# uiuc-robovision/video-dqn

Hardware: AMD Instinct MI355X
Metric: (s,a,r,s') TD-updates/sec, 224x224 frames, batch 256, 1/2/4/8 MI355X (higher is better)
Workload: dtype bf16; 1 GPU; HabitatDQNMultiAction ResNet-18 extra_capacity, 5 categories x 3 actions, full TD update (online fwd on [s;s'], target fwd on s', Double-DQN target + L2 TD loss, backward, Adam); batch_per_gpu=256, global_batch=256, frame=224x224x3 uint8 (normalise fused), parallelism=dp1, target_update_interval=1000, loss_clip=rect, loss_kind=l2, minibatch_pool=4, frame_pack=at the start of every update

## Files before the change

include/vdqn.h:

```cpp
#ifndef VDQN_H_
#define VDQN_H_

#include <stddef.h>
#include <stdint.h>

#ifdef __cplusplus
extern "C" {
#endif

#define VDQN_F32 0
#define VDQN_BF16 1
#define VDQN_F32X3 2

#define VDQN_OK 0
#define VDQN_ERR_INVALID (-1)
#define VDQN_ERR_LAUNCH (-2)

const char* vdqn_last_error(void);
int vdqn_abi_version(void);
int32_t vdqn_abi_struct_size(int32_t which);

typedef struct vdqn_prof_entry {
  char name[48];
  int64_t launches;
  double ms;
  double flops;
  double bytes;
} vdqn_prof_entry;
int vdqn_profile_enable(int on);
int vdqn_profile_collect(vdqn_prof_entry* out, int max_entries);


typedef struct vdqn_conv_args {
  const void* in;
  const void* wt;
  const float* bias;
  const void* resid;
  const void* mask;
  void* out;
  float* out_f32;
  float* colsum_part;
  int32_t n_img, hi, wi, ci, pix_stride;
  int32_t ho, wo, co, ldo;
  int32_t r, s, stride, pad;
  int32_t mode, relu, dtype;
  const void* in2;
  const void* wt2;
  const float* bias2;
  void* out2;
  int32_t co2, ldo2, relu2, ci2;
} vdqn_conv_args;
int vdqn_conv2d(const vdqn_conv_args* a, void* stream);
int32_t vdqn_conv2d_colsum_rows(const vdqn_conv_args* a);

typedef struct vdqn_wgrad_args {
  const void* gy;
  const void* x;
  float* dw;
  float* dbias;
  int32_t n_img, hi, wi, ci, pix_stride;
  int32_t ho, wo, co, ldg;
  int32_t r, s, stride, pad;
  int32_t splitk, dtype;
  void* workspace;
  int64_t workspace_bytes;
} vdqn_wgrad_args;
int vdqn_conv2d_wgrad(const vdqn_wgrad_args* a, void* stream);
int64_t vdqn_conv2d_wgrad_workspace_bytes(const vdqn_wgrad_args* a);

int vdqn_host_gather(void* dst, const void* const* src, int64_t n, int64_t bytes_each, int32_t threads);

int vdqn_pack_input(const void* src, int32_t src_kind, void* dst, int32_t n_img, int32_t dtype, void* stream);

int vdqn_maxpool_fwd(const void* in, void* out, uint8_t* idx, int32_t n_img, int32_t hi, int32_t wi, int32_t c,
                     int32_t dtype, void* stream);
int vdqn_maxpool_bwd(const void* gy, const uint8_t* idx, const void* x, void* gx, int32_t n_img, int32_t hi,
                     int32_t wi, int32_t c, int32_t dtype, void* stream);

typedef struct vdqn_td_args {
  const float* q_before;
  const float* q_after_online;
  const float* q_after_target;
  const int64_t* act;
  const float* rew;
  const float* term;
  const float* valid;
  float* loss;
  void* dq;
  float* dq_f32;
  int32_t batch, n_cat, n_act, ldq;
  float gamma, inv_count;
  int32_t clip_rect, linear, use_valid, dtype;
  int32_t loss_kind;
  int32_t deterministic;
  float* q_copy;
} vdqn_td_args;
int vdqn_td_loss(const vdqn_td_args* a, void* stream);
int vdqn_td_loss_weighted(const vdqn_td_args* a, const float* weight, float* err_out, void* stream);

int vdqn_gt_loss(const float* q_before, const int64_t* act, const float* gt, float* loss, void* dq, float* dq_f32,
                 int32_t batch, int32_t n_cat, int32_t n_act, int32_t ldq, float inv_count, int32_t value_learning,
                 int32_t dtype, void* stream);

int vdqn_stem_conv_pool(const void* t_in, const void* wt, const float* bias, void* pool, void* idx, int32_t n_img,
                        int32_t dtype, void* stream);
int vdqn_stem_conv_pool_n(const void* t_in, const void* wt, const float* bias, void* pool, void* idx, int32_t n_img,
                          int32_t n_idx_img, int32_t dtype, void* stream);

int vdqn_stem_wgrad_pool(const void* g_pool, const uint8_t* idx, const void* t_in, float* dw, int32_t n_img, void* workspace,
                         int64_t workspace_bytes, void* stream);
int64_t vdqn_stem_wgrad_pool_workspace_bytes(int32_t n_img);

int vdqn_softmax_rows(const float* x, float* y, int32_t rows, int32_t ld, int32_t n_valid, void* stream);

int vdqn_softmax_ce(const float* logits, const int64_t* labels, float* loss, void* dlogits, int32_t rows, int32_t ld,
                    int32_t n_cls, float inv_count, int32_t dtype, void* stream);
int vdqn_mask_scale(const void* x, const void* mask, void* out, int64_t n, float scale, int32_t dtype, void* stream);
int vdqn_axpy(float* y, const float* x, float alpha, int64_t n, void* stream);

int vdqn_adam(float* p, const float* g, float* m, float* v, int64_t n, int32_t step, double lr, double beta1,
              double beta2, double eps, void* stream);

int vdqn_bn_train_fwd(const void* y, const void* resid, void* z, const float* gamma, const float* beta,
                      float* running_mean, float* running_var, float* work, int32_t n_img, int32_t hw, int32_t c,
                      int32_t num_frames, int32_t imgs_per_half, int32_t relu, float momentum, float eps, int32_t dtype,
                      void* workspace, int64_t workspace_bytes, void* stream);
int vdqn_bn_train_bwd(const void* g, const void* y, void* dy, float* work, float* dgamma, float* dbeta, int32_t n_img,
                      int32_t hw, int32_t c, int32_t num_frames, int32_t imgs_per_half, int32_t dtype, void* workspace,
                      int64_t workspace_bytes, void* stream);
int64_t vdqn_bn_train_workspace_bytes(int32_t n_img, int32_t hw, int32_t c, int32_t num_frames, int32_t imgs_per_half);
int vdqn_avgpool_fwd(const void* x, void* out, int32_t n_img, int32_t hw, int32_t c, int32_t dtype, void* stream);
int vdqn_avgpool_bwd(const void* g, const void* x, void* gx, int32_t n_img, int32_t hw, int32_t c, int32_t dtype,
                     void* stream);

typedef struct vdqn_net_config {
  int32_t action_dim;
  int32_t num_classes;
  int32_t num_frames;
  int32_t extra_capacity;
  int32_t dtype;
// ... 60 lines not shown
  const float* term;
  const float* valid;
  const float* gt;
  float gamma;
  float inv_count;
  int32_t clip_rect, linear, use_valid, train_on_ground_truth, value_learning;
  void* acts_online;
  void* acts_target;
  void* bwd;
  float* grads;
  float* loss;
  float* q_before;
  int32_t loss_kind;
  const void* packed_frames;
  int32_t acts_samples;
} vdqn_step_args;
int vdqn_net_td_forward(vdqn_net* net, const vdqn_step_args* a, void* stream);
int vdqn_net_backward_stage(vdqn_net* net, const vdqn_step_args* a, int32_t stage, void* stream);
int vdqn_net_backward_begin(vdqn_net* net, const vdqn_step_args* a, const float* dq_f32, void* stream);
void* vdqn_net_grad_stream(vdqn_net* net);
int vdqn_net_set_sample_weights(vdqn_net* net, const float* weight, float* err_out);

int64_t vdqn_per_workspace_bytes(int64_t n);
int vdqn_per_sample(const float* prio, int64_t n, int32_t global_batch, uint64_t seed, uint64_t step, double beta, void* workspace,
                    int64_t* idx_out, float* weight_out, void* stream);
int vdqn_per_update(float* prio, int64_t n, const int64_t* idx, const float* err, int32_t global_batch, double alpha, void* stream);

int vdqn_aug_draw(uint64_t seed, uint64_t step, int32_t global_batch, int32_t first, int32_t n, int32_t pad, int32_t flip,
                  int32_t* params, void* stream);
int vdqn_aug_swap_actions(const int64_t* act, const int32_t* params, int32_t n, int32_t a0, int32_t a1, int64_t* act_out,
                          void* stream);
int vdqn_pack_input_aug(const void* src, void* dst, int32_t n_img, int32_t frames_per_sample, const int32_t* params,
                        int32_t n_params, int32_t dtype, void* stream);
int vdqn_net_set_augment(vdqn_net* net, const int32_t* params);

#define VDQN_COMM_UID_BYTES 128
typedef struct vdqn_comm vdqn_comm;
int vdqn_comm_unique_id(void* uid_host);
int vdqn_comm_init(int32_t rank, int32_t nranks, const void* uid_host, vdqn_comm** out);
int vdqn_allreduce_bucket(vdqn_comm* comm, void* ptr, int64_t count, int32_t dtype, void* stream);
int vdqn_comm_rank(const vdqn_comm* comm);
int vdqn_comm_size(const vdqn_comm* comm);
int vdqn_comm_destroy(vdqn_comm* comm);

#ifdef __cplusplus
}
#endif
#endif
```

video_dqn_amd/_lib.py:

```python
from __future__ import annotations

import ctypes as C
import os

import torch

_HERE = os.path.dirname(os.path.abspath(__file__))
LIB_PATH = os.path.join(_HERE, "lib", f"libvdqn{'_' + os.environ['VDQN_LIB'] if os.environ.get('VDQN_LIB') else ''}.so")

VDQN_F32, VDQN_BF16, VDQN_F32X3 = 0, 1, 2
ABI_VERSION = 15

c_i32, c_i64, c_f32, c_vp = C.c_int32, C.c_int64, C.c_float, C.c_void_p


class ConvArgs(C.Structure):
    _fields_ = [("in_", c_vp), ("wt", c_vp), ("bias", c_vp), ("resid", c_vp), ("mask", c_vp), ("out", c_vp),
                ("out_f32", c_vp), ("colsum_part", c_vp),
                ("n_img", c_i32), ("hi", c_i32), ("wi", c_i32), ("ci", c_i32), ("pix_stride", c_i32),
                ("ho", c_i32), ("wo", c_i32), ("co", c_i32), ("ldo", c_i32),
                ("r", c_i32), ("s", c_i32), ("stride", c_i32), ("pad", c_i32),
                ("mode", c_i32), ("relu", c_i32), ("dtype", c_i32),
                ("in2", c_vp), ("wt2", c_vp), ("bias2", c_vp), ("out2", c_vp),
                ("co2", c_i32), ("ldo2", c_i32), ("relu2", c_i32), ("ci2", c_i32),
]


class WgradArgs(C.Structure):
    _fields_ = [("gy", c_vp), ("x", c_vp), ("dw", c_vp), ("dbias", c_vp),
                ("n_img", c_i32), ("hi", c_i32), ("wi", c_i32), ("ci", c_i32), ("pix_stride", c_i32),
                ("ho", c_i32), ("wo", c_i32), ("co", c_i32), ("ldg", c_i32),
                ("r", c_i32), ("s", c_i32), ("stride", c_i32), ("pad", c_i32),
                ("splitk", c_i32), ("dtype", c_i32), ("workspace", c_vp), ("workspace_bytes", c_i64)]


class TdArgs(C.Structure):
    _fields_ = [("q_before", c_vp), ("q_after_online", c_vp), ("q_after_target", c_vp), ("act", c_vp),
                ("rew", c_vp), ("term", c_vp), ("valid", c_vp), ("loss", c_vp), ("dq", c_vp), ("dq_f32", c_vp),
                ("batch", c_i32), ("n_cat", c_i32), ("n_act", c_i32), ("ldq", c_i32),
                ("gamma", c_f32), ("inv_count", c_f32),
                ("clip_rect", c_i32), ("linear", c_i32), ("use_valid", c_i32), ("dtype", c_i32), ("loss_kind", c_i32), ("deterministic", c_i32), ("q_copy", c_vp)]


class NetConfig(C.Structure):
    _fields_ = [("action_dim", c_i32), ("num_classes", c_i32), ("num_frames", c_i32), ("extra_capacity", c_i32),
                ("dtype", c_i32), ("max_batch", c_i32), ("deterministic", c_i32)]


class ParamInfo(C.Structure):
    _fields_ = [("name", C.c_char * 96), ("offset", c_i64), ("numel", c_i64), ("ndim", c_i32),
                ("shape", c_i32 * 4), ("kind", c_i32), ("param_id", c_i32), ("stage", c_i32)]


class ProfEntry(C.Structure):
    _fields_ = [("name", C.c_char * 48), ("launches", c_i64), ("ms", C.c_double), ("flops", C.c_double),
                ("bytes", C.c_double)]


class StepArgs(C.Structure):
    _fields_ = [("params", c_vp), ("bnstats", c_vp), ("packed_online", c_vp), ("packed_target", c_vp),
                ("before", c_vp), ("after", c_vp), ("src_kind", c_i32), ("batch", c_i32),
                ("act", c_vp), ("rew", c_vp), ("term", c_vp), ("valid", c_vp), ("gt", c_vp),
                ("gamma", c_f32), ("inv_count", c_f32),
                ("clip_rect", c_i32), ("linear", c_i32), ("use_valid", c_i32), ("train_on_ground_truth", c_i32),
                ("value_learning", c_i32),
                ("acts_online", c_vp), ("acts_target", c_vp), ("bwd", c_vp), ("grads", c_vp), ("loss", c_vp),
                ("q_before", c_vp), ("loss_kind", c_i32), ("packed_frames", c_vp), ("acts_samples", c_i32)]


ALLREDUCE_FN = C.CFUNCTYPE(None, c_vp, c_vp, c_i64, c_vp)

_SIGS = {
    "vdqn_last_error": (C.c_char_p, []),
    "vdqn_abi_version": (C.c_int, []),
    "vdqn_profile_enable": (C.c_int, [C.c_int]),
    "vdqn_profile_collect": (C.c_int, [C.POINTER(ProfEntry), C.c_int]),
    "vdqn_conv2d": (C.c_int, [C.POINTER(ConvArgs), c_vp]),
    "vdqn_abi_struct_size": (c_i32, [c_i32]),
    "vdqn_conv2d_colsum_rows": (c_i32, [C.POINTER(ConvArgs)]),
    "vdqn_conv2d_wgrad": (C.c_int, [C.POINTER(WgradArgs), c_vp]),
    "vdqn_conv2d_wgrad_workspace_bytes": (c_i64, [C.POINTER(WgradArgs)]),
    "vdqn_pack_input": (C.c_int, [c_vp, c_i32, c_vp, c_i32, c_i32, c_vp]),
    "vdqn_maxpool_fwd": (C.c_int, [c_vp, c_vp, c_vp, c_i32, c_i32, c_i32, c_i32, c_i32, c_vp]),
    "vdqn_maxpool_bwd": (C.c_int, [c_vp, c_vp, c_vp, c_vp, c_i32, c_i32, c_i32, c_i32, c_i32, c_vp]),
    "vdqn_stem_conv_pool": (C.c_int, [c_vp, c_vp, c_vp, c_vp, c_vp, c_i32, c_i32, c_vp]),
    "vdqn_stem_conv_pool_n": (C.c_int, [c_vp, c_vp, c_vp, c_vp, c_vp, c_i32, c_i32, c_i32, c_vp]),
    "vdqn_td_loss": (C.c_int, [C.POINTER(TdArgs), c_vp]),
    "vdqn_gt_loss": (C.c_int, [c_vp, c_vp, c_vp, c_vp, c_vp, c_vp, c_i32, c_i32, c_i32, c_i32, c_f32, c_i32, c_i32, c_vp]),
    "vdqn_adam": (C.c_int, [c_vp, c_vp, c_vp, c_vp, c_i64, c_i32, C.c_double, C.c_double, C.c_double, C.c_double, c_vp]),
    "vdqn_bn_train_fwd": (C.c_int, [c_vp, c_vp, c_vp, c_vp, c_vp, c_vp, c_vp, c_vp, c_i32, c_i32, c_i32, c_i32, c_i32, c_i32,
                                    c_f32, c_f32, c_i32, c_vp, c_i64, c_vp]),
    "vdqn_bn_train_bwd": (C.c_int, [c_vp, c_vp, c_vp, c_vp, c_vp, c_vp, c_i32, c_i32, c_i32, c_i32, c_i32, c_i32, c_vp, c_i64, c_vp]),
    "vdqn_bn_train_workspace_bytes": (c_i64, [c_i32, c_i32, c_i32, c_i32, c_i32]),
    "vdqn_avgpool_fwd": (C.c_int, [c_vp, c_vp, c_i32, c_i32, c_i32, c_i32, c_vp]),
    "vdqn_avgpool_bwd": (C.c_int, [c_vp, c_vp, c_vp, c_i32, c_i32, c_i32, c_i32, c_vp]),
    "vdqn_net_create": (C.c_int, [C.POINTER(NetConfig), C.POINTER(c_vp)]),
    "vdqn_net_destroy": (None, [c_vp]),
    "vdqn_stem_wgrad_pool": (C.c_int, [c_vp, c_vp, c_vp, c_vp, c_i32, c_vp, c_i64, c_vp]),
    "vdqn_stem_wgrad_pool_workspace_bytes": (c_i64, [c_i32]),
    "vdqn_net_set_overlap": (C.c_int, [c_vp, C.c_int]),
    "vdqn_net_grad_stream": (c_vp, [c_vp]),
    "vdqn_net_set_bn_sync": (C.c_int, [c_vp, c_vp, c_vp, c_i32]),
    "vdqn_net_num_params": (C.c_int, [c_vp]),
    "vdqn_net_param_info": (C.c_int, [c_vp, C.c_int, C.POINTER(ParamInfo)]),
    "vdqn_net_params_numel": (c_i64, [c_vp]),
    "vdqn_net_trainable_numel": (c_i64, [c_vp]),
    "vdqn_net_bnstats_numel": (c_i64, [c_vp]),
    "vdqn_net_stage_range": (C.c_int, [c_vp, C.c_int, C.POINTER(c_i64), C.POINTER(c_i64)]),
    "vdqn_net_packed_bytes": (c_i64, [c_vp]),
    "vdqn_net_acts_bytes": (c_i64, [c_vp, c_i32]),
    "vdqn_net_bwd_bytes": (c_i64, [c_vp, c_i32]),
    "vdqn_net_act_offset": (c_i64, [c_vp, c_i32, C.c_char_p]),
    "vdqn_net_bwd_offset": (c_i64, [c_vp, c_i32, C.c_char_p]),
    "vdqn_net_pack_weights": (C.c_int, [c_vp, c_vp, c_vp, c_vp, c_i32, c_vp]),
    "vdqn_net_forward": (C.c_int, [c_vp, c_vp, c_vp, c_i32, c_i32, c_vp, c_vp, c_vp]),
    "vdqn_net_trunk_forward": (C.c_int, [c_vp, c_vp, c_vp, c_i32, c_i32, c_vp, c_vp]),
    "vdqn_softmax_rows": (C.c_int, [c_vp, c_vp, c_i32, c_i32, c_i32, c_vp]),
    "vdqn_softmax_ce": (C.c_int, [c_vp, c_vp, c_vp, c_vp, c_i32, c_i32, c_i32, c_f32, c_i32, c_vp]),
    "vdqn_mask_scale": (C.c_int, [c_vp, c_vp, c_vp, c_i64, c_f32, c_i32, c_vp]),
    "vdqn_axpy": (C.c_int, [c_vp, c_vp, c_f32, c_i64, c_vp]),
    "vdqn_net_forward_train": (C.c_int, [c_vp, c_vp, c_vp, c_vp, c_vp, c_i32, c_i32, c_vp, c_vp, c_vp]),
    "vdqn_net_td_forward": (C.c_int, [c_vp, C.POINTER(StepArgs), c_vp]),
    "vdqn_net_backward_stage": (C.c_int, [c_vp, C.POINTER(StepArgs), c_i32, c_vp]),
    "vdqn_net_backward_begin": (C.c_int, [c_vp, C.POINTER(StepArgs), c_vp, c_vp]),
    "vdqn_comm_unique_id": (C.c_int, [c_vp]),
    "vdqn_comm_init": (C.c_int, [c_i32, c_i32, c_vp, C.POINTER(c_vp)]),
    "vdqn_allreduce_bucket": (C.c_int, [c_vp, c_vp, c_i64, c_i32, c_vp]),
    "vdqn_comm_rank": (C.c_int, [c_vp]),
    "vdqn_comm_size": (C.c_int, [c_vp]),
    "vdqn_comm_destroy": (C.c_int, [c_vp]),
    "vdqn_host_gather": (C.c_int, [c_vp, c_vp, c_i64, c_i64, c_i32]),
    "vdqn_td_loss_weighted": (C.c_int, [C.POINTER(TdArgs), c_vp, c_vp, c_vp]),
    "vdqn_net_set_sample_weights": (C.c_int, [c_vp, c_vp, c_vp]),
    "vdqn_per_workspace_bytes": (c_i64, [c_i64]),
    "vdqn_per_sample": (C.c_int, [c_vp, c_i64, c_i32, C.c_uint64, C.c_uint64, C.c_double, c_vp, c_vp, c_vp, c_vp]),
    "vdqn_per_update": (C.c_int, [c_vp, c_i64, c_vp, c_vp, c_i32, C.c_double, c_vp]),
    "vdqn_aug_draw": (C.c_int, [C.c_uint64, C.c_uint64, c_i32, c_i32, c_i32, c_i32, c_i32, c_vp, c_vp]),
    "vdqn_aug_swap_actions": (C.c_int, [c_vp, c_vp, c_i32, c_i32, c_i32, c_vp, c_vp]),
    "vdqn_pack_input_aug": (C.c_int, [c_vp, c_vp, c_i32, c_i32, c_vp, c_i32, c_i32, c_vp]),
    "vdqn_net_set_augment": (C.c_int, [c_vp, c_vp]),
}
COMM_UID_BYTES = 128
EXPORTS = tuple(_SIGS)

_lib = None


class VdqnError(RuntimeError):
    pass


def load():
    global _lib
    if _lib is not None:
        return _lib
    if not os.path.exists(LIB_PATH):
        raise VdqnError(f"{LIB_PATH} is missing: build it with `python -m video_dqn_amd.build` "
                        "(the HIP extension is required; there is no CPU fallback)")
    lib = C.CDLL(LIB_PATH)
    for name, (res, args) in _SIGS.items():
        fn = getattr(lib, name)
        fn.restype = res
        fn.argtypes = args
    if lib.vdqn_abi_version() != ABI_VERSION:
        raise VdqnError(f"libvdqn ABI {lib.vdqn_abi_version()} != binding ABI {ABI_VERSION}: rebuild")
    for which, st in enumerate((ConvArgs, WgradArgs, TdArgs, NetConfig, ParamInfo, ProfEntry, StepArgs)):
        if lib.vdqn_abi_struct_size(which) != C.sizeof(st):
            raise VdqnError(f"libvdqn: sizeof({st.__name__}) is {lib.vdqn_abi_struct_size(which)} in the library, "
                            f"{C.sizeof(st)} in this binding: include/vdqn.h and video_dqn_amd/_lib.py have drifted apart")
    _lib = lib
    return lib

# ... 17 lines not shown
```

video_dqn_amd/augment.py:

```python
from __future__ import annotations

import torch

from . import _lib

MAX_PAD = 32


def check_config(pad, flip, flip_actions) -> None:
    if isinstance(pad, bool) or not isinstance(pad, int) or not 0 <= pad <= MAX_PAD:
        raise ValueError(f"AUG_SHIFT_PAD must be an integer in [0, {MAX_PAD}] (got {pad!r})")
    if not isinstance(flip, bool):
        raise ValueError(f"AUG_FLIP must be True or False (got {flip!r})")
    fa = list(flip_actions) if isinstance(flip_actions, (list, tuple)) else None
    if (fa is None or len(fa) != 2 or any(isinstance(a, bool) or not isinstance(a, int) for a in fa)
            or fa[0] == fa[1] or not all(0 <= a <= 2 for a in fa)):
        raise ValueError(f"AUG_FLIP_ACTIONS must be two different actions out of 0, 1, 2 (got {flip_actions!r})")


def _u64(v: int) -> int:
    return int(v) & (2**64 - 1)


def aug_draw(seed: int, step: int, global_batch: int, first: int, n: int, pad: int, flip: bool, device="cuda",
             out: torch.Tensor = None) -> torch.Tensor:
    dev = torch.device(device) if out is None else out.device
    with torch.cuda.device(dev):
        if out is None:
            out = torch.empty((n, 4), dtype=torch.int32, device=dev)
        _lib.check(_lib.load().vdqn_aug_draw(_u64(seed), _u64(step), global_batch, first, n, pad, int(bool(flip)), out.data_ptr(),
                                             torch.cuda.current_stream().cuda_stream), "vdqn_aug_draw")
    return out


def pack_input_aug(src: torch.Tensor, params: torch.Tensor, frames_per_sample: int, dtype: torch.dtype) -> torch.Tensor:
    if src.dtype != torch.uint8 or not src.is_contiguous() or params.dtype != torch.int32 or not params.is_contiguous():
        raise _lib.VdqnError("pack_input_aug: src must be contiguous uint8 NHWC frames and params contiguous int32 [*][4]")
    n_img = src.numel() // (224 * 224 * 3)
    with torch.cuda.device(src.device):
        dst = torch.empty((n_img, 115, 115, 16), dtype=dtype, device=src.device)
        code = _lib.VDQN_BF16 if dtype == torch.bfloat16 else _lib.VDQN_F32
        _lib.check(_lib.load().vdqn_pack_input_aug(src.data_ptr(), dst.data_ptr(), n_img, frames_per_sample, params.data_ptr(),
                                                   params.numel() // 4, code, torch.cuda.current_stream().cuda_stream), "vdqn_pack_input_aug")
    return dst


class Augmenter:

    def __init__(self, batch: int, device, pad: int = 0, flip: bool = False, flip_actions=(1, 2), seed: int = 0, rank: int = 0,
                 world_size: int = 1):
        check_config(pad, flip, flip_actions)
        self.lib = _lib.load()
        self.B, self.rank, self.world = int(batch), int(rank), int(world_size)
        self.G = self.B * self.world
        self.pad, self.flip, self.flip_actions, self.seed = int(pad), bool(flip), tuple(int(a) for a in flip_actions), int(seed)
        self.device = torch.device(device)
        with torch.cuda.device(self.device):
            self.params = torch.zeros((self.B, 4), dtype=torch.int32, device=self.device)
            self._act = torch.zeros(self.B, dtype=torch.int64, device=self.device)
        self.last_step = None

    def draw(self, step: int) -> torch.Tensor:
        aug_draw(self.seed, step, self.G, self.rank * self.B, self.B, self.pad, self.flip, out=self.params)
        self.last_step = int(step)
        return self.params

    def actions(self, act: torch.Tensor) -> torch.Tensor:
        if not self.flip:
            return act
        if act.dtype != torch.int64 or act.numel() != self.B or not act.is_contiguous() or act.device != self.params.device:
            raise _lib.VdqnError(f"Augmenter.actions: act must be a contiguous int64 [{self.B}] tensor on {self.params.device}")
        with torch.cuda.device(self.device):
            _lib.check(self.lib.vdqn_aug_swap_actions(act.data_ptr(), self.params.data_ptr(), self.B, self.flip_actions[0], self.flip_actions[1],
                                                      self._act.data_ptr(), torch.cuda.current_stream().cuda_stream), "vdqn_aug_swap_actions")
        return self._act
```

video_dqn_amd/csrc/augment.hip:

```cpp
#include "common.h"

namespace {

constexpr uint64_t kAugStream = 0x4155474D454E5431ull;
constexpr int kMaxPad = 32;

__host__ __device__ inline uint64_t splitmix64(uint64_t x) {
  uint64_t z = x + 0x9E3779B97F4A7C15ull;
  z = (z ^ (z >> 30)) * 0xBF58476D1CE4E5B9ull;
  z = (z ^ (z >> 27)) * 0x94D049BB133111EBull;
  return z ^ (z >> 31);
}

__global__ __launch_bounds__(256) void aug_draw_kernel(uint64_t seed, uint64_t step, int G, int first, int n, int pad, int flip_on,
                                                       int4* __restrict__ params) {
  const int i = blockIdx.x * blockDim.x + threadIdx.x;
  if (i >= n) return;
  const uint64_t key = splitmix64(seed ^ kAugStream);
  const uint64_t h = splitmix64(key ^ (step * (uint64_t)G + (uint64_t)(first + i)));
  const uint32_t span = 2u * (uint32_t)pad + 1u;
  const int sx = (int)((((uint32_t)h & 0xFFFFu) * span) >> 16) - pad;
  const int sy = (int)((((uint32_t)(h >> 16) & 0xFFFFu) * span) >> 16) - pad;
  params[i] = make_int4(sx, sy, flip_on ? (int)((h >> 32) & 1) : 0, 0);
}

__global__ __launch_bounds__(256) void aug_swap_actions_kernel(const int64_t* __restrict__ act, const int4* __restrict__ params, int n,
                                                               int64_t a0, int64_t a1, int64_t* __restrict__ act_out) {
  const int b = blockIdx.x * blockDim.x + threadIdx.x;
  if (b >= n) return;
  int64_t a = act[b];
  if (params[b].z != 0) a = a == a0 ? a1 : a == a1 ? a0 : a;
  act_out[b] = a;
}

constexpr int kPackPairs = 4;
__device__ __forceinline__ int clamp223(int v) { return min(max(v, 0), 223); }

template <typename T>
__global__ __launch_bounds__(256) void pack_input_aug_kernel(const uint8_t* __restrict__ src, T* __restrict__ dst, int frames_per_sample,
                                                             const int4* __restrict__ params, int n_params) {
  __shared__ uint4 rows[4][42];
  __shared__ T lut[3][256];
  const int n = blockIdx.y;
  const int tid = threadIdx.x;
  {
    const float mean[3] = {0.485f, 0.456f, 0.406f};
    const float stdv[3] = {0.229f, 0.224f, 0.225f};
#pragma unroll
    for (int c = 0; c < 3; ++c) lut[c][tid] = from_f32<T>((((float)tid / 255.0f) - mean[c]) / stdv[c]);
  }
  const int4 p = params[(n / frames_per_sample) % n_params];
  const int sx = min(max(p.x, -224), 224), sy = min(max(p.y, -224), 224);
  const bool flip = p.z != 0;
  const int yy = tid / 115, x = tid - yy * 115;
  int o0 = 0, o1 = 0;
  {
    const int xs = x - 2;
    int X0 = clamp223(2 * xs + sx), X1 = clamp223(2 * xs + 1 + sx);
    if (flip) {
      X0 = 223 - X0;
      X1 = 223 - X1;
    }
    o0 = 3 * X0;
    o1 = 3 * X1;
  }
  for (int pr = 0; pr < kPackPairs; ++pr) {
    const int y0 = 2 * ((int)blockIdx.x * kPackPairs + pr);
    if (y0 >= 115) break;
    const int Y0 = 2 * (y0 - 2);
    const bool inside = (unsigned)Y0 < 224u;
    const int Ys0 = clamp223(Y0 + sy), Ys3 = clamp223(Y0 + 3 + sy);
    __syncthreads();
    if (tid < 168 && inside) {
      const int s = tid / 42, c = tid - s * 42;
      if (Ys0 + s <= Ys3) rows[s][c] = reinterpret_cast<const uint4*>(src + ((size_t)n * 224 + (Ys0 + s)) * 672)[c];
    }
    __syncthreads();
    const int y = y0 + yy;
    if (tid >= 230 || y >= 115) continue;
    const int ys = y - 2, xs = x - 2;
    __attribute__((aligned(16))) T v[16];
#pragma unroll
    for (int e = 0; e < 16; ++e) v[e] = from_f32<T>(0.f);
    if (inside && (unsigned)ys < 112u && (unsigned)xs < 112u) {
      const int r0 = clamp223(Y0 + 2 * yy + sy) - Ys0, r1 = clamp223(Y0 + 2 * yy + 1 + sy) - Ys0;
      const uint8_t* b0 = reinterpret_cast<const uint8_t*>(rows[r0]);
      const uint8_t* b1 = reinterpret_cast<const uint8_t*>(rows[r1]);
#pragma unroll
      for (int c = 0; c < 3; ++c) {
        v[c] = lut[c][b0[o0 + c]];
        v[3 + c] = lut[c][b0[o1 + c]];
        v[6 + c] = lut[c][b1[o0 + c]];
        v[9 + c] = lut[c][b1[o1 + c]];
      }
    }
    T* d = dst + ((size_t)n * 115 * 115 + (size_t)y * 115 + x) * 16;
    constexpr int V16 = (int)(16 * sizeof(T) / 16);
#pragma unroll
    for (int q = 0; q < V16; ++q) reinterpret_cast<uint4*>(d)[q] = reinterpret_cast<const uint4*>(v)[q];
  }
// ... 2 lines not shown
}

extern "C" int vdqn_aug_draw(uint64_t seed, uint64_t step, int32_t global_batch, int32_t first, int32_t n, int32_t pad, int32_t flip,
                             int32_t* params, void* stream) {
  VDQN_CHECK(params, "vdqn_aug_draw: null params");
  VDQN_CHECK(n > 0, "vdqn_aug_draw: n = %d", n);
  VDQN_CHECK(global_batch >= 1 && first >= 0 && (int64_t)first + n <= (int64_t)global_batch,
             "vdqn_aug_draw: samples %d .. %lld outside the global batch of %d", first, (long long)first + n, global_batch);
  VDQN_CHECK(pad >= 0 && pad <= kMaxPad, "vdqn_aug_draw: pad %d outside [0, %d]", pad, kMaxPad);
  VDQN_CHECK(((uintptr_t)params & 15) == 0, "vdqn_aug_draw: params must be 16-byte aligned");
  ProfScope ps_("aug_draw", 0.0, (double)n * 16.0, (hipStream_t)stream);
  hipLaunchKernelGGL(aug_draw_kernel, dim3((n + 255) / 256), dim3(256), 0, (hipStream_t)stream, seed, step, (int)global_batch, (int)first, (int)n,
                     (int)pad, (int)(flip != 0), (int4*)params);
  VDQN_LAUNCH_CHECK();
  return VDQN_OK;
}

extern "C" int vdqn_aug_swap_actions(const int64_t* act, const int32_t* params, int32_t n, int32_t a0, int32_t a1, int64_t* act_out,
                                     void* stream) {
  VDQN_CHECK(act && params && act_out, "vdqn_aug_swap_actions: null arg");
  VDQN_CHECK(n > 0, "vdqn_aug_swap_actions: n = %d", n);
  VDQN_CHECK(a0 != a1 && a0 >= 0 && a0 <= 2 && a1 >= 0 && a1 <= 2, "vdqn_aug_swap_actions: actions (%d, %d) must be two different values of 0 .. 2",
             a0, a1);
  VDQN_CHECK(((uintptr_t)params & 15) == 0, "vdqn_aug_swap_actions: params must be 16-byte aligned");
  ProfScope ps_("aug_swap_actions", 0.0, (double)n * 32.0, (hipStream_t)stream);
  hipLaunchKernelGGL(aug_swap_actions_kernel, dim3((n + 255) / 256), dim3(256), 0, (hipStream_t)stream, act, (const int4*)params, (int)n,
                     (int64_t)a0, (int64_t)a1, act_out);
  VDQN_LAUNCH_CHECK();
  return VDQN_OK;
}

extern "C" int vdqn_pack_input_aug(const void* src, void* dst, int32_t n_img, int32_t frames_per_sample, const int32_t* params,
                                   int32_t n_params, int32_t dtype, void* stream) {
  VDQN_CHECK(src && dst && params, "vdqn_pack_input_aug: null arg");
  VDQN_CHECK(n_img > 0 && frames_per_sample > 0 && n_params > 0, "vdqn_pack_input_aug: n_img %d, frames_per_sample %d, n_params %d must be > 0",
             n_img, frames_per_sample, n_params);
  VDQN_CHECK(dtype == VDQN_F32 || dtype == VDQN_BF16, "vdqn_pack_input_aug: bad dtype");
  VDQN_CHECK((((uintptr_t)src | (uintptr_t)dst | (uintptr_t)params) & 15) == 0, "vdqn_pack_input_aug: src, dst and params must be 16-byte aligned");
  ProfScope ps_("pack_input_aug", 0.0, (double)n_img * (224.0 * 224 * 3 + 115.0 * 115 * 16 * (dtype == VDQN_BF16 ? 2 : 4)), (hipStream_t)stream);
  const dim3 grid((58 + kPackPairs - 1) / kPackPairs, n_img);
  if (dtype == VDQN_BF16)
    hipLaunchKernelGGL((pack_input_aug_kernel<bf16raw>), grid, dim3(256), 0, (hipStream_t)stream, (const uint8_t*)src, (bf16raw*)dst,
                       (int)frames_per_sample, (const int4*)params, (int)n_params);
  else
    hipLaunchKernelGGL((pack_input_aug_kernel<float>), grid, dim3(256), 0, (hipStream_t)stream, (const uint8_t*)src, (float*)dst,
                       (int)frames_per_sample, (const int4*)params, (int)n_params);
  VDQN_LAUNCH_CHECK();
  return VDQN_OK;
}
```

video_dqn_amd/csrc/common.h:

```cpp
#pragma once
#include <hip/hip_runtime.h>
#include <stdint.h>
#include <stdio.h>
#include <string.h>

#include "../../include/vdqn.h"

typedef uint16_t bf16raw;

typedef __attribute__((ext_vector_type(4))) float f32x4;
typedef __attribute__((ext_vector_type(8))) __bf16 bf16x8;
typedef __attribute__((ext_vector_type(4))) short s16x4;
typedef __attribute__((ext_vector_type(8))) short s16x8;

template <typename T> struct TInfo;
template <> struct TInfo<float> {
  static constexpr int kDtype = VDQN_F32;
  static constexpr int kPer16B = 4;
};
template <> struct TInfo<bf16raw> {
  static constexpr int kDtype = VDQN_BF16;
  static constexpr int kPer16B = 8;
};

// ... 5 lines not shown
__device__ __forceinline__ void split_bf16x8(const f32x4 x0, const f32x4 x1, bf16x8& hi, bf16x8& lo) {
#pragma unroll
  for (int j = 0; j < 8; ++j) {
    const float v = j < 4 ? x0[j] : x1[j - 4];
    const __bf16 h = (__bf16)v;
    hi[j] = h;
    lo[j] = (__bf16)(v - (float)h);
  }
}
template <typename T> __device__ __forceinline__ float to_f32(T v);
template <> __device__ __forceinline__ float to_f32<float>(float v) { return v; }
template <> __device__ __forceinline__ float to_f32<bf16raw>(bf16raw v) { return bf16_to_f32(v); }
template <typename T> __device__ __forceinline__ T from_f32(float v);
template <> __device__ __forceinline__ float from_f32<float>(float v) { return v; }
template <> __device__ __forceinline__ bf16raw from_f32<bf16raw>(float v) { return f32_to_bf16(v); }

struct FastDiv {
  uint64_t mul;
  uint32_t div;
};
static inline FastDiv make_fastdiv(uint32_t d) {
  FastDiv f;
  f.div = d;
  f.mul = ((1ull << 40) + d - 1) / d;
  return f;
}
__device__ __forceinline__ uint32_t fastdiv(uint32_t p, const FastDiv& f) { return (uint32_t)(((uint64_t)p * f.mul) >> 40); }

__device__ __forceinline__ uint32_t xcd_remap(uint32_t bid, uint32_t nblk) {
  const uint32_t q = nblk >> 3, r = nblk & 7, x = bid & 7, i = bid >> 3;
  return (x < r ? x * (q + 1) : r * (q + 1) + (x - r) * q) + i;
}

void vdqn_set_error(const char* fmt, ...);

void vdqn_ensure_dyn_smem(const void* kernel, size_t bytes);
int vdqn_num_cus();

void vdqn_prof_begin(const char* tag, double flops, double bytes, hipStream_t st);
void vdqn_prof_end(hipStream_t st);
extern thread_local double g_prof_alg_flops;
extern thread_local const char* g_prof_suffix;
struct ProfScope {
  hipStream_t st;
  ProfScope(const char* tag, double flops, double bytes, hipStream_t s) : st(s) { vdqn_prof_begin(tag, flops, bytes, s); }
  ~ProfScope() { vdqn_prof_end(st); }
};
struct BnSync {
  vdqn_allreduce_fn fn;
  void* user;
  float* scratch;
  int world;
  float* det_ws = nullptr;
  int64_t det_ws_bytes = 0;
};
int vdqn_bn_train_fwd_impl(const void* y, const void* resid, void* z, const float* gamma, const float* beta, float* running_mean,
                           float* running_var, float* work, int32_t n_img, int32_t hw, int32_t c, int32_t num_frames, int32_t imgs_per_half,
                           int32_t relu, float momentum, float eps, int32_t dtype, void* stream, const BnSync* sync);
int vdqn_bn_train_bwd_impl(const void* g, const void* y, void* dy, float* work, float* dgamma, float* dbeta, int32_t n_img, int32_t hw, int32_t c,
                           int32_t num_frames, int32_t imgs_per_half, int32_t dtype, void* stream, const BnSync* sync);

int vdqn_skinny_kind(const vdqn_conv_args* a);
int vdqn_skinny_part_rows(int conv);
int vdqn_launch_skinny(const void* igemm_params, int kind, hipStream_t stream);

#define VDQN_CHECK(cond, ...)        \
// ... 15 lines not shown
```

video_dqn_amd/csrc/engine.hip:

```cpp
#include <math.h>
#include <stdarg.h>
#include <stdlib.h>

#include <algorithm>
#include <string>
#include <vector>

#include "common.h"

static thread_local char g_err[512] = "";
void vdqn_set_error(const char* fmt, ...) {
  va_list ap;
  va_start(ap, fmt);
  vsnprintf(g_err, sizeof(g_err), fmt, ap);
  va_end(ap);
}
extern "C" const char* vdqn_last_error(void) { return g_err; }
extern "C" int vdqn_abi_version(void) { return 15; }
extern "C" int32_t vdqn_abi_struct_size(int32_t which) {
  switch (which) {
    case 0: return (int32_t)sizeof(vdqn_conv_args);
    case 1: return (int32_t)sizeof(vdqn_wgrad_args);
    case 2: return (int32_t)sizeof(vdqn_td_args);
    case 3: return (int32_t)sizeof(vdqn_net_config);
    case 4: return (int32_t)sizeof(vdqn_param_info);
    case 5: return (int32_t)sizeof(vdqn_prof_entry);
    case 6: return (int32_t)sizeof(vdqn_step_args);
    default: return -1;
  }
}

namespace {

constexpr int kMaxLayers = 24;
constexpr float kBnEps = 1e-5f;
constexpr float kBnMomentum = 0.1f;

enum LayerKind { K_CONV = 0, K_CONV1_S2D = 1, K_LINEAR = 2, K_LINEAR_PERM = 3 };

struct Layer {
  std::string name, bn_name;
  int kind;
  int co, ci, r, s, stride, pad;
  int has_bn, has_bias;
  int k_ci, k_r, k_s, pix_stride;
  int co_pad;
  int hi, wi, ho, wo;
  int per_sample;
  int stage, has_dgrad;
  int64_t w_off, g_off, b_off, mean_off, var_off;
  int64_t wf_off, wd_off, bias_off, scale_off;
// ... 25 lines not shown
  int64_t avg, r_c1, r_h[8], r_o[8], r_ds[8], bnw[kMaxLayers], bnw_begin, bnw_bytes, bn_sync;
  int64_t bn_det = -1, bn_det_bytes = 0;
  int64_t total;
};
struct BwdLayout {
  int64_t zero_begin, zero_bytes;
  int64_t dq, g_l1, g_l0, g_f8, g_o[8], g_h[8], dsg[8], g_pool, g_c1;
  int64_t p_l1, p_l0, p_f8, p_o[8], p_h[8], p_pool;
  int64_t g_avg, g_or[8], g_dsr[8];
  int64_t det_ws, det_ws_bytes;
  int64_t total;
};

inline int64_t align_up(int64_t v, int64_t a = 256) { return (v + a - 1) / a * a; }

}

struct vdqn_net {
  vdqn_net_config cfg;
  int gemm_dtype;
  int esz;
  std::vector<Layer> layers;
  std::vector<vdqn_param_info> params;
  int64_t trainable_numel, params_numel, bnstats_numel, packed_bytes;
  int64_t stage_begin[3], stage_end[3];
  int layer_stage_first[3], layer_stage_count[3];
  int64_t dw_bytes;
  FoldTable fold;
  int l_conv1, l_f8, l_top0, l_top2, l_top4;
  bool basic() const { return cfg.extra_capacity == 0; }
  int l_b_conv1[8], l_b_conv2[8], l_b_ds[8];
  BnSync bn_sync = {nullptr, nullptr, nullptr, 1};
  int wgrad_rr = 0;
  int overlap = 1;
  int bwd_samples = 0;
  const float* sample_w = nullptr;
  float* sample_err = nullptr;
  const int32_t* aug = nullptr;
  hipStream_t side = nullptr;
  hipStream_t side2 = nullptr;
  std::vector<hipEvent_t> events;
  size_t ev_next = 0;
};

namespace {

bool side_ready(vdqn_net* net) {
  if (!net->overlap) return false;
  if (!net->side) {
    int prio = 0;
    {
      const char* e = getenv("VDQN_SIDE_PRIORITY");
      int lo = 0, hi = 0;
      if (hipDeviceGetStreamPriorityRange(&lo, &hi) == hipSuccess) prio = (!e || e[0] == 'l') ? lo : (e[0] == 'h' ? hi : 0);
    }
    if (hipStreamCreateWithPriority(&net->side, hipStreamNonBlocking, prio) != hipSuccess ||
        hipStreamCreateWithPriority(&net->side2, hipStreamNonBlocking, prio) != hipSuccess) {
      net->overlap = 0;
      net->side = nullptr;
      net->side2 = nullptr;
      return false;
    }
    net->events.resize(64);
    for (auto& e : net->events)
      if (hipEventCreateWithFlags(&e, hipEventDisableTiming) != hipSuccess) {
        net->overlap = 0;
// ... 15 lines not shown
  return net->side;
}
void join_side(vdqn_net* net, hipStream_t main) {
  if (!net->overlap || !net->side) return;
  hipEvent_t e = next_event(net);
  (void)hipEventRecord(e, net->side);
  (void)hipStreamWaitEvent(main, e, 0);
}
hipStream_t fork_side2(vdqn_net* net, hipStream_t main) {
  if (!side_ready(net)) return main;
  hipEvent_t e = next_event(net);
  (void)hipEventRecord(e, main);
  (void)hipStreamWaitEvent(net->side2, e, 0);
  return net->side2;
}
void join_side2(vdqn_net* net, hipStream_t main) {
  if (!net->overlap || !net->side2) return;
  hipEvent_t e = next_event(net);
  (void)hipEventRecord(e, net->side2);
  (void)hipStreamWaitEvent(main, e, 0);
}

int g_wgrad_streams_override = -1;
bool wgrad_two_streams(const vdqn_net* net) {
  static const bool env_on = [] { const char* e = getenv("VDQN_WGRAD_STREAMS"); return !e || atoi(e) == 2; }();
  const bool on = g_wgrad_streams_override > 0 ? g_wgrad_streams_override == 2 : env_on;
  static const bool two_stage = [] { const char* e = getenv("VDQN_WGRAD_TWO_STAGE"); return e && e[0] == '1'; }();
  return on && !two_stage && !net->cfg.deterministic;
}
}
extern "C" void vdqn_debug_set_wgrad_streams(int v) { g_wgrad_streams_override = v; }
static int g_stem_wgrad_main_override = -1;
extern "C" void vdqn_debug_set_stem_wgrad_main(int v) { g_stem_wgrad_main_override = v; }
namespace {
hipStream_t wgrad_stream(vdqn_net* net, hipStream_t main) {
  if (!wgrad_two_streams(net)) return fork_side(net, main);
  net->wgrad_rr ^= 1;
  return net->wgrad_rr ? fork_side2(net, main) : fork_side(net, main);
}
void join_wgrad_streams(vdqn_net* net) {
  if (!wgrad_two_streams(net) || !net->overlap || !net->side2) return;
  hipEvent_t e = next_event(net);
  (void)hipEventRecord(e, net->side2);
  (void)hipStreamWaitEvent(net->side, e, 0);
}

__device__ __forceinline__ long fold_src_index(const FoldDesc& d, int co, int k) {
  if (d.kind == K_CONV1_S2D) {
    const int a = k >> 6, j = (k >> 4) & 3, ch = k & 15;
    if (ch >= 12) return -1;
    const int bh = ch / 6, bw = (ch / 3) & 1, c = ch % 3;
    const int r7 = 2 * a + bh - 1, s7 = 2 * j + bw - 1;
    if (r7 < 0 || s7 < 0) return -1;
    return ((long)(co * 3 + c) * 7 + r7) * 7 + s7;
  } else if (d.kind == K_LINEAR_PERM) {
    const int f = k / 1600, rem = k - f * 1600;
    const int hw = rem >> 6, c = rem & 63;
    return (long)co * d.ci + f * 1600 + c * 25 + hw;
  } else {
    const int tap = k / d.k_ci, c = k - tap * d.k_ci;
    const int kr = tap / d.k_s, ks = tap - kr * d.k_s;
    return (((long)co * d.ci + c) * d.r + kr) * d.s + ks;
  }
}

__device__ __forceinline__ float fold_scale(const FoldDesc& d, const float* params, const float* bnstats, int co, int raw) {
  if (!d.has_bn || raw) return 1.0f;
// ... 589 lines not shown
vdqn_wgrad_args wgrad_shape_args(const vdqn_net* net, const Layer& L, int n_units) {
  vdqn_wgrad_args a;
  memset(&a, 0, sizeof(a));
  a.n_img = n_units; a.hi = L.hi; a.wi = L.wi; a.ci = L.k_ci; a.pix_stride = L.pix_stride;
  a.ho = L.ho; a.wo = L.wo; a.co = L.co_pad; a.ldg = L.co_pad;
  a.r = L.k_r; a.s = L.k_s;
  a.stride = L.kind == K_CONV1_S2D ? 1 : L.stride;
  a.pad = L.kind == K_CONV1_S2D ? 0 : L.pad;
  a.splitk = 0; a.dtype = net->gemm_dtype;
  return a;
}
int64_t wgrad_max_imgs(const vdqn_net* net, const Layer& L) {
  const int64_t esz = net->esz;
  const int64_t pix = (int64_t)L.ho * L.wo, gy_img = pix * L.co_pad * esz, x_img = (int64_t)L.hi * L.wi * L.pix_stride * esz;
  int64_t m = ((1ll << 24) - 1) / pix;
  m = std::min(m, (int64_t)0x7ffffffell / gy_img);
  m = std::min(m, (int64_t)0x7ffffffell / x_img);
  return m;
}

bool wgrad_two_stage() {
  static const bool on = [] { const char* e = getenv("VDQN_WGRAD_TWO_STAGE"); return e && e[0] == '1'; }();
  return on;
}

int fuse_ds_mask() {
  static const int m = [] { const char* e = getenv("VDQN_FUSE_DS"); return e ? atoi(e) : 3; }();
  return m;
}
bool fuse_ds() { return (fuse_ds_mask() & 1) != 0; }
bool fuse_ds_fwd(int dtype) { return (fuse_ds_mask() & 2) != 0 && (dtype == VDQN_BF16 || (fuse_ds_mask() & 4) != 0); }

int run_conv(const vdqn_net* net, const Layer& L, const unsigned char* packed, const void* in, void* out, int n_units, const void* resid,
             int relu, float* out_f32, hipStream_t st, const Layer* sib = nullptr, void* sib_out = nullptr) {
  vdqn_conv_args a;
  memset(&a, 0, sizeof(a));
  a.in = in;
  a.wt = packed + L.wf_off;
  a.bias = reinterpret_cast<const float*>(packed + L.bias_off);
  a.resid = resid;
  a.mask = nullptr;
  a.out = out;
  a.out_f32 = out_f32;
  a.n_img = n_units; a.hi = L.hi; a.wi = L.wi; a.ci = L.k_ci; a.pix_stride = L.pix_stride;
  a.ho = L.ho; a.wo = L.wo; a.co = L.co_pad; a.ldo = L.co_pad;
  a.r = L.k_r; a.s = L.k_s;
  a.stride = L.kind == K_CONV1_S2D ? 1 : L.stride;
  a.pad = L.kind == K_CONV1_S2D ? 0 : L.pad;
  a.mode = 0; a.relu = relu; a.dtype = net->gemm_dtype;
  g_prof_alg_flops = 2.0 * n_units * L.ho * L.wo * (double)L.co * L.ci * L.r * L.s;
  if (sib) {
    a.wt2 = packed + sib->wf_off;
    a.bias2 = reinterpret_cast<const float*>(packed + sib->bias_off);
    a.out2 = sib_out;
    a.co2 = sib->co_pad; a.ldo2 = sib->co_pad; a.relu2 = 0;
    g_prof_alg_flops += 2.0 * n_units * sib->ho * sib->wo * (double)sib->co * sib->ci;
  }
  prof_layer(L, n_units);
  return vdqn_conv2d(&a, st);
}

int run_dgrad(const vdqn_net* net, const Layer& L, const unsigned char* packed, const void* gy, void* gx, int n_units, const void* resid,
              const void* mask, hipStream_t st, void* colsum_part = nullptr, const Layer* sib = nullptr, const void* sib_gy = nullptr,
              int* part_rows = nullptr) {
  vdqn_conv_args a;
  memset(&a, 0, sizeof(a));
  a.in = gy;
  a.wt = packed + L.wd_off;
  a.bias = nullptr;
  a.resid = resid;
  a.mask = mask;
  a.out = gx;
  a.colsum_part = reinterpret_cast<float*>(colsum_part);
  a.n_img = n_units; a.hi = L.ho; a.wi = L.wo; a.ci = L.co_pad; a.pix_stride = L.co_pad;
  a.ho = L.hi; a.wo = L.wi; a.co = L.k_ci; a.ldo = L.k_ci;
  a.r = L.k_r; a.s = L.k_s; a.stride = L.stride; a.pad = L.pad;
  a.mode = 1; a.relu = 0; a.dtype = net->gemm_dtype;
  g_prof_alg_flops = 2.0 * n_units * L.ho * L.wo * (double)L.co * L.ci * L.r * L.s;
  if (sib) {
    a.in2 = sib_gy;
    a.wt2 = packed + sib->wd_off;
    a.ci2 = sib->co_pad;
    g_prof_alg_flops += 2.0 * n_units * sib->ho * sib->wo * (double)sib->co * sib->ci;
  }
  if (part_rows) {
    const int kind = vdqn_skinny_kind(&a);
    *part_rows = kind ? vdqn_skinny_part_rows(kind == 2) : 128;
  }
  prof_layer(L, n_units);
  return vdqn_conv2d(&a, st);
}

int run_wgrad(const vdqn_net* net, const Layer& L, unsigned char* bwd, const void* gy, const void* x, int n_units, hipStream_t st,
              bool colsum_kernel = false) {
  vdqn_wgrad_args a = wgrad_shape_args(net, L, n_units);
  a.gy = gy;
  a.x = x;
  a.dw = reinterpret_cast<float*>(bwd + L.dw_off);
  a.dbias = colsum_kernel ? reinterpret_cast<float*>(bwd + L.db_off) : nullptr;
  if (net->cfg.deterministic || wgrad_two_stage()) {
    const BwdLayout W = bwd_layout(net, net->bwd_samples);
    a.workspace = bwd + W.det_ws;
    a.workspace_bytes = W.det_ws_bytes;
  }
  const int64_t esz = net->esz;
  const int64_t pix = (int64_t)L.ho * L.wo, gy_img = pix * L.co_pad * esz, x_img = (int64_t)L.hi * L.wi * L.pix_stride * esz;
  const int64_t max_imgs = wgrad_max_imgs(net, L);
  if (max_imgs < 1) {
    vdqn_set_error("run_wgrad: one image of layer %s exceeds the weight-gradient kernel's addressing range", L.name.c_str());
    return VDQN_ERR_INVALID;
  }
  for (int64_t i0 = 0; i0 < n_units; i0 += max_imgs) {
    const int n_chunk = (int)std::min<int64_t>(max_imgs, n_units - i0);
    a.gy = (const unsigned char*)gy + i0 * gy_img;
    a.x = (const unsigned char*)x + i0 * x_img;
    a.n_img = n_chunk;
    g_prof_alg_flops = 2.0 * n_chunk * L.ho * L.wo * (double)L.co * L.ci * L.r * L.s;
    prof_layer(L, n_chunk);
    const int rc = vdqn_conv2d_wgrad(&a, st);
    if (rc != VDQN_OK) return rc;
  }
  return VDQN_OK;
}

#define RC(x)                     \
  do {                            \
    int rc_ = (x);                \
    if (rc_ != VDQN_OK) return rc_; \
  } while (0)

int forward_impl(const vdqn_net* net, const unsigned char* packed, const void* t_in, int n_samples, unsigned char* acts, const ActLayout& A,
                 hipStream_t st, bool trunk_only = false, int grad_samples = -1) {
  const int n = n_samples * net->cfg.num_frames;
  const int dt = net->cfg.dtype;
  static const bool stem_noidx = [] { const char* e = getenv("VDQN_STEM_NOIDX"); return !(e && e[0] == '0'); }();
  const int n_idx = (grad_samples >= 0 && stem_noidx) ? (grad_samples * net->cfg.num_frames < n ? grad_samples * net->cfg.num_frames : n) : n;
  if (A.c1 >= 0) {
    RC(run_conv(net, net->layers[net->l_conv1], packed, t_in, acts + A.c1, n, nullptr, 1, nullptr, st));
    RC(vdqn_maxpool_fwd(acts + A.c1, acts + A.pool, acts + A.idx, n, 112, 112, 64, dt, st));
  } else {
    const Layer& L1 = net->layers[net->l_conv1];
    prof_layer(L1, n);
    RC(vdqn_stem_conv_pool_n(t_in, packed + L1.wf_off, reinterpret_cast<const float*>(packed + L1.bias_off), acts + A.pool, acts + A.idx, n, n_idx, net->gemm_dtype, st));
  }
  const unsigned char* x = acts + A.pool;
  for (int b = 0; b < 8; ++b) {
    const Layer& c1 = net->layers[net->l_b_conv1[b]];
    const Layer& c2 = net->layers[net->l_b_conv2[b]];
    const void* identity = x;
    if (net->l_b_ds[b] >= 0 && fuse_ds_fwd(dt)) {
      RC(run_conv(net, c1, packed, x, acts + A.h[b], n, nullptr, 1, nullptr, st, &net->layers[net->l_b_ds[b]], acts + A.ds[b]));
      identity = acts + A.ds[b];
    } else {
      RC(run_conv(net, c1, packed, x, acts + A.h[b], n, nullptr, 1, nullptr, st));
      if (net->l_b_ds[b] >= 0) {
        RC(run_conv(net, net->layers[net->l_b_ds[b]], packed, x, acts + A.ds[b], n, nullptr, 0, nullptr, st));
        identity = acts + A.ds[b];
      }
    }
    RC(run_conv(net, c2, packed, acts + A.h[b], acts + A.o[b], n, identity, 1, nullptr, st));
    x = acts + A.o[b];
  }
  if (trunk_only) return VDQN_OK;
  if (net->basic()) {
    RC(vdqn_avgpool_fwd(x, acts + A.avg, n, 49, 512, dt, st));
    RC(run_conv(net, net->layers[net->l_top4], packed, acts + A.avg, acts + A.q, n_samples, nullptr, 0, reinterpret_cast<float*>(acts + A.qf), st));
    return VDQN_OK;
  }
  RC(run_conv(net, net->layers[net->l_f8], packed, x, acts + A.f8, n, nullptr, 1, nullptr, st));
  RC(run_conv(net, net->layers[net->l_top0], packed, acts + A.f8, acts + A.l0, n_samples, nullptr, 1, nullptr, st));
  RC(run_conv(net, net->layers[net->l_top2], packed, acts + A.l0, acts + A.l1, n_samples, nullptr, 1, nullptr, st));
  RC(run_conv(net, net->layers[net->l_top4], packed, acts + A.l1, acts + A.q, n_samples, nullptr, 0, reinterpret_cast<float*>(acts + A.qf), st));
  return VDQN_OK;
}

int run_bn(const vdqn_net* net, int li, const float* params, float* bnstats, unsigned char* acts, const ActLayout& A, const void* y,
           const void* resid, void* z, int n_img, int iph, int relu, hipStream_t st) {
  const Layer& L = net->layers[li];
  BnSync sy = net->bn_sync;
  sy.scratch = reinterpret_cast<float*>(acts + A.bn_sync);
  if (A.bn_det >= 0) {
    sy.det_ws = reinterpret_cast<float*>(acts + A.bn_det);
    sy.det_ws_bytes = A.bn_det_bytes;
  }
  return vdqn_bn_train_fwd_impl(y, resid, z, params + L.g_off, params + L.b_off, bnstats + L.mean_off, bnstats + L.var_off,
                                reinterpret_cast<float*>(acts + A.bnw[li]), n_img, L.ho * L.wo, L.co, net->cfg.num_frames, iph, relu, kBnMomentum,
                                kBnEps, net->cfg.dtype, st, &sy);
}

int forward_train_impl(const vdqn_net* net, const unsigned char* packed, const float* params, float* bnstats, const void* t_in, int n_samples,
                       int halves, unsigned char* acts, const ActLayout& A, hipStream_t st) {
  const int F = net->cfg.num_frames, n = n_samples * F, iph = n / halves;
  const int dt = net->cfg.dtype;
  RC(run_conv(net, net->layers[net->l_conv1], packed, t_in, acts + A.r_c1, n, nullptr, 0, nullptr, st));
  RC(run_bn(net, net->l_conv1, params, bnstats, acts, A, acts + A.r_c1, nullptr, acts + A.c1, n, iph, 1, st));
  RC(vdqn_maxpool_fwd(acts + A.c1, acts + A.pool, acts + A.idx, n, 112, 112, 64, dt, st));
  const unsigned char* x = acts + A.pool;
  for (int b = 0; b < 8; ++b) {
    const int i1 = net->l_b_conv1[b], i2 = net->l_b_conv2[b], ids = net->l_b_ds[b];
    RC(run_conv(net, net->layers[i1], packed, x, acts + A.r_h[b], n, nullptr, 0, nullptr, st));
    RC(run_bn(net, i1, params, bnstats, acts, A, acts + A.r_h[b], nullptr, acts + A.h[b], n, iph, 1, st));
    RC(run_conv(net, net->layers[i2], packed, acts + A.h[b], acts + A.r_o[b], n, nullptr, 0, nullptr, st));
    const void* identity = x;
    if (ids >= 0) {
      RC(run_conv(net, net->layers[ids], packed, x, acts + A.r_ds[b], n, nullptr, 0, nullptr, st));
// ... 295 lines not shown
    t.clip_rect = a->clip_rect; t.linear = a->linear; t.use_valid = a->use_valid; t.dtype = dt;
    t.loss_kind = a->loss_kind;
    t.deterministic = net->cfg.deterministic;
    t.q_copy = a->q_before;
    if (net->sample_w) RC(vdqn_td_loss_weighted(&t, net->sample_w, net->sample_err, st));
    else RC(vdqn_td_loss(&t, st));
  } else {
    VDQN_CHECK(!net->sample_w, "vdqn_net_td_forward: sample weights are set, but the ground-truth branch has no weighted loss");
    RC(vdqn_gt_loss(qf_online, a->act, a->gt, a->loss, bw + W.dq, nullptr, B, net->cfg.num_classes, net->cfg.action_dim, 64, a->inv_count,
                    a->value_learning, dt, st));
  }
  if (a->q_before && gtb) {
    const int nq = net->cfg.action_dim * net->cfg.num_classes;
    e = hipMemcpy2DAsync(a->q_before, (size_t)nq * 4, qf_online, 64 * 4, (size_t)nq * 4, (size_t)B, hipMemcpyDeviceToDevice, st);
    VDQN_CHECK(e == hipSuccess, "vdqn_net_td_forward: q copy failed: %s", hipGetErrorString(e));
  }
  return VDQN_OK;
}

namespace {

int block_backward(vdqn_net* net, const vdqn_step_args* a, int b, const ActLayout& A, const BwdLayout& W, int n, hipStream_t st) {
  const unsigned char* pk = (const unsigned char*)a->packed_online;
  unsigned char* ao = (unsigned char*)a->acts_online;
  unsigned char* bw = (unsigned char*)a->bwd;
  const Layer& c1 = net->layers[net->l_b_conv1[b]];
  const Layer& c2 = net->layers[net->l_b_conv2[b]];
  const unsigned char* x = b == 0 ? ao + A.pool : ao + A.o[b - 1];
  unsigned char* gx = b == 0 ? bw + W.g_pool : bw + W.g_o[b - 1];
  const void* g_out = bw + W.g_o[b];
  hipStream_t ws = wgrad_stream(net, st);
  RC(run_wgrad(net, c2, bw, g_out, ao + A.h[b], n, ws));
  if (net->l_b_ds[b] >= 0) RC(run_wgrad(net, net->layers[net->l_b_ds[b]], bw, g_out, x, n, ws));
  RC(run_dgrad(net, c2, pk, g_out, bw + W.g_h[b], n, nullptr, ao + A.h[b], st, bw + W.p_h[b]));
  ws = wgrad_stream(net, st);
  RC(run_wgrad(net, c1, bw, bw + W.g_h[b], x, n, ws));
  const void* resid = g_out;
  if (net->l_b_ds[b] >= 0) {
    const Layer& ds = net->layers[net->l_b_ds[b]];
    if (fuse_ds()) {
      RC(run_dgrad(net, c1, pk, bw + W.g_h[b], gx, n, nullptr, x, st, b > 0 ? bw + W.p_o[b - 1] : bw + W.p_pool, &ds, g_out));
      return VDQN_OK;
    }
    RC(run_dgrad(net, ds, pk, g_out, bw + W.dsg[b], n, nullptr, nullptr, st));
    resid = bw + W.dsg[b];
  }
  RC(run_dgrad(net, c1, pk, bw + W.g_h[b], gx, n, resid, x, st, b > 0 ? bw + W.p_o[b - 1] : bw + W.p_pool));
  return VDQN_OK;
}

int run_bn_bwd(const vdqn_net* net, const vdqn_step_args* a, int li, const ActLayout& A, const void* g, const void* y, void* dy, int n,
               hipStream_t st) {
  const Layer& L = net->layers[li];
  BnSync sy = net->bn_sync;
  sy.scratch = reinterpret_cast<float*>((unsigned char*)a->acts_online + A.bn_sync);
  if (A.bn_det >= 0) {
    sy.det_ws = reinterpret_cast<float*>((unsigned char*)a->acts_online + A.bn_det);
    sy.det_ws_bytes = A.bn_det_bytes;
  }
  return vdqn_bn_train_bwd_impl(g, y, dy, reinterpret_cast<float*>((unsigned char*)a->acts_online + A.bnw[li]), a->grads + L.g_off, a->grads + L.b_off,
                                n, L.ho * L.wo, L.co, net->cfg.num_frames, n, net->cfg.dtype, st, &sy);
}

int block_backward_train(vdqn_net* net, const vdqn_step_args* a, int b, const ActLayout& A, const BwdLayout& W, int n, hipStream_t st) {
  const unsigned char* pk = (const unsigned char*)a->packed_online;
  unsigned char* ao = (unsigned char*)a->acts_online;
  unsigned char* bw = (unsigned char*)a->bwd;
  const int i1 = net->l_b_conv1[b], i2 = net->l_b_conv2[b], ids = net->l_b_ds[b];
  const Layer& c1 = net->layers[i1];
  const Layer& c2 = net->layers[i2];
  const unsigned char* x = b == 0 ? ao + A.pool : ao + A.o[b - 1];
  unsigned char* gx = b == 0 ? bw + W.g_pool : bw + W.g_o[b - 1];
  const void* g_out = bw + W.g_o[b];
  RC(run_bn_bwd(net, a, i2, A, g_out, ao + A.r_o[b], bw + W.g_or[b], n, st));
  hipStream_t ws = fork_side(net, st);
  RC(run_wgrad(net, c2, bw, bw + W.g_or[b], ao + A.h[b], n, ws));
  if (ids >= 0) {
    RC(run_bn_bwd(net, a, ids, A, g_out, ao + A.r_ds[b], bw + W.g_dsr[b], n, st));
    ws = fork_side(net, st);
    RC(run_wgrad(net, net->layers[ids], bw, bw + W.g_dsr[b], x, n, ws));
// ... 63 lines not shown
  bool split_conv1 = false;
  int pr_l1 = 128, pr_l0 = 128, pr_f8 = 128;

  if (net->basic()) {
    if (stage == 0) {
      const Layer& top = net->layers[net->l_top4];
      RC(run_wgrad(net, top, bw, bw + W.dq, ao + A.avg, B, wgrad_stream(net, st), true));
      RC(run_dgrad(net, top, pk, bw + W.dq, bw + W.g_avg, B, nullptr, nullptr, st));
      RC(vdqn_avgpool_bwd(bw + W.g_avg, ao + A.o[7], bw + W.g_o[7], n, 49, 512, dt, st));
      RC(block_backward_train(net, a, 7, A, W, n, st));
      RC(block_backward_train(net, a, 6, A, W, n, st));
    } else if (stage == 1) {
      RC(block_backward_train(net, a, 5, A, W, n, st));
      RC(block_backward_train(net, a, 4, A, W, n, st));
    } else {
      for (int b = 3; b >= 0; --b) RC(block_backward_train(net, a, b, A, W, n, st));
      RC(vdqn_maxpool_bwd(bw + W.g_pool, ao + A.idx, nullptr, bw + W.g_c1, n, 112, 112, 64, dt, st));
      RC(run_bn_bwd(net, a, net->l_conv1, A, bw + W.g_c1, ao + A.r_c1, bw + W.g_c1, n, st));
      RC(run_wgrad(net, net->layers[net->l_conv1], bw, bw + W.g_c1, a->packed_frames ? a->packed_frames : ao + A.t_in, n, wgrad_stream(net, st)));
    }
  } else if (stage == 0) {
    const Layer& t4 = net->layers[net->l_top4];
    const Layer& t2 = net->layers[net->l_top2];
    const Layer& t0 = net->layers[net->l_top0];
    const Layer& f8 = net->layers[net->l_f8];
    RC(run_wgrad(net, t4, bw, bw + W.dq, ao + A.l1, B, wgrad_stream(net, st), true));
    RC(run_dgrad(net, t4, pk, bw + W.dq, bw + W.g_l1, B, nullptr, ao + A.l1, st, bw + W.p_l1, nullptr, nullptr, &pr_l1));
    RC(run_wgrad(net, t2, bw, bw + W.g_l1, ao + A.l0, B, wgrad_stream(net, st)));
    RC(run_dgrad(net, t2, pk, bw + W.g_l1, bw + W.g_l0, B, nullptr, ao + A.l0, st, bw + W.p_l0, nullptr, nullptr, &pr_l0));
    RC(run_wgrad(net, t0, bw, bw + W.g_l0, ao + A.f8, B, wgrad_stream(net, st)));
    RC(run_dgrad(net, t0, pk, bw + W.g_l0, bw + W.g_f8, B, nullptr, ao + A.f8, st, bw + W.p_f8, nullptr, nullptr, &pr_f8));
    RC(run_wgrad(net, f8, bw, bw + W.g_f8, ao + A.o[7], n, wgrad_stream(net, st)));
    RC(run_dgrad(net, f8, pk, bw + W.g_f8, bw + W.g_o[7], n, nullptr, ao + A.o[7], st, bw + W.p_o[7]));
    RC(block_backward(net, a, 7, A, W, n, st));
    RC(block_backward(net, a, 6, A, W, n, st));
  } else if (stage == 1) {
    RC(block_backward(net, a, 5, A, W, n, st));
    RC(block_backward(net, a, 4, A, W, n, st));
  } else {
    for (int b = 3; b >= 0; --b) RC(block_backward(net, a, b, A, W, n, st));
    split_conv1 = net->overlap && net->side && net->l_conv1 == net->layer_stage_first[2] && net->layer_stage_count[2] > 1;
  }
  int max_co = 0;
  for (int i = net->layer_stage_first[stage]; i < net->layer_stage_first[stage] + net->layer_stage_count[stage]; ++i)
    max_co = net->layers[i].co > max_co ? net->layers[i].co : max_co;
  PartTable pt;
  memset(&pt, 0, sizeof(pt));
  if (!net->basic()) {
    auto tiles = [](int64_t rows) { return (int)((rows + 127) / 128); };
    auto set = [&](int li, int64_t off, int64_t rows, int ld, int groups, int gstride) {
      if (li < 0) return;
      pt.off[li] = off; pt.tiles[li] = tiles(rows); pt.ld[li] = ld; pt.groups[li] = groups; pt.gstride[li] = gstride;
    };
    set(net->l_top2, W.p_l1, B, 256, 1, 0);
    set(net->l_top0, W.p_l0, B, 512, 1, 0);
    set(net->l_f8, W.p_f8, B, 1600 * F, 25 * F, 64);
    if (stage == 0) {
      pt.tiles[net->l_top2] = (B + pr_l1 - 1) / pr_l1;
      pt.tiles[net->l_top0] = (B + pr_l0 - 1) / pr_l0;
      pt.tiles[net->l_f8] = (B + pr_f8 - 1) / pr_f8;
    }
    set(net->l_conv1, W.p_pool, (int64_t)n * 56 * 56, 64, 1, 0);
    for (int b = 0; b < 8; ++b) {
      const int planes = 64 << (b / 2), sp = 56 >> (b / 2);
      set(net->l_b_conv2[b], W.p_o[b], (int64_t)n * sp * sp, planes, 1, 0);
      set(net->l_b_ds[b], W.p_o[b], (int64_t)n * sp * sp, planes, 1, 0);
// ... 51 lines not shown
```

video_dqn_amd/csrc/igemm.hip:

```cpp
#include <stdlib.h>

#include "common.h"

int vdqn_stem_bf16(const void* t_in, const void* wt, const float* bias, void* pool, void* idx, int n_img, int n_idx_img, hipStream_t st);
int vdqn_launch_win9s(const void* igemm_params, hipStream_t stream);
int vdqn_win9s_supports(int cpk, int has_sib);
int vdqn_launch_win9d(const void* igemm_params, hipStream_t stream);
int vdqn_win9d_supports(int ci, int co, int has_sib, int ci2);
int vdqn_launch_win9u(const void* igemm_params, int mode, hipStream_t stream);

#include "igemm_common.h"

namespace {

template <typename T, int BM, int BN, int MODE, int WN, int NS = 2, bool X3 = false>
__global__ __launch_bounds__(BM * WN, 2) void igemm_kernel(const IgemmParams p) {
  static_assert(!X3 || sizeof(T) == 4, "bf16x3 splits f32 operands");
  constexpr int NT = BM * WN;
  constexpr int RPS = NT / 8;
  constexpr int ESZ = (int)sizeof(T);
  constexpr int KC = 128 / ESZ;
  constexpr int NF = BN / (16 * WN);
  constexpr int CPL = 4 * NF;
  constexpr int BROWS = BN / RPS;
  constexpr int AROWS = BM / RPS;
  static_assert(AROWS == 4 || AROWS == 8, "A staging is issued in groups of four pieces");
  static_assert(NF == 2 || NF == 4, "wave tile is 64 x 32 or 64 x 64");
  constexpr int PSTR = RPS * 128;
  extern __shared__ __attribute__((aligned(16))) unsigned char smem[];
  static_assert(NS == 2 || (NS == 4 && (MODE == 0 || MODE == 1)), "deep ring: forward / stride-1 data gradient only");
  unsigned char* sA = smem;
  unsigned char* sB = smem + NS * BM * 128;

  const int tid = threadIdx.x;
  const int lane = tid & 63, wave = tid >> 6;
  const uint32_t lb = xcd_remap(blockIdx.x, gridDim.x);
  const int tile_n = (int)(lb % (uint32_t)p.tiles_n), tile_m = (int)(lb / (uint32_t)p.tiles_n);
  const bool sib = MODE == 0 && tile_n >= p.tiles_n1;
  const int n0 = (sib ? tile_n - p.tiles_n1 : tile_n) * BN;
  int m0 = tile_m * BM, nk = p.nk, kr0 = 0, ks0 = 0, cls_ph = 0, cls_pw = 0;
  if constexpr (MODE == 2) {
    const int cls = p.cls_interleave ? (tile_m & 3) : (tile_m >= p.cls_tile0[1]) + (tile_m >= p.cls_tile0[2]) + (tile_m >= p.cls_tile0[3]);
    m0 = (p.cls_interleave ? (tile_m >> 2) : (tile_m - p.cls_tile0[cls])) * BM;
    cls_ph = cls >> 1;
    cls_pw = cls & 1;
    kr0 = (cls_ph + p.pad) & 1;
    ks0 = (cls_pw + p.pad) & 1;
    const int nkr = p.r > kr0 ? (p.r - kr0 + 1) / 2 : 0, nks = p.s > ks0 ? (p.s - ks0 + 1) / 2 : 0;
    nk = nkr * nks * (p.ci / KC);
  }
  if (sib) {
    kr0 = p.r >> 1;
    ks0 = p.s >> 1;
    nk = p.ci / KC;
  }
  const int nk2 = (MODE == 2 && p.in2 != nullptr && cls_ph == 0 && cls_pw == 0) ? p.ci2 / KC : 0;
  const int nk_all = nk + nk2;
  constexpr bool FWD = (MODE == 0 || MODE == 3);
  const int st_img = MODE == 3 ? tile_m >> 6 : 0, st_ty = (tile_m >> 3) & 7, st_tx = tile_m & 7;
  const int row_w = MODE == 2 ? p.cls_w[cls_pw] : p.wo;
  const int pix_per_img = MODE == 2 ? p.cls_h[cls_ph] * row_w : p.howo;
  const int rows_total = MODE == 2 ? p.n_img * pix_per_img : p.M;
  const int lrow = tid >> 3;
  const int lchunk_a = (tid & 7) ^ (lrow & 7);
  const int lchunk_b = (tid & 7) ^ ((((lrow / CPL) & 1) << 2) | (lrow & 3));

  const int img0 = MODE == 3 ? st_img : m0 / pix_per_img;
  const long long img_bytes = (long long)p.hi * p.wi * p.pix_stride * ESZ;
  const long long a_base_off = (long long)img0 * img_bytes;
// ... 414 lines not shown
        const int img = mm / pix_per_img;
        const int rem = mm - img * pix_per_img;
        const int ohc = rem / row_w;
        const int mo = (img * p.ho + 2 * ohc + cls_ph) * p.wo + 2 * (rem - ohc * row_w) + cls_pw;
        off[f] = ok ? (uint32_t)(mo * p.ldo + ncol) * 2u : kOob;
      }
      lean_epilogue_dgrad<NF>(led, acc, reinterpret_cast<float*>(smem), off, n0, tile_m, tid);
      return;
    }
  }
  igemm_epilogue<T, BM, BN, MODE, WN>(p, acc, smem, m0, n0, tile_m, rows_total, pix_per_img, row_w, cls_ph, cls_pw, p.bias);
}

template <typename T, int BN, int MODE, bool X3 = false>
__global__ __launch_bounds__(256, BN == 64 ? 3 : 2) void igemm_win_kernel(const IgemmParams p) {
  static_assert(MODE == 0 || MODE == 1, "window kernel: forward or stride-1 data gradient");
  static_assert(!X3 || sizeof(T) == 4, "bf16x3 splits f32 operands");
  constexpr int BM = 128, WN = 2, RPS = 32, AROWS = 4;
  constexpr int ESZ = (int)sizeof(T);
  constexpr int KC = 128 / ESZ;
  constexpr int NF = BN / (16 * WN);
  constexpr int CPL = 4 * NF;
  constexpr int BROWS = BN / RPS;
  constexpr int PSTR = RPS * 128;
  constexpr int WROWS = BM + 8;
  constexpr int WBYTES = WROWS * 128;
  extern __shared__ __attribute__((aligned(16))) unsigned char smem[];
  unsigned char* sA = smem;
  unsigned char* sB = smem + 2 * WBYTES;
  unsigned char* sZ = smem + 2 * WBYTES + 2 * BN * 128;

  const int tid = threadIdx.x;
  const int lane = tid & 63, wave = tid >> 6;
  const uint32_t lb = xcd_remap(blockIdx.x, gridDim.x);
  const int tile_n = (int)(lb % (uint32_t)p.tiles_n), tile_m = (int)(lb / (uint32_t)p.tiles_n);
  const int n0 = tile_n * BN, m0 = tile_m * BM;
  const int nk = p.nk;
  const int row_w = p.wo, pix_per_img = p.howo, rows_total = p.M;
  const int lrow = tid >> 3;
  const int lchunk_a = (tid & 7) ^ (lrow & 7);
  const int lchunk_b = (tid & 7) ^ ((((lrow / CPL) & 1) << 2) | (lrow & 3));
  if (tid < 8) reinterpret_cast<uint4*>(sZ)[tid] = make_uint4(0, 0, 0, 0);

  const int q0 = m0 > 0 ? m0 - 1 : 0;
  const int img0 = q0 / pix_per_img;
  const long long img_bytes = (long long)p.hi * p.wi * p.pix_stride * ESZ;
  const long long a_base_off = (long long)img0 * img_bytes;
  long long a_rem = p.in_bytes - a_base_off;
  if (a_rem > 0x7fffffffLL) a_rem = 0x7fffffffLL;
  const unsigned long long a_ptr = (unsigned long long)((const unsigned char*)p.in + a_base_off);
  const unsigned long long b_ptr = (unsigned long long)p.wt;
  const i32x4 rs_a = {__builtin_amdgcn_readfirstlane((int)(unsigned)a_ptr), __builtin_amdgcn_readfirstlane((int)((a_ptr >> 32) & 0xffff)),
                      __builtin_amdgcn_readfirstlane((int)a_rem), 0x00020000};
  const i32x4 rs_b = {__builtin_amdgcn_readfirstlane((int)(unsigned)b_ptr), __builtin_amdgcn_readfirstlane((int)((b_ptr >> 32) & 0xffff)),
                      __builtin_amdgcn_readfirstlane(p.wt_bytes), 0x00020000};

  const int pixB = p.pix_stride * ESZ;
  uint32_t a_off[AROWS + 1];
  int a_hb[AROWS + 1];
#pragma unroll
  for (int i = 0; i <= AROWS; ++i) {
    const int j = i < AROWS ? lrow + RPS * i : BM + (lrow & 7);
    const int q = m0 - 1 + j;
    const bool ok = q >= 0 && q < rows_total;
    const int qq = ok ? q : q0;
    const int img = qq / pix_per_img;
    const int rem = qq - img * pix_per_img;
// ... 180 lines not shown
                  esz * ((double)p.n_img * p.hi * p.wi * p.ci + (double)p.co * p.ktot + (double)p.M * p.co * (1 + (p.resid != nullptr) + (p.mask != nullptr))),
                  stream);
  hipLaunchKernelGGL((igemm_win_kernel<T, BN, MODE, X3>), dim3(grid), dim3(256), smem, stream, p);
  vdqn_prof_end(stream);
  VDQN_LAUNCH_CHECK();
  return VDQN_OK;
}

template <typename T, int MODE>
__global__ __launch_bounds__(256, 2) void igemm_win9_kernel(const IgemmParams p, const int wrows, const FastDiv d_wo, const FastDiv d_howo) {
  static_assert(MODE == 0 || MODE == 1, "window kernel: forward or stride-1 data gradient");
  constexpr int BM = 128, BN = 128, WN = 2, RPS = 32;
  constexpr int ESZ = (int)sizeof(T);
  constexpr int KC = 128 / ESZ;
  constexpr int NF = BN / (16 * WN);
  constexpr int CPL = 4 * NF;
  constexpr int BROWS = BN / RPS;
  constexpr int PSTR = RPS * 128;
  constexpr int NPASS = 6;
  const int WBYTES = wrows * 128;
  extern __shared__ __attribute__((aligned(16))) unsigned char smem[];
  unsigned char* sA = smem;
  unsigned char* sB = smem + 2 * WBYTES;

  const int tid = threadIdx.x;
  const int lane = tid & 63, wave = tid >> 6;
#ifdef VDQN_PRIO
  {
    unsigned hwid_p;
    asm volatile("s_getreg_b32 %0, hwreg(HW_REG_HW_ID)" : "=s"(hwid_p));
    if (hwid_p & 1) __builtin_amdgcn_s_setprio(VDQN_PRIO);
  }
#endif
  const uint32_t lb = xcd_remap(blockIdx.x, gridDim.x);
  const int tile_n = (int)(lb % (uint32_t)p.tiles_n), tile_m = (int)(lb / (uint32_t)p.tiles_n);
  const int n0 = tile_n * BN, m0 = tile_m * BM;
  const int nk = p.nk;
  const int W = p.wo, H = p.ho, rows_total = p.M;
  const int lrow = tid >> 3;
  const int lchunk_a = (tid & 7) ^ (lrow & 7);
  const int lchunk_b = (tid & 7) ^ ((((lrow / CPL) & 1) << 2) | (lrow & 3));

  const unsigned long long a_ptr = (unsigned long long)p.in;
  const unsigned long long b_ptr = (unsigned long long)p.wt;
  const i32x4 rs_a = {__builtin_amdgcn_readfirstlane((int)(unsigned)a_ptr), __builtin_amdgcn_readfirstlane((int)((a_ptr >> 32) & 0xffff)),
                      __builtin_amdgcn_readfirstlane((int)p.in_bytes), 0x00020000};
  const i32x4 rs_b = {__builtin_amdgcn_readfirstlane((int)(unsigned)b_ptr), __builtin_amdgcn_readfirstlane((int)((b_ptr >> 32) & 0xffff)),
                      __builtin_amdgcn_readfirstlane(p.wt_bytes), 0x00020000};

  const int pixB = p.pix_stride * ESZ;
  const int need = BM + 2 * W + 2;
  uint32_t a_off[NPASS];
#pragma unroll
  for (int i = 0; i < NPASS; ++i) {
    const int j = lrow + RPS * i;
    const int q = m0 - W - 1 + j;
    a_off[i] = (j < need && (unsigned)q < (unsigned)rows_total) ? (uint32_t)q * (uint32_t)pixB + (uint32_t)(lchunk_a * 16) : kOob;
  }
  uint32_t b_off[BROWS];
#pragma unroll
  for (int i = 0; i < BROWS; ++i) b_off[i] = (uint32_t)(n0 + lrow + RPS * i) * (uint32_t)(p.ktot * ESZ) + (uint32_t)(lchunk_b * 16);

  const uint32_t lds_base = (uint32_t)(uintptr_t)(__attribute__((address_space(3))) unsigned char*)smem;
  const int wave_u = __builtin_amdgcn_readfirstlane(wave);
  const uint32_t lds_wave = lds_base + (uint32_t)wave_u * (8 * 128);
  const int npass_w = (wrows - 8 * wave_u + 31) / 32;

// ... 286 lines not shown
      if (wave_u < 3) {
        const uint32_t l2_ = l_ + (uint32_t)PSTR;
        asm volatile("s_nop 4\n\ts_mov_b32 m0, %1\n\ts_nop 0\n\tbuffer_load_dwordx4 %0, %2, 0 offen lds" ::"v"(vo[7]), "s"(l2_), "s"(rs_a) : "memory");
      }
    }
  };

  auto issue_window_part = [&](int tl, int buf, int part) {
    const int q0 = tl * 128 - W - 1;
    const uint32_t v0 = (uint32_t)(q0 + lrow + 32 * (2 * part)) * 128u + (uint32_t)(lchunk * 16);
    const uint32_t v1 = v0 + 32u * 128u;
    const uint32_t l_ = lds_wave + (uint32_t)(buf * kC64WinBytes) + (uint32_t)(2 * part * PSTR);
    if (part < 3) {
      asm volatile(
          "s_mov_b32 m0, %2\n\ts_nop 0\n\tbuffer_load_dwordx4 %0, %3, 0 offen lds\n\t"
          "s_add_u32 m0, %2, %4\n\ts_nop 0\n\tbuffer_load_dwordx4 %1, %3, 0 offen lds"
          ::"v"(v0), "v"(v1), "s"(l_), "s"(rs_a), "n"(PSTR)
          : "memory", "scc");
    } else {
      asm volatile("s_mov_b32 m0, %1\n\ts_nop 0\n\tbuffer_load_dwordx4 %0, %2, 0 offen lds" ::"v"(v0), "s"(l_), "s"(rs_a) : "memory");
      if (wave_u < 3) {
        const uint32_t l2_ = l_ + (uint32_t)PSTR;
        asm volatile("s_mov_b32 m0, %1\n\ts_nop 0\n\tbuffer_load_dwordx4 %0, %2, 0 offen lds" ::"v"(v1), "s"(l2_), "s"(rs_a) : "memory");
      }
    }
  };
  (void)issue_window_part;
#ifndef VDQN_C64_SPREAD
#define VDQN_C64_SPREAD 1
#endif
  constexpr bool kSpread = VDQN_C64_SPREAD == 2 || (VDQN_C64_SPREAD == 1 && MODE == 0);
  const uint32_t c64_adv_oh = (uint32_t)((16 / W) % H), c64_adv_ow = (uint32_t)(16 - (16 / W) * W);
  int t = g_bid, buf = 0;
  if (t < g_tiles) issue_window(g_first + (int)xcd_remap((uint32_t)t, (uint32_t)g_tiles), 0);
  for (; t < g_tiles; t += g_blocks, buf ^= 1) {
    const int tl = g_first + (int)xcd_remap((uint32_t)t, (uint32_t)g_tiles);
    const int m0 = tl * 128;
#ifdef VDQN_STAMP
    const unsigned long long st_w0 = __builtin_amdgcn_s_memtime();
#endif
    asm volatile("s_waitcnt vmcnt(0)" ::: "memory");
    __builtin_amdgcn_s_barrier();
#ifdef VDQN_STAMP
    const int st_k = (t - g_bid) / g_blocks;
    unsigned long long* st_row = (p.pool_out && st_k < 16) ? reinterpret_cast<unsigned long long*>(p.pool_out) + ((size_t)blockIdx.x * 16 + st_k) * 8 : nullptr;
    if (st_row && tid == 0) { st_row[0] = st_w0; st_row[1] = __builtin_amdgcn_s_memtime(); }
#endif
    const bool c64_has_nx = t + g_blocks < g_tiles;
    const int c64_tl_nx = c64_has_nx ? g_first + (int)xcd_remap((uint32_t)(t + g_blocks), (uint32_t)g_tiles) : 0;
    if constexpr (!kSpread) {
      if (c64_has_nx) issue_window(c64_tl_nx, buf ^ 1);
    }
#ifdef VDQN_STAMP
    if (st_row && tid == 0) st_row[2] = __builtin_amdgcn_s_memtime();
#endif
#pragma unroll
    for (int f = 0; f < 4; ++f) __builtin_amdgcn_raw_buffer_store_b128(held[f], r_out, (int)held_off[f], 0, 0);
    __builtin_amdgcn_raw_buffer_store_b32(__float_as_uint(held_cs), r_cs, (int)held_cs_off, 0, 0);

    uint32_t edge = 0u;
    {
      const uint32_t m = (uint32_t)(m0 + wr * 64 + i16);
      const uint32_t rem = m - fastdiv(m, d_howo) * d_howo.div;
      uint32_t oh = fastdiv(rem, d_wo), ow = rem - oh * d_wo.div;
      const uint32_t adv_oh = c64_adv_oh, adv_ow = c64_adv_ow;
#pragma unroll
      for (int f = 0; f < 4; ++f) {
        edge |= ((oh == 0 ? 1u : 0u) | (oh == (uint32_t)H - 1 ? 2u : 0u) | (ow == 0 ? 4u : 0u) | (ow == (uint32_t)W - 1 ? 8u : 0u)) << (4 * f);
        ow += adv_ow;
        oh += adv_oh;
        const bool c1 = ow >= (uint32_t)W;
        ow -= c1 ? (uint32_t)W : 0u;
        oh += c1 ? 1u : 0u;
        oh -= oh >= (uint32_t)H ? (uint32_t)H : 0u;
      }
    }
    f32x4 acc[4][2];
#pragma unroll
    for (int f = 0; f < 4; ++f)
#pragma unroll
      for (int j = 0; j < 2; ++j) acc[f][j] = (f32x4){0.f, 0.f, 0.f, 0.f};
    const unsigned char* a_rd = smem + buf * kC64WinBytes + (wr * 64 + i16) * 128;
// ... 219 lines not shown
  if (mode == 0) return launch_igemm<T, BM, BN, 0, 2, X3>(p, st);
  if (mode == 1) return launch_igemm<T, BM, BN, 1, 2, X3>(p, st);
  if constexpr (BM == 128) return launch_igemm<T, BM, BN, 2, 2, X3>(p, st);
  return VDQN_ERR_INVALID;
}

}

#ifdef VDQN_STAMP
extern "C" void vdqn_debug_stamp_buffer(void* p) { g_stamp_buffer = p; }
#endif

extern "C" int vdqn_conv2d(const vdqn_conv_args* a, void* stream) {
  VDQN_CHECK(a != nullptr, "vdqn_conv2d: null args");
  VDQN_CHECK(a != nullptr, "vdqn_conv2d: null args");
  VDQN_CHECK(a->dtype == VDQN_F32 || a->dtype == VDQN_BF16 || a->dtype == VDQN_F32X3, "vdqn_conv2d: bad dtype %d", a->dtype);
  const int esz = a->dtype == VDQN_BF16 ? 2 : 4;
  const bool x3 = a->dtype == VDQN_F32X3;
  const int kc = 128 / esz;
  VDQN_CHECK(a->in && a->wt && (a->out || a->out_f32), "vdqn_conv2d: null tensor");
  VDQN_CHECK(a->ci > 0 && a->ci % kc == 0, "vdqn_conv2d: ci=%d must be a multiple of %d", a->ci, kc);
  VDQN_CHECK(a->stride == 1 || a->stride == 2, "vdqn_conv2d: stride %d unsupported", a->stride);
  VDQN_CHECK(a->mode == 0 || a->mode == 1, "vdqn_conv2d: bad mode %d", a->mode);
  VDQN_CHECK(a->n_img > 0 && a->ho > 0 && a->wo > 0 && a->co > 0 && a->ldo >= a->co, "vdqn_conv2d: bad dims");
  VDQN_CHECK((int64_t)a->n_img * a->ho * a->wo < (1ll << 31), "vdqn_conv2d: too many output pixels");
  VDQN_CHECK((a->pix_stride * esz) % 16 == 0 && (((uintptr_t)a->in | (uintptr_t)a->wt) & 15) == 0, "vdqn_conv2d: in/wt must be 16-byte aligned");
  IgemmParams p;
  p.in = a->in; p.wt = a->wt; p.bias = a->bias; p.resid = a->resid; p.mask = a->mask; p.out = a->out; p.out_f32 = a->out_f32; p.colsum_part = a->colsum_part;
  p.pool_out = nullptr; p.pool_idx = nullptr;
  p.in2 = nullptr; p.wt2 = nullptr; p.bias2 = nullptr; p.out2 = nullptr;
  p.co2 = p.ldo2 = p.relu2 = p.ci2 = p.wt2_bytes = 0;
  static const int no_lean = [] { const char* e = getenv("VDQN_LEAN_EPILOGUE"); return (e && e[0] == '0') ? 1 : 0; }();
  p.no_lean = no_lean;
  p.n_img = a->n_img; p.hi = a->hi; p.wi = a->wi; p.ci = a->ci; p.pix_stride = a->pix_stride;
  p.ho = a->ho; p.wo = a->wo; p.co = a->co; p.ldo = a->ldo; p.r = a->r; p.s = a->s; p.stride = a->stride; p.pad = a->pad;
  p.relu = a->relu;
  p.M = a->n_img * a->ho * a->wo;
  p.howo = a->ho * a->wo;
  p.ktot = a->r * a->s * a->ci;
  p.nk = p.ktot / kc;
  const int bn = (a->co % 128 == 0) ? 128 : 64;
  p.tiles_m = (p.M + 127) / 128;
  memset(p.cls_tile0, 0, sizeof(p.cls_tile0));
  p.cls_h[0] = p.cls_h[1] = p.cls_w[0] = p.cls_w[1] = 0;
  p.cls_interleave = 0;
  if (a->mode == 1 && a->stride == 2) {
    p.cls_h[0] = (a->ho + 1) / 2; p.cls_h[1] = a->ho / 2;
    p.cls_w[0] = (a->wo + 1) / 2; p.cls_w[1] = a->wo / 2;
    for (int c = 0; c < 4; ++c) p.cls_tile0[c + 1] = p.cls_tile0[c] + (a->n_img * p.cls_h[c >> 1] * p.cls_w[c & 1] + 127) / 128;
    p.tiles_m = p.cls_tile0[4];
    static const int inter = [] { const char* e = getenv("VDQN_DGRAD_S2_INTERLEAVE"); return e ? atoi(e) : 1; }();
    p.cls_interleave = inter && p.cls_h[0] == p.cls_h[1] && p.cls_w[0] == p.cls_w[1];
  }
  p.tiles_n = (a->co + bn - 1) / bn;
  p.tiles_n1 = p.tiles_n;
  const bool has_sib = a->wt2 != nullptr;
  if (has_sib) {
    VDQN_CHECK(a->r == 3 && a->s == 3 && a->stride == 2 && a->pad == 1, "vdqn_conv2d: a sibling 1x1 needs a 3x3 / stride-2 / pad-1 call");
    VDQN_CHECK((((uintptr_t)a->wt2) & 15) == 0, "vdqn_conv2d: wt2 must be 16-byte aligned");
    if (a->mode == 0) {
      VDQN_CHECK(a->out2 && a->co2 > 0 && a->ldo2 >= a->co2 && a->co2 % bn == 0 && bn == 128 && !a->out_f32 && !a->colsum_part,
                 "vdqn_conv2d: fused sibling (forward) needs out2, co2 a multiple of the 128-column tile, no f32 copy / column sums");
      VDQN_CHECK(((a->ldo2 * esz) % 16 == 0) && ((((uintptr_t)a->out2) & 15) == 0) && (a->ldo2 % 8 == 0), "vdqn_conv2d: out2 must be 16-byte aligned rows");
      p.wt2 = a->wt2; p.bias2 = a->bias2; p.out2 = a->out2; p.co2 = a->co2; p.ldo2 = a->ldo2; p.relu2 = a->relu2;
      p.wt2_bytes = (int)((long long)a->co2 * a->ci * esz);
      p.tiles_n = p.tiles_n1 + a->co2 / bn;
// ... 42 lines not shown
      if (bn == 128) return mode == 0 ? launch_igemm_win<float, 128, 0, true>(p, st) : launch_igemm_win<float, 128, 1, true>(p, st);
      return mode == 0 ? launch_igemm_win<float, 64, 0, true>(p, st) : launch_igemm_win<float, 64, 1, true>(p, st);
    }
    if (bn == 128) return mode == 0 ? launch_igemm_win<float, 128, 0>(p, st) : launch_igemm_win<float, 128, 1>(p, st);
    return mode == 0 ? launch_igemm_win<float, 64, 0>(p, st) : launch_igemm_win<float, 64, 1>(p, st);
  }
  static const int use_s2win = [] { const char* e = getenv("VDQN_S2WIN"); return e ? atoi(e) : 1; }();
  if (use_s2win && mode == 0 && a->dtype == VDQN_BF16 && a->r == 3 && a->s == 3 && a->stride == 2 && a->pad == 1 &&
      bn == 128 && a->co % 128 == 0 && a->hi == 2 * a->ho && a->wi == 2 * a->wo && a->wo >= 2 && a->wo <= 28 && a->pix_stride == a->ci && a->ci % 64 == 0 &&
      p.in_bytes < 0x7fffffffLL && !a->colsum_part && !a->mask && vdqn_win9s_supports(a->ci / 64, has_sib) &&
      (!has_sib || (a->co2 == a->co && p.vec_ok && !a->out_f32 && !a->resid))) {
    return vdqn_launch_win9s(&p, st);
  }
  static const int use_s2dwin = [] { const char* e = getenv("VDQN_S2DGRAD_WIN"); return e ? atoi(e) : 1; }();
  if (use_s2dwin && mode == 2 && a->dtype == VDQN_BF16 && a->r == 3 && a->s == 3 && a->pad == 1 && a->ho == 2 * a->hi && a->wo == 2 * a->wi &&
      a->wi >= 2 && a->wi <= 28 && a->pix_stride == a->ci && p.vec_ok && a->out && !a->out_f32 && !a->bias && !p.no_lean &&
      p.in_bytes < 0x7fffffffLL && (long long)p.M * a->ldo * 2 < 0x7fffffffLL && (long long)a->co * p.ktot * 2 < 0x7fffffffLL &&
      vdqn_win9d_supports(a->ci, a->co, has_sib, a->ci2)) {
    return vdqn_launch_win9d(&p, st);
  }
  static const long long min256 = [] { const char* e = getenv("VDQN_BM256_MIN_ROWS"); return e ? atoll(e) : 256ll * 1024; }();
  if (bn == 64 && mode != 2 && p.M >= min256 && !has_sib) {
    p.tiles_m = (p.M + 255) / 256;
    if (x3) return launch_mode<float, 256, 64, true>(p, mode, st);
    return a->dtype == VDQN_BF16 ? launch_mode<bf16raw, 256, 64>(p, mode, st) : launch_mode<float, 256, 64>(p, mode, st);
  }
  if (a->dtype == VDQN_BF16) return bn == 128 ? launch_mode<bf16raw, 128, 128>(p, mode, st) : launch_mode<bf16raw, 128, 64>(p, mode, st);
  if (x3) return bn == 128 ? launch_mode<float, 128, 128, true>(p, mode, st) : launch_mode<float, 128, 64, true>(p, mode, st);
  return bn == 128 ? launch_mode<float, 128, 128>(p, mode, st) : launch_mode<float, 128, 64>(p, mode, st);
}

extern "C" int vdqn_stem_conv_pool_n(const void* t_in, const void* wt, const float* bias, void* pool, void* idx, int32_t n_img, int32_t n_idx_img,
                                     int32_t dtype, void* stream) {
  VDQN_CHECK(t_in && wt && bias && pool && n_img > 0 && n_idx_img >= 0 && n_idx_img <= n_img && (idx || n_idx_img == 0), "vdqn_stem_conv_pool: bad args");
  VDQN_CHECK(dtype == VDQN_F32 || dtype == VDQN_BF16 || dtype == VDQN_F32X3, "vdqn_stem_conv_pool: bad dtype %d", dtype);
  VDQN_CHECK((((uintptr_t)t_in | (uintptr_t)wt | (uintptr_t)pool | (uintptr_t)idx) & 15) == 0, "vdqn_stem_conv_pool: tensors must be 16-byte aligned");
  const int esz = dtype == VDQN_BF16 ? 2 : 4;
  VDQN_CHECK((long long)n_img * 64 < (1ll << 31) / 256, "vdqn_stem_conv_pool: too many images");
  IgemmParams p;
  memset(&p, 0, sizeof(p));
  p.in = t_in; p.wt = wt; p.bias = bias; p.pool_out = pool; p.pool_idx = (uint8_t*)idx; p.n_idx_img = n_idx_img;
  p.n_img = n_img; p.hi = 115; p.wi = 115; p.ci = 64; p.pix_stride = 16;
  p.ho = 112; p.wo = 112; p.co = 64; p.ldo = 64; p.r = 4; p.s = 1; p.stride = 1; p.pad = 0; p.relu = 1;
  p.howo = 112 * 112;
  p.ktot = 256;
  p.nk = p.ktot / (128 / esz);
  p.tiles_m = n_img * 64;
  p.tiles_n = 1;
  p.M = p.tiles_m * 256;
  p.in_bytes = (long long)n_img * 115 * 115 * 16 * esz;
  p.wt_bytes = 64 * p.ktot * esz;
  p.vec_ok = 1;
  hipStream_t st = (hipStream_t)stream;
  static const bool persistent = [] { const char* e = getenv("VDQN_STEM_PERSISTENT"); return !(e && e[0] == '0'); }();
  if (dtype == VDQN_BF16 && persistent) return vdqn_stem_bf16(t_in, wt, bias, pool, idx, n_img, n_idx_img, st);
  if (dtype == VDQN_F32X3) return launch_igemm<float, 256, 64, 3, 2, true>(p, st);
  return dtype == VDQN_BF16 ? launch_igemm<bf16raw, 256, 64, 3>(p, st) : launch_igemm<float, 256, 64, 3>(p, st);
}

extern "C" int vdqn_stem_conv_pool(const void* t_in, const void* wt, const float* bias, void* pool, void* idx, int32_t n_img, int32_t dtype,
                                   void* stream) {
  return vdqn_stem_conv_pool_n(t_in, wt, bias, pool, idx, n_img, idx ? n_img : 0, dtype, stream);
}
```

video_dqn_amd/csrc/igemm_common.h:

```cpp
#pragma once
#include "common.h"

namespace {


typedef int i32x4 __attribute__((ext_vector_type(4)));
typedef unsigned u32x4 __attribute__((ext_vector_type(4)));

struct IgemmParams {
  const void* in;
  const void* wt;
  const float* bias;
  const void* resid;
  const void* mask;
  void* out;
  float* out_f32;
  float* colsum_part;
  void* pool_out;
  uint8_t* pool_idx;
  int n_idx_img;
  int n_img, hi, wi, ci, pix_stride, ho, wo, co, ldo, r, s, stride, pad, relu;
  int M, howo, ktot, nk, tiles_m, tiles_n;
  int cls_tile0[5], cls_h[2], cls_w[2];
  int cls_interleave;
  long long in_bytes;
  int wt_bytes;
  int vec_ok;
  const void* in2;
  const void* wt2;
  const float* bias2;
  void* out2;
  int co2, ldo2, relu2, ci2, wt2_bytes, tiles_n1;
  int no_lean;
};

constexpr unsigned kOob = 0x80000000u;

template <typename T, int BM, int BN, int MODE, int WN>
__device__ __forceinline__ void igemm_epilogue(const IgemmParams& p, f32x4 (&acc)[4][BN / (16 * WN)], unsigned char* smem, int m0, int n0, int tile_m,
                                               int rows_total, int pix_per_img, int row_w, int cls_ph, int cls_pw, const float* __restrict__ bias,
                                               int tid_override = -1) {
  constexpr int ESZ = (int)sizeof(T);
  constexpr int NF = BN / (16 * WN);
  constexpr int CPL = 4 * NF;
  const int tid = tid_override >= 0 ? tid_override : (int)threadIdx.x;
  const int lane = tid & 63, wave = tid >> 6;
  const int wr = wave / WN, wc = wave % WN;
  const int i16 = lane & 15, g = lane >> 4;
  T* __restrict__ out = (T*)p.out;
  const T* __restrict__ resid = (const T*)p.resid;
  const T* __restrict__ mask = (const T*)p.mask;
  constexpr int V16 = CPL * ESZ / 16;
  const int ncol = n0 + wc * (BN / WN) + g * CPL;
  float cs[CPL];
#pragma unroll
  for (int e = 0; e < CPL; ++e) cs[e] = 0.f;
  if (ncol < p.co) {
    const bool vec = p.vec_ok && (ncol + CPL <= p.co);
    float bv[CPL];
#pragma unroll
    for (int e = 0; e < CPL; ++e) bv[e] = (bias && ncol + e < p.co) ? bias[ncol + e] : 0.f;
    size_t o[4];
    bool okr[4];
#pragma unroll
    for (int f = 0; f < 4; ++f) {
// ... 322 lines not shown
```

video_dqn_amd/csrc/pointwise.hip:

```cpp
#include <math.h>

#include "common.h"

namespace {

template <typename T>
__global__ __launch_bounds__(256) void pack_input_kernel(const void* __restrict__ src, int src_kind, T* __restrict__ dst, int n_img) {
  const int total = n_img * 115 * 115;
  const float mean[3] = {0.485f, 0.456f, 0.406f};
  const float stdv[3] = {0.229f, 0.224f, 0.225f};
  for (int i = blockIdx.x * blockDim.x + threadIdx.x; i < total; i += gridDim.x * blockDim.x) {
    const int n = i / (115 * 115);
    const int rem = i - n * (115 * 115);
    const int y = rem / 115, x = rem - y * 115;
    const int ys = y - 2, xs = x - 2;
    float v[16];
#pragma unroll
    for (int e = 0; e < 16; ++e) v[e] = 0.f;
    if ((unsigned)ys < 112u && (unsigned)xs < 112u) {
#pragma unroll
      for (int bh = 0; bh < 2; ++bh)
#pragma unroll
        for (int bw = 0; bw < 2; ++bw) {
          const int Y = 2 * ys + bh, X = 2 * xs + bw;
#pragma unroll
          for (int c = 0; c < 3; ++c) {
            float val;
            if (src_kind == 0) {
              const uint8_t u = ((const uint8_t*)src)[(((size_t)n * 224 + Y) * 224 + X) * 3 + c];
              val = (((float)u / 255.0f) - mean[c]) / stdv[c];
            } else {
              val = ((const float*)src)[(((size_t)n * 3 + c) * 224 + Y) * 224 + X];
            }
            v[(bh * 2 + bw) * 3 + c] = val;
          }
        }
    }
    T* d = dst + (size_t)i * 16;
    if constexpr (sizeof(T) == 2) {
      uint32_t w[8];
#pragma unroll
      for (int e = 0; e < 8; ++e) w[e] = (uint32_t)f32_to_bf16(v[2 * e]) | ((uint32_t)f32_to_bf16(v[2 * e + 1]) << 16);
      reinterpret_cast<uint4*>(d)[0] = make_uint4(w[0], w[1], w[2], w[3]);
      reinterpret_cast<uint4*>(d)[1] = make_uint4(w[4], w[5], w[6], w[7]);
    } else {
#pragma unroll
      for (int e = 0; e < 4; ++e) reinterpret_cast<float4*>(d)[e] = make_float4(v[4 * e], v[4 * e + 1], v[4 * e + 2], v[4 * e + 3]);
    }
  }
}

constexpr int kPackPairs = 4;
template <typename T>
__global__ __launch_bounds__(256) void pack_input_rows_kernel(const uint8_t* __restrict__ src, T* __restrict__ dst) {
  __shared__ uint4 rows[4][42];
  __shared__ T lut[3][256];
  const int n = blockIdx.y;
  const int tid = threadIdx.x;
  {
    const float mean[3] = {0.485f, 0.456f, 0.406f};
    const float stdv[3] = {0.229f, 0.224f, 0.225f};
#pragma unroll
    for (int c = 0; c < 3; ++c) lut[c][tid] = from_f32<T>((((float)tid / 255.0f) - mean[c]) / stdv[c]);
  }
  const int yy = tid / 115, x = tid - yy * 115;
  for (int pr = 0; pr < kPackPairs; ++pr) {
    const int y0 = 2 * ((int)blockIdx.x * kPackPairs + pr);
    if (y0 >= 115) break;
    const int Y0 = 2 * (y0 - 2);
    __syncthreads();
    if (tid < 168) {
      const int r = tid / 42, c = tid - r * 42, Y = Y0 + r;
      rows[r][c] = ((unsigned)Y < 224u) ? reinterpret_cast<const uint4*>(src + ((size_t)n * 224 + Y) * 672)[c] : make_uint4(0, 0, 0, 0);
    }
    __syncthreads();
    const int y = y0 + yy;
    if (tid >= 230 || y >= 115) continue;
    const int ys = y - 2, xs = x - 2;
    __attribute__((aligned(16))) T v[16];
#pragma unroll
    for (int e = 0; e < 16; ++e) v[e] = from_f32<T>(0.f);
    if ((unsigned)ys < 112u && (unsigned)xs < 112u) {
      const uint8_t* b0 = reinterpret_cast<const uint8_t*>(rows[2 * yy]) + 6 * xs;
      const uint8_t* b1 = reinterpret_cast<const uint8_t*>(rows[2 * yy + 1]) + 6 * xs;
#pragma unroll
      for (int e = 0; e < 6; ++e) {
        v[e] = lut[e % 3][b0[e]];
        v[6 + e] = lut[e % 3][b1[e]];
      }
    }
    T* d = dst + ((size_t)n * 115 * 115 + (size_t)y * 115 + x) * 16;
    constexpr int V16 = (int)(16 * sizeof(T) / 16);
#pragma unroll
    for (int q = 0; q < V16; ++q) reinterpret_cast<uint4*>(d)[q] = reinterpret_cast<const uint4*>(v)[q];
  }
}

template <typename T>
__global__ __launch_bounds__(256) void maxpool_fwd_kernel(const T* __restrict__ in, T* __restrict__ out, uint8_t* __restrict__ idx,
                                                          int n_img, int hi, int wi, int c) {
// ... 325 lines not shown
    const float4 gg = reinterpret_cast<const float4*>(g)[i];
    float4 mm = reinterpret_cast<float4*>(m)[i];
    float4 vv = reinterpret_cast<float4*>(v)[i];
#define VDQN_ADAM1(c)                                              \
  mm.c = beta1 * mm.c + omb1 * gg.c;                     \
  vv.c = beta2 * vv.c + omb2 * gg.c * gg.c;              \
  pp.c = pp.c - step_size * (mm.c / (sqrtf(vv.c) * inv_sqrt_bc2 + eps));
    VDQN_ADAM1(x) VDQN_ADAM1(y) VDQN_ADAM1(z) VDQN_ADAM1(w)
#undef VDQN_ADAM1
    reinterpret_cast<float4*>(p)[i] = pp;
    reinterpret_cast<float4*>(m)[i] = mm;
    reinterpret_cast<float4*>(v)[i] = vv;
  }
  for (long i = (n4 << 2) + (long)blockIdx.x * blockDim.x + threadIdx.x; i < n; i += stride) {
    const float gg = g[i];
    const float mm = beta1 * m[i] + omb1 * gg;
    const float vv = beta2 * v[i] + omb2 * gg * gg;
    m[i] = mm;
    v[i] = vv;
    p[i] = p[i] - step_size * (mm / (sqrtf(vv) * inv_sqrt_bc2 + eps));
  }
}

inline int grid_for(long total, int cap = 8192) {
  long b = (total + 255) / 256;
  if (b > cap) b = cap;
  if (b < 1) b = 1;
  return (int)b;
}

}

extern "C" int vdqn_pack_input(const void* src, int32_t src_kind, void* dst, int32_t n_img, int32_t dtype, void* stream) {
  VDQN_CHECK(src && dst && n_img > 0, "vdqn_pack_input: bad args");
  VDQN_CHECK(src_kind == 0 || src_kind == 1, "vdqn_pack_input: src_kind %d", src_kind);
  VDQN_CHECK(dtype == VDQN_F32 || dtype == VDQN_BF16, "vdqn_pack_input: bad dtype");
  const int g = grid_for((long)n_img * 115 * 115);
  ProfScope ps_("pack_input", 0.0, (double)n_img * (224.0 * 224 * 3 * (src_kind == 0 ? 1 : 4) + 115.0 * 115 * 16 * (dtype == VDQN_BF16 ? 2 : 4)), (hipStream_t)stream);
  if (src_kind == 0 && n_img <= 65535 && (((uintptr_t)src) & 15) == 0) {
    if (dtype == VDQN_BF16) hipLaunchKernelGGL((pack_input_rows_kernel<bf16raw>), dim3((58 + kPackPairs - 1) / kPackPairs, n_img), dim3(256), 0, (hipStream_t)stream, (const uint8_t*)src, (bf16raw*)dst);
    else hipLaunchKernelGGL((pack_input_rows_kernel<float>), dim3((58 + kPackPairs - 1) / kPackPairs, n_img), dim3(256), 0, (hipStream_t)stream, (const uint8_t*)src, (float*)dst);
    VDQN_LAUNCH_CHECK();
    return VDQN_OK;
  }
  if (dtype == VDQN_BF16) hipLaunchKernelGGL((pack_input_kernel<bf16raw>), dim3(g), dim3(256), 0, (hipStream_t)stream, src, src_kind, (bf16raw*)dst, n_img);
  else hipLaunchKernelGGL((pack_input_kernel<float>), dim3(g), dim3(256), 0, (hipStream_t)stream, src, src_kind, (float*)dst, n_img);
  VDQN_LAUNCH_CHECK();
  return VDQN_OK;
}

extern "C" int vdqn_maxpool_fwd(const void* in, void* out, uint8_t* idx, int32_t n_img, int32_t hi, int32_t wi, int32_t c, int32_t dtype,
                                void* stream) {
  VDQN_CHECK(in && out && idx && n_img > 0, "vdqn_maxpool_fwd: bad args");
  VDQN_CHECK(dtype == VDQN_F32 || dtype == VDQN_BF16, "vdqn_maxpool_fwd: bad dtype");
  VDQN_CHECK(c % 8 == 0, "vdqn_maxpool_fwd: channels must be a multiple of 8");
  const int ho = (hi - 1) / 2 + 1, wo = (wi - 1) / 2 + 1;
  const int e16 = dtype == VDQN_BF16 ? 8 : 4;
  const int g = grid_for((long)n_img * ho * wo * (c / e16), 65536);
  ProfScope ps_("maxpool_fwd", 0.0, (double)n_img * c * ((double)hi * wi * (16 / e16) + (double)ho * wo * (16 / e16 + 1)), (hipStream_t)stream);
  if (dtype == VDQN_BF16) hipLaunchKernelGGL((maxpool_fwd_kernel<bf16raw>), dim3(g), dim3(256), 0, (hipStream_t)stream, (const bf16raw*)in, (bf16raw*)out, idx, n_img, hi, wi, c);
  else hipLaunchKernelGGL((maxpool_fwd_kernel<float>), dim3(g), dim3(256), 0, (hipStream_t)stream, (const float*)in, (float*)out, idx, n_img, hi, wi, c);
  VDQN_LAUNCH_CHECK();
  return VDQN_OK;
}

extern "C" int vdqn_maxpool_bwd(const void* gy, const uint8_t* idx, const void* x, void* gx, int32_t n_img, int32_t hi, int32_t wi,
                                int32_t c, int32_t dtype, void* stream) {
  VDQN_CHECK(gy && idx && gx && n_img > 0, "vdqn_maxpool_bwd: bad args");
  VDQN_CHECK(dtype == VDQN_F32 || dtype == VDQN_BF16, "vdqn_maxpool_bwd: bad dtype");
  VDQN_CHECK(c % 8 == 0, "vdqn_maxpool_bwd: channels must be a multiple of 8");
  const int e16 = dtype == VDQN_BF16 ? 8 : 4;
  const int g = grid_for((long)n_img * hi * wi * (c / e16), 65536);
  ProfScope ps_("maxpool_bwd", 0.0, (double)n_img * c * ((x ? 2.0 : 1.0) * hi * wi * (16 / e16) + (double)(hi / 2) * (wi / 2) * (16 / e16 + 1)), (hipStream_t)stream);
  const size_t rows_smem = (size_t)2 * (wi / 2) * c * ((dtype == VDQN_BF16 ? 2 : 4) + 1);
// ... 153 lines not shown
```

video_dqn_amd/csrc/stem.hip:

```cpp
#include "common.h"

namespace {

typedef int i32x4 __attribute__((ext_vector_type(4)));
typedef unsigned u32x4 __attribute__((ext_vector_type(4)));
typedef short i16x2 __attribute__((ext_vector_type(2)));

struct StemParams {
  const bf16raw* t_in;
  const bf16raw* wt;
  const float* bias;
  bf16raw* pool;
  uint8_t* idx;
  int n_img, n_tiles;
  int n_idx_img;
  void* stamps;
};

struct KindArg { static constexpr bool value = true; };
struct KindPlain { static constexpr bool value = false; };

constexpr int kRowPitch = 38 * 16;
constexpr int kWBytes = 3 * 256 * 16;
constexpr int kPatchOff = 2 * kWBytes;
constexpr int kBiasOff = kPatchOff + 256 * 128;
constexpr int kXchOff = kBiasOff + 256;
constexpr int kSmem = kXchOff + 3 * 7 * 128;
constexpr unsigned kOobS = 0x80000000u;

__global__ __launch_bounds__(256, 2) void stem_kernel(const StemParams p) {
  extern __shared__ __attribute__((aligned(16))) unsigned char smem[];
  unsigned char* sW = smem;
  const int tid = threadIdx.x, lane = tid & 63, wave = tid >> 6;
  const int i16 = lane & 15, g = lane >> 4;
  const uint32_t lds_base = (uint32_t)(uintptr_t)(__attribute__((address_space(3))) unsigned char*)smem;
  const int wave_u = __builtin_amdgcn_readfirstlane(wave);
  const uint32_t lds_wave = lds_base + (uint32_t)wave_u * 1024u;
  constexpr int PSTR = 256 * 16;
  constexpr long long kImgBytes = 115ll * 115 * 16 * 2;

  auto load_weights = [&](u32x4 (&fb)[4][2][4]) {
    const unsigned char* wrow = reinterpret_cast<const unsigned char*>(p.wt) + (size_t)((lane & 15) >> 2) * 16 * 512 + (size_t)(lane & 3) * 512;
    asm volatile("" : "+v"(wrow));
#pragma unroll
    for (int kr = 0; kr < 4; ++kr)
#pragma unroll
      for (int h = 0; h < 2; ++h)
#pragma unroll
        for (int j = 0; j < 4; ++j)
          fb[kr][h][j] = *reinterpret_cast<const u32x4*>(wrow + (size_t)j * 4 * 512 + kr * 128 + ((lane >> 4) + 4 * h) * 16);
  };
  auto issue_window = [&](int t, int buf) {
    int tid_w = tid;
    asm volatile("" : "+v"(tid_w));
    const int img = t >> 6, ty = (t >> 3) & 7, tx = t & 7;
    const int y0 = 14 * ty - 1, x0 = 14 * tx - 1;
    const unsigned long long a_ptr = (unsigned long long)((const unsigned char*)p.t_in + (long long)img * kImgBytes);
    const i32x4 rs_a = {__builtin_amdgcn_readfirstlane((int)(unsigned)a_ptr), __builtin_amdgcn_readfirstlane((int)((a_ptr >> 32) & 0xffff)), (int)kImgBytes, 0x00020000};
    uint32_t vw[3];
#pragma unroll
    for (int i = 0; i < 3; ++i) {
      const int sl = i * 256 + tid_w;
      const int row = (sl * 1725) >> 16;
      const int pc = sl - row * 38;
      const int lc = pc ^ ((pc >> 4) & 1);
      const int sy = y0 + row;
      const bool ok = row < 19 && (unsigned)sy < 115u;
      vw[i] = ok ? (uint32_t)((sy * 115 + x0) * 32 + lc * 16) : kOobS;
    }
    const uint32_t l0 = lds_wave + (uint32_t)(buf * kWBytes);
    asm volatile(
        "s_nop 4\n\t"
        "s_mov_b32 m0, %3\n\ts_nop 0\n\tbuffer_load_dwordx4 %0, %4, 0 offen lds\n\t"
        "s_add_u32 m0, %3, %5\n\ts_nop 0\n\tbuffer_load_dwordx4 %1, %4, 0 offen lds\n\t"
        "s_add_u32 m0, %3, %6\n\ts_nop 0\n\tbuffer_load_dwordx4 %2, %4, 0 offen lds"
        ::"v"(vw[0]), "v"(vw[1]), "v"(vw[2]), "s"(l0), "s"(rs_a), "n"(PSTR), "n"(2 * PSTR)
        : "memory", "scc");
  };
  if (tid < 64) reinterpret_cast<float*>(smem + kBiasOff)[tid] = p.bias[tid];

  const int lc0 = 2 * i16 + g, lc1 = lc0 + 4;
  const int coff0 = (lc0 ^ ((lc0 >> 4) & 1)) << 4, coff1 = (lc1 ^ ((lc1 >> 4) & 1)) << 4;

#ifdef VDQN_STEM_LDS_POOL
  const int Ta = p.n_tiles;
#else
  const int Ta = p.n_idx_img * 64;
#endif
  const int Tn = p.n_tiles - Ta, G = (int)gridDim.x, b0 = (int)blockIdx.x;
  const int ka = b0 < Ta ? (Ta - b0 + G - 1) / G : 0;
  const int kn = b0 < Tn ? (Tn - b0 + G - 1) / G : 0;
  auto tile_at = [&](int k) {
    if (k < ka) return (int)xcd_remap((uint32_t)(b0 + k * G), (uint32_t)Ta);
    if (k < ka + kn) return Ta + (int)xcd_remap((uint32_t)(b0 + (k - ka) * G), (uint32_t)Tn);
    return -1;
  };
  auto tile = [&](auto kind, const int k, const u32x4 (&fb)[4][2][4]) {
    constexpr bool ARG = decltype(kind)::value;
    const int buf = k & 1;
    const int tl = tile_at(k);
    asm volatile("s_waitcnt vmcnt(0)" ::: "memory");
    __builtin_amdgcn_s_barrier();
#ifdef VDQN_STAMP
    const int st_k = k;
    unsigned long long* st_row = (p.stamps && st_k < 16) ? reinterpret_cast<unsigned long long*>(p.stamps) + ((size_t)blockIdx.x * 16 + st_k) * 8 : nullptr;
    if (st_row && tid == 0) { st_row[0] = __builtin_amdgcn_s_memtime(); st_row[5] = __builtin_amdgcn_s_getreg(4 | (31 << 11)); }
#endif
    {
      const int nx = tile_at(k + 1);
      if (nx >= 0) issue_window(nx, buf ^ 1);
    }
#ifdef VDQN_STAMP
    if (st_row && tid == 0) st_row[1] = __builtin_amdgcn_s_memtime();
#endif

    f32x4 acc[4][4];
#pragma unroll
    for (int f = 0; f < 4; ++f)
#pragma unroll
      for (int j = 0; j < 4; ++j) acc[f][j] = (f32x4){0.f, 0.f, 0.f, 0.f};
    const unsigned char* a_rd = sW + buf * kWBytes + (4 * wave) * kRowPitch;
#if !(defined(VDQN_STEM_PROBE) && (VDQN_STEM_PROBE & 1))
    u32x4 fa[2][2];
    fa[0][0] = *reinterpret_cast<const u32x4*>(a_rd + coff0);
    fa[0][1] = *reinterpret_cast<const u32x4*>(a_rd + coff1);
#pragma unroll
    for (int R = 0; R < 7; ++R) {
// ... 174 lines not shown
        }
      uint32_t key[8];
#pragma unroll
      for (int e = 0; e < 8; ++e) key[e] = 0u;
#pragma unroll
      for (int kh = 0; kh < 3; ++kh)
#pragma unroll
        for (int kw = 0; kw < 3; ++kw) {
          const uint32_t m = (kh == 0 ? row0 : 0x7fff0u) & (kw == 0 ? col0 : 0x7fff0u);
          const uint32_t tag = (kh == 0 || kw == 0) ? ((m >> 4) & (uint32_t)(8 - (kh * 3 + kw))) : (uint32_t)(8 - (kh * 3 + kw));
          const uint32_t w4[4] = {v[kh * 3 + kw].x, v[kh * 3 + kw].y, v[kh * 3 + kw].z, v[kh * 3 + kw].w};
#pragma unroll
          for (int q = 0; q < 4; ++q) {
            key[2 * q] = max(key[2 * q], ((w4[q] << 4) & m) | tag);
            key[2 * q + 1] = max(key[2 * q + 1], ((w4[q] >> 12) & m) | tag);
          }
        }
      uint4 ov;
      uint2 bi;
      ov.x = (key[0] >> 4) | ((key[1] << 12) & 0xffff0000u);
      ov.y = (key[2] >> 4) | ((key[3] << 12) & 0xffff0000u);
      ov.z = (key[4] >> 4) | ((key[5] << 12) & 0xffff0000u);
      ov.w = (key[6] >> 4) | ((key[7] << 12) & 0xffff0000u);
      bi.x = (8u - (key[0] & 15u)) | ((8u - (key[1] & 15u)) << 8) | ((8u - (key[2] & 15u)) << 16) | ((8u - (key[3] & 15u)) << 24);
      bi.y = (8u - (key[4] & 15u)) | ((8u - (key[5] & 15u)) << 8) | ((8u - (key[6] & 15u)) << 16) | ((8u - (key[7] & 15u)) << 24);
      *reinterpret_cast<uint4*>(p.pool + o) = ov;
      *reinterpret_cast<uint2*>(p.idx + o) = bi;
    }
#ifdef VDQN_STAMP
    if (st_row && tid == 0) st_row[4] = __builtin_amdgcn_s_memtime();
#endif
  };
  if (ka + kn > 0) issue_window(tile_at(0), 0);
  if (ka > 0) {
    u32x4 fb[4][2][4];
    load_weights(fb);
    for (int k = 0; k < ka; ++k) tile(KindArg{}, k, fb);
  }
  if (kn > 0) {
    u32x4 fb[4][2][4];
    load_weights(fb);
    for (int k = ka; k < ka + kn; ++k) tile(KindPlain{}, k, fb);
  }
}

}

int vdqn_stem_bf16(const void* t_in, const void* wt, const float* bias, void* pool, void* idx, int n_img, int n_idx_img, hipStream_t st) {
  vdqn_ensure_dyn_smem(reinterpret_cast<const void*>(&stem_kernel), (size_t)kSmem);
  const int n_cu = vdqn_num_cus();
  StemParams p;
  p.t_in = (const bf16raw*)t_in; p.wt = (const bf16raw*)wt; p.bias = bias; p.pool = (bf16raw*)pool; p.idx = (uint8_t*)idx;
  p.n_img = n_img;
  p.n_idx_img = idx ? n_idx_img : 0;
  p.n_tiles = n_img * 64;
  p.stamps = nullptr;
#ifdef VDQN_STAMP
  { extern void* g_stamp_buffer; p.stamps = g_stamp_buffer; }
#endif
  const int grid = p.n_tiles < 2 * n_cu ? p.n_tiles : 2 * n_cu;
  vdqn_prof_begin("stem_conv_pool<bf16>", 2.0 * n_img * 112 * 112 * 64 * 147,
                  2.0 * ((double)n_img * 115 * 115 * 16 + 64.0 * 256 + (double)n_img * 56 * 56 * 64) + (double)p.n_idx_img * 56 * 56 * 64, st);
  hipLaunchKernelGGL(stem_kernel, dim3(grid), dim3(256), kSmem, st, p);
  vdqn_prof_end(st);
  VDQN_LAUNCH_CHECK();
  return VDQN_OK;
}
```

video_dqn_amd/csrc/win9.hip:

```cpp
#include <stdlib.h>

#include "igemm_common.h"

namespace {

constexpr int kU_WtTile = 128 * 128;
constexpr int kU_WinBase = 2 * kU_WtTile;

template <int BM>
struct Win9Geom {
  static constexpr int NT = 2 * BM;
  static constexpr int RPP = NT / 8;
  static constexpr int PSTR = RPP * 128;
  static constexpr int WinRows = BM == 128 ? 192 : 320;
  static constexpr int WinStride = WinRows * 128;
  static constexpr int WPass = WinRows / RPP;
  static constexpr int BPass = 128 / RPP;
  static constexpr int Smem = kU_WinBase + 2 * WinStride;
};

template <int MODE, int BM>
__global__ __launch_bounds__(2 * BM, 2) void win9u_kernel(const IgemmParams p, const int wrows, const FastDiv d_wo, const FastDiv d_howo, const uint32_t total_tiles, void* stamps) {
  static_assert(MODE == 0 || MODE == 1, "window kernel: forward or stride-1 data gradient");
  static_assert(BM == 128 || BM == 256, "tile rows");
  using T = bf16raw;
  using G = Win9Geom<BM>;
  constexpr int BN = 128, WN = 2;
  constexpr int NF = BN / (16 * WN);
  constexpr int CPL = 4 * NF;
  constexpr int PSTR = G::PSTR;
  constexpr int kU_WinStride = G::WinStride;
  extern __shared__ __attribute__((aligned(16))) unsigned char smem[];

  const int tid = threadIdx.x;
  const int lane = tid & 63, wave = tid >> 6;
  const uint32_t xcd = blockIdx.x & 7u;
  const uint32_t tq = total_tiles >> 3, tr = total_tiles & 7u;
  const uint32_t x_first = xcd < tr ? xcd * (tq + 1) : tr * (tq + 1) + (xcd - tr) * tq;
  const uint32_t x_count = tq + (xcd < tr ? 1u : 0u);
  const uint32_t x_blocks = (gridDim.x >> 3) + (xcd < (gridDim.x & 7u) ? 1u : 0u);
  uint32_t lt = blockIdx.x >> 3;
  int tile_n, tile_m, n0, m0;
  const int m_end = p.M;
  if (lt >= x_count) return;
  tile_n = (int)((x_first + lt) % (uint32_t)p.tiles_n);
  tile_m = (int)((x_first + lt) / (uint32_t)p.tiles_n);
  n0 = tile_n * BN;
  m0 = tile_m * BM;
  const int W = p.wo, H = p.ho, rows_total = p.M;
  const int lrow = tid >> 3;
  const int lchunk_a = (tid & 7) ^ (lrow & 7);
  const int lchunk_b = (tid & 7) ^ ((((lrow / CPL) & 1) << 2) | (lrow & 3));

  const unsigned long long a_ptr = (unsigned long long)p.in;
  const unsigned long long b_ptr = (unsigned long long)p.wt;
  const i32x4 rs_a = {__builtin_amdgcn_readfirstlane((int)(unsigned)a_ptr), __builtin_amdgcn_readfirstlane((int)((a_ptr >> 32) & 0xffff)),
                      __builtin_amdgcn_readfirstlane((int)p.in_bytes), 0x00020000};
  const i32x4 rs_b = {__builtin_amdgcn_readfirstlane((int)(unsigned)b_ptr), __builtin_amdgcn_readfirstlane((int)((b_ptr >> 32) & 0xffff)),
                       __builtin_amdgcn_readfirstlane(p.wt_bytes), 0x00020000};

  const int pixB = p.pix_stride * 2;
  const int need = BM + 2 * W + 2;
  int q0 = m0 - W - 1 + lrow;
  const uint32_t a_lane = (uint32_t)(lchunk_a * 16);
  uint32_t b_off0 = (uint32_t)(n0 + lrow) * (uint32_t)(p.ktot * 2) + (uint32_t)(lchunk_b * 16);
  const int b_row32 = G::RPP * p.ktot * 2;

  const uint32_t lds_base = (uint32_t)(uintptr_t)(__attribute__((address_space(3))) unsigned char*)smem;
  const int wave_u = __builtin_amdgcn_readfirstlane(wave);
  const uint32_t lds_wave = lds_base + (uint32_t)wave_u * (8 * 128);

#define VDQN_DMA4(V0, V1, V2, V3, LDS, RSRC, SOFF)                                                                  \
  asm volatile(                                                                                                     \
      "s_mov_b32 m0, %4\n\ts_nop 0\n\tbuffer_load_dwordx4 %0, %5, %6 offen lds\n\t"                                \
      "s_add_u32 m0, %4, %7\n\ts_nop 0\n\tbuffer_load_dwordx4 %1, %5, %6 offen lds\n\t"                            \
      "s_add_u32 m0, %4, %8\n\ts_nop 0\n\tbuffer_load_dwordx4 %2, %5, %6 offen lds\n\t"                            \
      "s_add_u32 m0, %4, %9\n\ts_nop 0\n\tbuffer_load_dwordx4 %3, %5, %6 offen lds"                                 \
// ... 149 lines not shown
          \
                                                                                             \
    if constexpr (ci_ == 2) {                                                                                            \
      VDQN_ISSUE_B(cur_, ti_ * tap_k + so_nx, b_nx, rs_b)                                                               \
      if constexpr (ti_ == 0) VDQN_ISSUE_AW(0, so_nx, q_nx)                                                              \
    } else {                                                                                                             \
      VDQN_ISSUE_B(cur_, ti_ * tap_k + (cc2 + ci_) * 128, b_off0, rs_b)                                                  \
      if constexpr (ti_ == 0) VDQN_ISSUE_AW(ci_ & 1, (cc2 + ci_) * 128, q0)                                              \
    }                                                                                                                    \
    VDQN_ST(st_issue)                                                                                                    \
    __builtin_amdgcn_sched_barrier(0);                                                                                   \
    VDQN_LOAD_FRAGS(nxt_, tl_, cl_ & 1, nxt_)  \
    VDQN_MFMA_ALL(cur_)                                                                                                  \
    VDQN_INTERLEAVE(8 + 2 * NF)                                                                                          \
    __builtin_amdgcn_sched_barrier(0);                                                                                   \
  }


  VDQN_ISSUE_B(0, 0, b_off0, rs_b)
  VDQN_ISSUE_AW(0, 0, q0)
  VDQN_ISSUE_B(1, tap_k, b_off0, rs_b)
  asm volatile("s_waitcnt vmcnt(0)" ::: "memory");
  __builtin_amdgcn_s_barrier();
#ifdef VDQN_STAMP
  st_t = __builtin_amdgcn_s_memtime();
  unsigned long long st_loop_end = 0;
#endif
  for (;;) {
#pragma unroll
    for (int f = 0; f < 4; ++f)
#pragma unroll
      for (int j = 0; j < NF; ++j) acc[f][j] = (f32x4){0.f, 0.f, 0.f, 0.f};
    VDQN_LOAD_FRAGS(0, 0, 0, 0)
    const uint32_t lt_nx = lt + x_blocks;
    const bool has_nx = lt_nx < x_count;
    const int tn_nx = !has_nx ? tile_n : (int)((x_first + lt_nx) % (uint32_t)p.tiles_n);
    const int tm_nx = !has_nx ? tile_m : (int)((x_first + lt_nx) / (uint32_t)p.tiles_n);
    const int m0_nx = tm_nx * BM;
    const int q0_t = m0_nx - W - 1 + lrow;
    const uint32_t b_t = (uint32_t)(tn_nx * BN + lrow) * (uint32_t)(p.ktot * 2) + (uint32_t)(lchunk_b * 16);
#pragma clang loop unroll(disable)
    for (int it = 0; it < n_it; ++it) {
      const int cc2 = 2 * it;
      const bool last_it = has_nx && it == n_it - 1;
      const int so_nx = last_it ? 0 : (cc2 + 2) * 128;
      const int q_nx = last_it ? q0_t : q0;
      const uint32_t b_nx = last_it ? b_t : b_off0;
      VDQN_USTEP(0) VDQN_USTEP(1) VDQN_USTEP(2) VDQN_USTEP(3) VDQN_USTEP(4) VDQN_USTEP(5)
      VDQN_USTEP(6) VDQN_USTEP(7) VDQN_USTEP(8) VDQN_USTEP(9) VDQN_USTEP(10) VDQN_USTEP(11)
      VDQN_USTEP(12) VDQN_USTEP(13) VDQN_USTEP(14) VDQN_USTEP(15) VDQN_USTEP(16) VDQN_USTEP(17)
    }
    VDQN_ST(st_comp)
    asm volatile("s_waitcnt vmcnt(0)" ::: "memory");
    __builtin_amdgcn_s_barrier();
#ifdef VDQN_STAMP
    st_loop_end = __builtin_amdgcn_s_memtime();
#endif
    if (MODE == 0 && lean) lean_epilogue_128<WN>(le, acc, m0, n0, m_end, tid);
    else if (MODE == 1 && lean_d)
      lean_epilogue_dgrad_128<WN, BM / 64>(led, acc, reinterpret_cast<float*>(smem + kU_WinBase + kU_WinStride), m0, n0, tile_m, m_end, tid);
    else igemm_epilogue<T, BM, BN, MODE, WN>(p, acc, smem + kU_WinBase + kU_WinStride, m0, n0, tile_m, m_end, p.howo, W, 0, 0,
                                             p.bias);
    if (!has_nx) break;
    lt = lt_nx;
    tile_n = tn_nx; tile_m = tm_nx;
    n0 = tile_n * BN; m0 = m0_nx;
    q0 = q0_t;
// ... 72 lines not shown
```

video_dqn_amd/csrc/win9d.hip:

```cpp
#include <stdlib.h>

#include "igemm_common.h"

namespace {

constexpr int kD_WinRows = 160;
constexpr int kD_WinStride = kD_WinRows * 128;
constexpr int kD_WPass = kD_WinRows / 32;

struct DTap { int tap, dy, dx; };
__host__ __device__ constexpr int d_len(int kind) { return kind == 0 ? 4 : (kind <= 2 ? 2 : 1); }
__host__ __device__ constexpr DTap d_tap(int kind, int i) {
  constexpr DTap t0[4] = {{0, 1, 1}, {2, 1, 0}, {6, 0, 1}, {8, 0, 0}};
  constexpr DTap t1[2] = {{1, 1, 0}, {7, 0, 0}};
  constexpr DTap t2[2] = {{3, 0, 1}, {5, 0, 0}};
  return kind == 0 ? t0[i & 3] : kind == 1 ? t1[i & 1] : kind == 2 ? t2[i & 1] : kind == 3 ? DTap{4, 0, 0} : DTap{0, 0, 0};
}

template <int NF>
struct DGeom {
  static constexpr int BN = 32 * NF;
  static constexpr int WtTile = BN * 128;
  static constexpr int WinBase = 2 * WtTile;
  static constexpr int Scratch = WinBase + 2 * kD_WinStride;
  static constexpr int Smem = Scratch + 2 * BN * 4;
};

template <int NF, bool SIB, bool SPLIT>
__global__ __launch_bounds__(256, 2) void win9d_kernel(const IgemmParams p, const FastDiv d_wo, const FastDiv d_howo, const uint32_t total_tiles, const int tiles_n,
                                                       const uint32_t n_a) {
  using T = bf16raw;
  using G = DGeom<NF>;
  constexpr int BM = 128, BN = G::BN, WN = 2, CPL = 4 * NF;
  constexpr int PSTR = 32 * 128;
  constexpr int BPASS = BN / 32;
  extern __shared__ __attribute__((aligned(16))) unsigned char smem[];
  const int tid = threadIdx.x, lane = tid & 63, wave = tid >> 6;
  const uint32_t xcd = blockIdx.x & 7u;
  const uint32_t tq = total_tiles >> 3, tr = total_tiles & 7u;
  const uint32_t x_first = xcd < tr ? xcd * (tq + 1) : tr * (tq + 1) + (xcd - tr) * tq;
  const uint32_t x_count = tq + (xcd < tr ? 1u : 0u);
  const uint32_t x_blocks = (gridDim.x >> 3) + (xcd < (gridDim.x & 7u) ? 1u : 0u);
  uint32_t lt = blockIdx.x >> 3, lt_step = x_blocks;
  int grp = 0;
  if constexpr (SPLIT) {
    grp = lt < n_a ? 0 : (lt < 2u * n_a ? 1 : 2);
    grp = __builtin_amdgcn_readfirstlane(grp);
    lt_step = grp == 2 ? x_blocks - 2u * n_a : n_a;
    lt -= (uint32_t)grp * n_a;
  }
  if (lt >= x_count) return;
  int tile_n = (int)((x_first + lt) % (uint32_t)tiles_n), tile_m = (int)((x_first + lt) / (uint32_t)tiles_n);
  int n0 = tile_n * BN, m0 = tile_m * BM;
  const int Wo = p.wi, Ho = p.hi, Wi = p.wo;
  const int rows_total = p.n_img * Ho * Wo;
  const int lrow = tid >> 3;
  const int lchunk_a = (tid & 7) ^ (lrow & 7);
  const int lchunk_b = (tid & 7) ^ ((((lrow / CPL) & 1) << 2) | (lrow & 3));
  const int cpk = p.ci / 64;
  const int tap_k = p.ci * 2;
  const int b_row32 = 32 * 9 * tap_k;
  const int b2_row32 = 32 * tap_k;
  const int pixB = tap_k;
  const int need = BM + Wo + 2;

  const unsigned long long a_ptr = (unsigned long long)p.in, b_ptr = (unsigned long long)p.wt;
  const unsigned long long a2_ptr = (unsigned long long)(SIB ? p.in2 : p.in), b2_ptr = (unsigned long long)(SIB ? p.wt2 : p.wt);
  const i32x4 rs_a = {__builtin_amdgcn_readfirstlane((int)(unsigned)a_ptr), __builtin_amdgcn_readfirstlane((int)((a_ptr >> 32) & 0xffff)),
                      __builtin_amdgcn_readfirstlane((int)p.in_bytes), 0x00020000};
  const i32x4 rs_a2 = {__builtin_amdgcn_readfirstlane((int)(unsigned)a2_ptr), __builtin_amdgcn_readfirstlane((int)((a2_ptr >> 32) & 0xffff)),
                       __builtin_amdgcn_readfirstlane((int)p.in_bytes), 0x00020000};
  const i32x4 rs_b = {__builtin_amdgcn_readfirstlane((int)(unsigned)b_ptr), __builtin_amdgcn_readfirstlane((int)((b_ptr >> 32) & 0xffff)),
                      __builtin_amdgcn_readfirstlane(p.wt_bytes), 0x00020000};
  const i32x4 rs_b2 = {__builtin_amdgcn_readfirstlane((int)(unsigned)b2_ptr), __builtin_amdgcn_readfirstlane((int)((b2_ptr >> 32) & 0xffff)),
                       __builtin_amdgcn_readfirstlane(SIB ? p.wt2_bytes : p.wt_bytes), 0x00020000};

  const uint32_t lds_base = (uint32_t)(uintptr_t)(__attribute__((address_space(3))) unsigned char*)smem;
  const int wave_u = __builtin_amdgcn_readfirstlane(wave);
  const uint32_t lds_wave = lds_base + (uint32_t)wave_u * (8 * 128);
  const uint32_t a_lane = (uint32_t)(lchunk_a * 16);
  const uint32_t b_off0 = (uint32_t)lrow * (uint32_t)(9 * tap_k) + (uint32_t)(lchunk_b * 16);
  const uint32_t b2_off0 = (uint32_t)lrow * (uint32_t)tap_k + (uint32_t)(lchunk_b * 16);
  int b_n0 = n0 * 9 * tap_k, b2_n0 = n0 * tap_k;

// ... 329 lines not shown
```

video_dqn_amd/csrc/win9s.hip:

```cpp
#include <stdlib.h>

#include "igemm_common.h"

namespace {

constexpr int kS_WtTile = 128 * 128;
constexpr int kS_WinRows = 160;
constexpr int kS_WinStride = kS_WinRows * 128;
constexpr int kS_WinBase = 2 * kS_WtTile;
constexpr int kS_Smem = kS_WinBase + 2 * kS_WinStride;
constexpr int kS_WPass = kS_WinRows / 32;
constexpr int kSP_BiasCols = 512;
constexpr int kSP_Smem = kS_Smem + 2 * kSP_BiasCols * 4;

struct S2Step { int tap, a, b, dy, dx, wbuf; };
__host__ __device__ constexpr S2Step s2_step(int s) {
  constexpr S2Step tab[9] = {{0, 1, 1, -1, -1, 0}, {2, 1, 1, -1, 0, 0}, {6, 1, 1, 0, -1, 0}, {8, 1, 1, 0, 0, 0},
                             {1, 1, 0, -1, 0, 1},  {7, 1, 0, 0, 0, 1},
                             {3, 0, 1, 0, -1, 0},  {5, 0, 1, 0, 0, 0},
                             {4, 0, 0, 0, 0, 1}};
  return tab[s];
}
__host__ __device__ constexpr int s2_window_issued_at(int s) { return s == 2 ? 4 : s == 4 ? 6 : s == 6 ? 8 : s == 7 ? 9 : -1; }

__global__ __launch_bounds__(256, 2) void win9s_kernel(const IgemmParams p, const FastDiv d_wo, const FastDiv d_howo) {
  using T = bf16raw;
  constexpr int BM = 128, BN = 128, WN = 2, NF = 4, CPL = 16;
  constexpr int PSTR = 32 * 128;
  extern __shared__ __attribute__((aligned(16))) unsigned char smem[];
  const int tid = threadIdx.x, lane = tid & 63, wave = tid >> 6;
  const uint32_t lb = xcd_remap(blockIdx.x, gridDim.x);
  const int tile_n = (int)(lb % (uint32_t)p.tiles_n), tile_m = (int)(lb / (uint32_t)p.tiles_n);
  const int n0 = tile_n * BN, m0 = tile_m * BM;
  const int Wo = p.wo, rows_total = p.M;
  const int lrow = tid >> 3;
  const int lchunk_a = (tid & 7) ^ (lrow & 7);
  const int lchunk_b = (tid & 7) ^ ((((lrow / CPL) & 1) << 2) | (lrow & 3));

  const unsigned long long a_ptr = (unsigned long long)p.in, b_ptr = (unsigned long long)p.wt;
  const i32x4 rs_a = {__builtin_amdgcn_readfirstlane((int)(unsigned)a_ptr), __builtin_amdgcn_readfirstlane((int)((a_ptr >> 32) & 0xffff)),
                      __builtin_amdgcn_readfirstlane((int)p.in_bytes), 0x00020000};
  const i32x4 rs_b = {__builtin_amdgcn_readfirstlane((int)(unsigned)b_ptr), __builtin_amdgcn_readfirstlane((int)((b_ptr >> 32) & 0xffff)),
                      __builtin_amdgcn_readfirstlane(p.wt_bytes), 0x00020000};

  const int pixB = p.pix_stride * 2;
  const int need = BM + Wo + 1;
  uint32_t a_row[kS_WPass];
#pragma unroll
  for (int i = 0; i < kS_WPass; ++i) {
    const int j = lrow + 32 * i;
    const int q = m0 - Wo - 1 + j;
    const bool ok = j < need && (unsigned)q < (unsigned)rows_total;
    const uint32_t qq = ok ? (uint32_t)q : 0u;
    const uint32_t img = fastdiv(qq, d_howo), rem = qq - img * d_howo.div;
    const uint32_t y = fastdiv(rem, d_wo), x = rem - y * d_wo.div;
    a_row[i] = ok ? ((img * (uint32_t)p.hi + 2u * y) * (uint32_t)p.wi + 2u * x) * (uint32_t)pixB + (uint32_t)(lchunk_a * 16) : kOob;
  }
  const uint32_t b_off0 = (uint32_t)(n0 + lrow) * (uint32_t)(p.ktot * 2) + (uint32_t)(lchunk_b * 16);
  const int b_row32 = 32 * p.ktot * 2;

  const uint32_t lds_base = (uint32_t)(uintptr_t)(__attribute__((address_space(3))) unsigned char*)smem;
  const int wave_u = __builtin_amdgcn_readfirstlane(wave);
  const uint32_t lds_wave = lds_base + (uint32_t)wave_u * (8 * 128);

// ... 128 lines not shown
  asm volatile("s_waitcnt vmcnt(0) lgkmcnt(0)" ::: "memory");
  __builtin_amdgcn_s_barrier();
  igemm_epilogue<T, BM, BN, 0, WN>(p, acc, smem + kS_WinBase, m0, n0, tile_m, rows_total, p.howo, Wo, 0, 0, p.bias);
#undef VDQN_S_USTEP
#undef VDQN_S_LOAD_FRAGS
#undef VDQN_S_MFMA_ALL
#undef VDQN_S_ISSUE_AW
#undef VDQN_S_ISSUE_B
}


template <int CPK, bool SIB>
__global__ __launch_bounds__(256, 2) void win9sp_kernel(const IgemmParams p, const FastDiv d_wo, const FastDiv d_howo, const uint32_t total_tiles, const int tiles_n,
                                                       void* stamps) {
  static_assert(CPK == 1 || CPK == 2 || CPK == 4, "channel chunks of layer2.0 / layer3.0 / layer4.0");
  static_assert(SIB || CPK != 1, "nine steps per tile: odd");
  using T = bf16raw;
  constexpr int BM = 128, BN = 128, WN = 2, NF = 4, CPL = 16;
  constexpr int PSTR = 32 * 128;
  const int tap_k = p.ci * 2;
  const int b_row32 = 32 * 9 * tap_k;
  const int b2_row32 = 32 * tap_k;
  const int pixB = tap_k;
#define VDQN_SCONST(V) ({ int r_; asm volatile("s_mov_b32 %0, %1" : "=s"(r_) : "n"(V)); r_; })
  extern __shared__ __attribute__((aligned(16))) unsigned char smem[];
  const int tid = threadIdx.x, lane = tid & 63, wave = tid >> 6;
  const uint32_t xcd = blockIdx.x & 7u;
  const uint32_t tq = total_tiles >> 3, tr = total_tiles & 7u;
  const uint32_t x_first = xcd < tr ? xcd * (tq + 1) : tr * (tq + 1) + (xcd - tr) * tq;
  const uint32_t x_count = tq + (xcd < tr ? 1u : 0u);
  const uint32_t x_blocks = (gridDim.x >> 3) + (xcd < (gridDim.x & 7u) ? 1u : 0u);
  uint32_t lt = blockIdx.x >> 3;
  if (lt >= x_count) return;
  int tile_n = (int)((x_first + lt) % (uint32_t)tiles_n), tile_m = (int)((x_first + lt) / (uint32_t)tiles_n);
  int n0 = tile_n * BN, m0 = tile_m * BM;
  const int Wo = p.wo, rows_total = p.M;
  const int lrow = tid >> 3;
  const int lchunk_a = (tid & 7) ^ (lrow & 7);
  const int lchunk_b = (tid & 7) ^ ((((lrow / CPL) & 1) << 2) | (lrow & 3));

  const unsigned long long a_ptr = (unsigned long long)p.in, b_ptr = (unsigned long long)p.wt, b2_ptr = (unsigned long long)(SIB ? p.wt2 : p.wt);
  const i32x4 rs_a = {__builtin_amdgcn_readfirstlane((int)(unsigned)a_ptr), __builtin_amdgcn_readfirstlane((int)((a_ptr >> 32) & 0xffff)),
                      __builtin_amdgcn_readfirstlane((int)p.in_bytes), 0x00020000};
  const i32x4 rs_b = {__builtin_amdgcn_readfirstlane((int)(unsigned)b_ptr), __builtin_amdgcn_readfirstlane((int)((b_ptr >> 32) & 0xffff)),
                      __builtin_amdgcn_readfirstlane(p.wt_bytes), 0x00020000};
  const i32x4 rs_b2 = {__builtin_amdgcn_readfirstlane((int)(unsigned)b2_ptr), __builtin_amdgcn_readfirstlane((int)((b2_ptr >> 32) & 0xffff)),
                       __builtin_amdgcn_readfirstlane(SIB ? p.wt2_bytes : p.wt_bytes), 0x00020000};

  const int need = BM + Wo + 1;
  auto plane_rows = [&](int m_base, uint32_t (&ar)[kS_WPass]) {
#pragma unroll
    for (int i = 0; i < kS_WPass; ++i) {
      const int j = lrow + 32 * i;
      const int q = m_base - Wo - 1 + j;
      const bool ok = j < need && (unsigned)q < (unsigned)rows_total;
      const uint32_t qq = ok ? (uint32_t)q : 0u;
      const uint32_t img = fastdiv(qq, d_howo), rem = qq - img * d_howo.div;
      const uint32_t y = fastdiv(rem, d_wo), x = rem - y * d_wo.div;
      ar[i] = ok ? ((img * (uint32_t)p.hi + 2u * y) * (uint32_t)p.wi + 2u * x) * (uint32_t)pixB + (uint32_t)(lchunk_a * 16) : kOob;
    }
  };
  uint32_t a_row[kS_WPass], a_row_n[kS_WPass];
  plane_rows(m0, a_row);
  uint32_t b_off0 = (uint32_t)(n0 + lrow) * (uint32_t)(9 * tap_k) + (uint32_t)(lchunk_b * 16);
  uint32_t b2_off0 = (uint32_t)(n0 + lrow) * (uint32_t)tap_k + (uint32_t)(lchunk_b * 16);

// ... 210 lines not shown
        for (int r = 0; r < 4; ++r) {
          float v = acc[f][j][r] + bv[j * 4 + r];
          if (relu) v = fmaxf(v, 0.f);
          ov[j * 4 + r] = f32_to_bf16(v);
        }
      __builtin_amdgcn_raw_buffer_store_b128(reinterpret_cast<const u32x4*>(ov)[0], rsrc, (int)off, 0, 0);
      __builtin_amdgcn_raw_buffer_store_b128(reinterpret_cast<const u32x4*>(ov)[1], rsrc, (int)off + 16, 0, 0);
    }
  };

  IgemmParams q = p;
  if constexpr (SIB) {
    q.bias = p.bias2; q.out = p.out2; q.relu = p.relu2; q.co = p.co2; q.ldo = p.ldo2;
    q.resid = nullptr; q.mask = nullptr; q.out_f32 = nullptr; q.colsum_part = nullptr;
  }

  VDQN_P_ISSUE_B(0, b_off0, rs_b, s2_step(0).tap * tap_k, b_row32)
  VDQN_P_ISSUE_AW(0, a_row, so_p11)
  VDQN_P_ISSUE_B(1, b_off0, rs_b, s2_step(1).tap * tap_k, b_row32)
  asm volatile("s_waitcnt vmcnt(0)" ::: "memory");
  __builtin_amdgcn_s_barrier();
#ifdef VDQN_STAMP
  st_t = __builtin_amdgcn_s_memtime();
#endif
  for (;;) {
#ifdef VDQN_STAMP
    ++st_tiles;
#endif
#pragma unroll
    for (int f = 0; f < 4; ++f)
#pragma unroll
      for (int j = 0; j < NF; ++j) acc[f][j] = (f32x4){0.f, 0.f, 0.f, 0.f};
    VDQN_P_LOAD_STEP(0, 0, 0)
    const uint32_t lt_nx = lt + x_blocks;
    const bool has_nx = lt_nx < x_count;
    const int tn_nx = has_nx ? (int)((x_first + lt_nx) % (uint32_t)tiles_n) : tile_n;
    const int tm_nx = has_nx ? (int)((x_first + lt_nx) / (uint32_t)tiles_n) : tile_m;
    plane_rows(tm_nx * BM, a_row_n);
    const uint32_t b_t = (uint32_t)(tn_nx * BN + lrow) * (uint32_t)(9 * tap_k) + (uint32_t)(lchunk_b * 16);
    VDQN_PST(st_top)
    if constexpr (CPK == 1) {
      VDQN_P_USTEP(0, 0, false, true) VDQN_P_USTEP(1, 0, false, true) VDQN_P_USTEP(2, 0, false, true) VDQN_P_USTEP(3, 0, false, true)
      VDQN_P_USTEP(4, 0, false, true) VDQN_P_USTEP(5, 0, false, true) VDQN_P_USTEP(6, 0, false, true) VDQN_P_USTEP(7, 0, false, true)
      VDQN_P_USTEP(8, 0, false, true)
    } else if constexpr (CPK == 2) {
      VDQN_P_PAIR(0, true)
    } else {
      VDQN_P_PAIR(0, false)
      VDQN_P_PAIR(2, true)
    }
    VDQN_PST(st_comp)
    asm volatile("s_waitcnt vmcnt(0) lgkmcnt(0)" ::: "memory");
    __builtin_amdgcn_s_barrier();
    VDQN_PST(st_bnd)
    if (lean) lean_epilogue(r_out, p.ldo, p.relu, sBias);
    else igemm_epilogue<T, BM, BN, 0, WN>(p, acc, smem + kS_WinBase, m0, n0, tile_m, rows_total, p.howo, Wo, 0, 0, p.bias);
    VDQN_PST(st_epi1)
    if constexpr (SIB) {
#pragma unroll
      for (int f = 0; f < 4; ++f)
#pragma unroll
        for (int j = 0; j < NF; ++j) acc[f][j] = (f32x4){0.f, 0.f, 0.f, 0.f};
      VDQN_P_LOAD_FRAGS((9 * CPK) & 1, CPK == 1 ? 1 : 0, 0, 0, (9 * CPK) & 1)
      VDQN_P_DSTEP(0)
      if constexpr (CPK >= 2) VDQN_P_DSTEP(1)
      if constexpr (CPK >= 4) { VDQN_P_DSTEP(2) VDQN_P_DSTEP(3) }
      VDQN_PST(st_comp)
// ... 89 lines not shown
```

video_dqn_amd/ops.py:

```python
from __future__ import annotations

import ctypes as C
from typing import Optional

import torch

from . import _lib
from .engine import _ptr, _stream, require_gpu

TORCH_DTYPE = {_lib.VDQN_F32: torch.float32, _lib.VDQN_BF16: torch.bfloat16}


def dtype_code(t: torch.Tensor) -> int:
    if t.dtype == torch.float32:
        return _lib.VDQN_F32
    if t.dtype == torch.bfloat16:
        return _lib.VDQN_BF16
    raise TypeError(f"unsupported activation dtype {t.dtype}")


def gemm_dtype_code(t: torch.Tensor, precision: Optional[str]) -> int:
    code = dtype_code(t)
    if precision is None:
        return code
    if precision != "bf16x3":
        raise ValueError(f"unknown precision {precision!r} (None or 'bf16x3')")
    if code != _lib.VDQN_F32:
        raise TypeError(f"precision='bf16x3' splits f32 operands; got {t.dtype}")
    return _lib.VDQN_F32X3


def conv2d(x: torch.Tensor, wt: torch.Tensor, *, ho: int, wo: int, co: int, r: int, s: int, stride: int, pad: int,
           bias: Optional[torch.Tensor] = None, resid: Optional[torch.Tensor] = None, mask: Optional[torch.Tensor] = None,
           relu: bool = False, mode: int = 0, pix_stride: Optional[int] = None, ci: Optional[int] = None,
           want_f32: bool = False, ldo: Optional[int] = None, want_colsum: bool = False,
           wt2: Optional[torch.Tensor] = None, bias2: Optional[torch.Tensor] = None, co2: int = 0, relu2: bool = False,
           in2: Optional[torch.Tensor] = None, precision: Optional[str] = None):
    lib = _lib.load()
    require_gpu()
    n, hi, wi, cx = x.shape
    ci = cx if ci is None else ci
    pix_stride = cx if pix_stride is None else pix_stride
    ldo = co if ldo is None else ldo
    out = torch.empty((n, ho, wo, ldo), dtype=x.dtype, device=x.device)
    out_f32 = torch.empty((n, ho, wo, ldo), dtype=torch.float32, device=x.device) if want_f32 else None
    a = _lib.ConvArgs()
    a.in_, a.wt, a.bias, a.resid, a.mask = _ptr(x), _ptr(wt), _ptr(bias), _ptr(resid), _ptr(mask)
    a.out, a.out_f32 = _ptr(out), _ptr(out_f32)
    a.n_img, a.hi, a.wi, a.ci, a.pix_stride = n, hi, wi, ci, pix_stride
    a.ho, a.wo, a.co, a.ldo = ho, wo, co, ldo
    a.r, a.s, a.stride, a.pad = r, s, stride, pad
    a.mode, a.relu, a.dtype = mode, int(relu), gemm_dtype_code(x, precision)
    out2 = None
    if wt2 is not None and mode == 0:
        out2 = torch.empty((n, ho, wo, co2), dtype=x.dtype, device=x.device)
        a.wt2, a.bias2, a.out2, a.co2, a.ldo2, a.relu2 = _ptr(wt2), _ptr(bias2), _ptr(out2), co2, co2, int(relu2)
    elif wt2 is not None:
        a.wt2, a.in2, a.ci2 = _ptr(wt2), _ptr(in2), in2.shape[-1]
    part = None
    if want_colsum:
        a.colsum_part = 16
        rows = lib.vdqn_conv2d_colsum_rows(C.byref(a))
        if mode == 1 and stride == 2:
            n_tiles = sum((n * hc * wc + rows - 1) // rows for hc in ((ho + 1) // 2, ho // 2) for wc in ((wo + 1) // 2, wo // 2))
        else:
            n_tiles = (n * ho * wo + rows - 1) // rows
        part = torch.empty((n_tiles, ldo), dtype=torch.float32, device=x.device)
    a.colsum_part = _ptr(part)
    _lib.check(lib.vdqn_conv2d(C.byref(a), _stream()), "vdqn_conv2d")
    if out2 is not None:
        return out, out2
    if want_colsum:
        return out, part
    return (out, out_f32) if want_f32 else out


def conv2d_wgrad(gy: torch.Tensor, x: torch.Tensor, *, co: int, r: int, s: int, stride: int, pad: int,
                 ci: Optional[int] = None, pix_stride: Optional[int] = None, splitk: int = 0, want_dbias: bool = True,
                 deterministic: bool = False, poison_workspace: bool = False, precision: Optional[str] = None):
    lib = _lib.load()
    n, ho, wo, ldg = gy.shape
    _, hi, wi, cx = x.shape
    ci = cx if ci is None else ci
    pix_stride = cx if pix_stride is None else pix_stride
    co_pad = (co + 63) // 64 * 64
    dw = torch.zeros((co_pad, r, s, ci), dtype=torch.float32, device=x.device)
    db = torch.zeros((co_pad,), dtype=torch.float32, device=x.device) if want_dbias else None
    a = _lib.WgradArgs()
    a.gy, a.x, a.dw, a.dbias = _ptr(gy), _ptr(x), _ptr(dw), _ptr(db)
    a.n_img, a.hi, a.wi, a.ci, a.pix_stride = n, hi, wi, ci, pix_stride
    a.ho, a.wo, a.co, a.ldg = ho, wo, co, ldg
    a.r, a.s, a.stride, a.pad = r, s, stride, pad
    a.splitk, a.dtype = splitk, gemm_dtype_code(x, precision)
    ws = None
    if deterministic:
        nbytes = lib.vdqn_conv2d_wgrad_workspace_bytes(C.byref(a))
        if nbytes < 0:
            _lib.check(-1, "vdqn_conv2d_wgrad_workspace_bytes")
        ws = torch.empty(max(nbytes, 16), dtype=torch.uint8, device=x.device)
        if poison_workspace:
            ws.fill_(0xFF)
        a.workspace, a.workspace_bytes = _ptr(ws), nbytes
    _lib.check(lib.vdqn_conv2d_wgrad(C.byref(a), _stream()), "vdqn_conv2d_wgrad")
    return (dw, db) if want_dbias else dw


def pack_input(src: torch.Tensor, src_kind: int, n_img: int, dtype: torch.dtype) -> torch.Tensor:
    lib = _lib.load()
    dst = torch.empty((n_img, 115, 115, 16), dtype=dtype, device=src.device)
    _lib.check(lib.vdqn_pack_input(_ptr(src), src_kind, _ptr(dst), n_img, dtype_code(dst), _stream()), "vdqn_pack_input")
    return dst


def maxpool_fwd(x: torch.Tensor):
    lib = _lib.load()
    n, hi, wi, c = x.shape
    ho, wo = (hi - 1) // 2 + 1, (wi - 1) // 2 + 1
    out = torch.empty((n, ho, wo, c), dtype=x.dtype, device=x.device)
    idx = torch.empty((n, ho, wo, c), dtype=torch.uint8, device=x.device)
    _lib.check(lib.vdqn_maxpool_fwd(_ptr(x), _ptr(out), _ptr(idx), n, hi, wi, c, dtype_code(x), _stream()), "vdqn_maxpool_fwd")
    return out, idx


def maxpool_bwd(gy: torch.Tensor, idx: torch.Tensor, x: Optional[torch.Tensor] = None, out_hw=None) -> torch.Tensor:
    lib = _lib.load()
    if x is not None:
        n, hi, wi, c = x.shape
        gx = torch.empty_like(x)
    else:
        n, _, _, c = gy.shape
        hi, wi = out_hw
        gx = torch.empty((n, hi, wi, c), dtype=gy.dtype, device=gy.device)
    _lib.check(lib.vdqn_maxpool_bwd(_ptr(gy), _ptr(idx), _ptr(x), _ptr(gx), n, hi, wi, c, dtype_code(gy), _stream()), "vdqn_maxpool_bwd")
    return gx


def stem_wgrad_pool(g_pool: torch.Tensor, idx: torch.Tensor, t_in: torch.Tensor, deterministic: bool = False) -> torch.Tensor:
    lib = _lib.load()
    n = g_pool.shape[0]
    dw = torch.zeros((64, 4, 1, 64), dtype=torch.float32, device=g_pool.device)
    ws, nbytes = None, 0
    if deterministic:
        nbytes = lib.vdqn_stem_wgrad_pool_workspace_bytes(n)
# ... 67 lines not shown
    return torch.full((max(nbytes, 16),), 0xFF, dtype=torch.uint8, device=y.device), nbytes


def bn_train_bwd(g: torch.Tensor, y: torch.Tensor, work: torch.Tensor, *, num_frames=1, imgs_per_half=None, deterministic=False):
    lib = _lib.load()
    n, h, w, c = y.shape
    iph = n if imgs_per_half is None else imgs_per_half
    dy = torch.empty_like(y)
    dgamma = torch.empty(c, dtype=torch.float32, device=y.device)
    dbeta = torch.empty(c, dtype=torch.float32, device=y.device)
    ws, nbytes = _bn_workspace(lib, y, n, h * w, c, num_frames, iph, deterministic)
    _lib.check(lib.vdqn_bn_train_bwd(_ptr(g), _ptr(y), _ptr(dy), _ptr(work), _ptr(dgamma), _ptr(dbeta), n, h * w, c, num_frames, iph,
                                     dtype_code(y), _ptr(ws), nbytes, _stream()), "vdqn_bn_train_bwd")
    return dy, dgamma, dbeta


def avgpool_fwd(x: torch.Tensor) -> torch.Tensor:
    lib = _lib.load()
    n, h, w, c = x.shape
    out = torch.empty((n, c), dtype=x.dtype, device=x.device)
    _lib.check(lib.vdqn_avgpool_fwd(_ptr(x), _ptr(out), n, h * w, c, dtype_code(x), _stream()), "vdqn_avgpool_fwd")
    return out


def avgpool_bwd(g: torch.Tensor, x: torch.Tensor) -> torch.Tensor:
    lib = _lib.load()
    n, h, w, c = x.shape
    gx = torch.empty_like(x)
    _lib.check(lib.vdqn_avgpool_bwd(_ptr(g), _ptr(x), _ptr(gx), n, h * w, c, dtype_code(x), _stream()), "vdqn_avgpool_bwd")
    return gx


def stem_conv_pool(t_in: torch.Tensor, wt: torch.Tensor, bias: torch.Tensor, want_idx: bool = True, n_idx: int = None,
                   precision: Optional[str] = None):
    lib = _lib.load()
    n = t_in.shape[0]
    dt = gemm_dtype_code(t_in, precision)
    pool = torch.empty((n, 56, 56, 64), dtype=t_in.dtype, device=t_in.device)
    if n_idx is not None:
        idx = torch.zeros((n, 56, 56, 64), dtype=torch.uint8, device=t_in.device)
        _lib.check(lib.vdqn_stem_conv_pool_n(_ptr(t_in), _ptr(wt), _ptr(bias), _ptr(pool), _ptr(idx), n, int(n_idx), dt, _stream()),
                   "vdqn_stem_conv_pool_n")
        return pool, idx
    idx = torch.empty((n, 56, 56, 64), dtype=torch.uint8, device=t_in.device) if want_idx else None
    _lib.check(lib.vdqn_stem_conv_pool(_ptr(t_in), _ptr(wt), _ptr(bias), _ptr(pool), _ptr(idx) if want_idx else None, n, dt, _stream()),
               "vdqn_stem_conv_pool")
    return pool, idx
```

Before: 42650 tuples/s.

## Alternate conv tile traversal direction between consecutive layers for cache reuse

Adds a tile_order flag to the conv, dgrad, stem and pack kernels that reverses the order in which each XCD walks its tiles. The forward and backward chains alternate the direction from one layer to the next, so the tiles a layer writes last are the first ones the next layer reads, while they may still be in L2/MALL. Alternation is on by default through an environment mask and can be overridden by a debug hook. It adds a little index arithmetic in each kernel and a second template instantiation of the stem kernel.

```diff
diff --git a/include/vdqn.h b/include/vdqn.h
--- a/include/vdqn.h
+++ b/include/vdqn.h
@@ -49,6 +49,7 @@
   const float* bias2;
   void* out2;
   int32_t co2, ldo2, relu2, ci2;
+  int32_t tile_order;
 } vdqn_conv_args;
 int vdqn_conv2d(const vdqn_conv_args* a, void* stream);
 int32_t vdqn_conv2d_colsum_rows(const vdqn_conv_args* a);
@@ -71,6 +72,8 @@
 int vdqn_host_gather(void* dst, const void* const* src, int64_t n, int64_t bytes_each, int32_t threads);
 
 int vdqn_pack_input(const void* src, int32_t src_kind, void* dst, int32_t n_img, int32_t dtype, void* stream);
+int vdqn_pack_input_ord(const void* src, int32_t src_kind, void* dst, int32_t n_img, int32_t dtype, int32_t tile_order, void* stream);
+int32_t vdqn_tile_walk(int32_t bid, int32_t n_tiles, int32_t tile_order);
 
 int vdqn_maxpool_fwd(const void* in, void* out, uint8_t* idx, int32_t n_img, int32_t hi, int32_t wi, int32_t c,
                      int32_t dtype, void* stream);
@@ -106,6 +109,8 @@
                         int32_t dtype, void* stream);
 int vdqn_stem_conv_pool_n(const void* t_in, const void* wt, const float* bias, void* pool, void* idx, int32_t n_img,
                           int32_t n_idx_img, int32_t dtype, void* stream);
+int vdqn_stem_conv_pool_ord(const void* t_in, const void* wt, const float* bias, void* pool, void* idx, int32_t n_img,
+                            int32_t n_idx_img, int32_t dtype, int32_t tile_order, void* stream);
 
 int vdqn_stem_wgrad_pool(const void* g_pool, const uint8_t* idx, const void* t_in, float* dw, int32_t n_img, void* workspace,
                          int64_t workspace_bytes, void* stream);
@@ -232,6 +237,8 @@
                           void* stream);
 int vdqn_pack_input_aug(const void* src, void* dst, int32_t n_img, int32_t frames_per_sample, const int32_t* params,
                         int32_t n_params, int32_t dtype, void* stream);
+int vdqn_pack_input_aug_ord(const void* src, void* dst, int32_t n_img, int32_t frames_per_sample, const int32_t* params,
+                            int32_t n_params, int32_t dtype, int32_t tile_order, void* stream);
 int vdqn_net_set_augment(vdqn_net* net, const int32_t* params);
 
 #define VDQN_COMM_UID_BYTES 128
diff --git a/video_dqn_amd/_lib.py b/video_dqn_amd/_lib.py
--- a/video_dqn_amd/_lib.py
+++ b/video_dqn_amd/_lib.py
@@ -23,7 +23,7 @@
                 ("mode", c_i32), ("relu", c_i32), ("dtype", c_i32),
                 ("in2", c_vp), ("wt2", c_vp), ("bias2", c_vp), ("out2", c_vp),
                 ("co2", c_i32), ("ldo2", c_i32), ("relu2", c_i32), ("ci2", c_i32),
-]
+                ("tile_order", c_i32)]
 
 
 class WgradArgs(C.Structure):
@@ -81,10 +81,13 @@
     "vdqn_conv2d_wgrad": (C.c_int, [C.POINTER(WgradArgs), c_vp]),
     "vdqn_conv2d_wgrad_workspace_bytes": (c_i64, [C.POINTER(WgradArgs)]),
     "vdqn_pack_input": (C.c_int, [c_vp, c_i32, c_vp, c_i32, c_i32, c_vp]),
+    "vdqn_pack_input_ord": (C.c_int, [c_vp, c_i32, c_vp, c_i32, c_i32, c_i32, c_vp]),
+    "vdqn_tile_walk": (c_i32, [c_i32, c_i32, c_i32]),
     "vdqn_maxpool_fwd": (C.c_int, [c_vp, c_vp, c_vp, c_i32, c_i32, c_i32, c_i32, c_i32, c_vp]),
     "vdqn_maxpool_bwd": (C.c_int, [c_vp, c_vp, c_vp, c_vp, c_i32, c_i32, c_i32, c_i32, c_i32, c_vp]),
     "vdqn_stem_conv_pool": (C.c_int, [c_vp, c_vp, c_vp, c_vp, c_vp, c_i32, c_i32, c_vp]),
     "vdqn_stem_conv_pool_n": (C.c_int, [c_vp, c_vp, c_vp, c_vp, c_vp, c_i32, c_i32, c_i32, c_vp]),
+    "vdqn_stem_conv_pool_ord": (C.c_int, [c_vp, c_vp, c_vp, c_vp, c_vp, c_i32, c_i32, c_i32, c_i32, c_vp]),
     "vdqn_td_loss": (C.c_int, [C.POINTER(TdArgs), c_vp]),
     "vdqn_gt_loss": (C.c_int, [c_vp, c_vp, c_vp, c_vp, c_vp, c_vp, c_i32, c_i32, c_i32, c_i32, c_f32, c_i32, c_i32, c_vp]),
     "vdqn_adam": (C.c_int, [c_vp, c_vp, c_vp, c_vp, c_i64, c_i32, C.c_double, C.c_double, C.c_double, C.c_double, c_vp]),
@@ -138,6 +141,7 @@
     "vdqn_aug_draw": (C.c_int, [C.c_uint64, C.c_uint64, c_i32, c_i32, c_i32, c_i32, c_i32, c_vp, c_vp]),
     "vdqn_aug_swap_actions": (C.c_int, [c_vp, c_vp, c_i32, c_i32, c_i32, c_vp, c_vp]),
     "vdqn_pack_input_aug": (C.c_int, [c_vp, c_vp, c_i32, c_i32, c_vp, c_i32, c_i32, c_vp]),
+    "vdqn_pack_input_aug_ord": (C.c_int, [c_vp, c_vp, c_i32, c_i32, c_vp, c_i32, c_i32, c_i32, c_vp]),
     "vdqn_net_set_augment": (C.c_int, [c_vp, c_vp]),
 }
 COMM_UID_BYTES = 128
diff --git a/video_dqn_amd/augment.py b/video_dqn_amd/augment.py
--- a/video_dqn_amd/augment.py
+++ b/video_dqn_amd/augment.py
@@ -33,15 +33,16 @@
     return out
 
 
-def pack_input_aug(src: torch.Tensor, params: torch.Tensor, frames_per_sample: int, dtype: torch.dtype) -> torch.Tensor:
+def pack_input_aug(src: torch.Tensor, params: torch.Tensor, frames_per_sample: int, dtype: torch.dtype, tile_order: int = 0) -> torch.Tensor:
     if src.dtype != torch.uint8 or not src.is_contiguous() or params.dtype != torch.int32 or not params.is_contiguous():
         raise _lib.VdqnError("pack_input_aug: src must be contiguous uint8 NHWC frames and params contiguous int32 [*][4]")
     n_img = src.numel() // (224 * 224 * 3)
     with torch.cuda.device(src.device):
         dst = torch.empty((n_img, 115, 115, 16), dtype=dtype, device=src.device)
         code = _lib.VDQN_BF16 if dtype == torch.bfloat16 else _lib.VDQN_F32
-        _lib.check(_lib.load().vdqn_pack_input_aug(src.data_ptr(), dst.data_ptr(), n_img, frames_per_sample, params.data_ptr(),
-                                                   params.numel() // 4, code, torch.cuda.current_stream().cuda_stream), "vdqn_pack_input_aug")
+        _lib.check(_lib.load().vdqn_pack_input_aug_ord(src.data_ptr(), dst.data_ptr(), n_img, frames_per_sample, params.data_ptr(),
+                                                       params.numel() // 4, code, int(tile_order), torch.cuda.current_stream().cuda_stream),
+                   "vdqn_pack_input_aug")
     return dst
 
 
diff --git a/video_dqn_amd/csrc/augment.hip b/video_dqn_amd/csrc/augment.hip
--- a/video_dqn_amd/csrc/augment.hip
+++ b/video_dqn_amd/csrc/augment.hip
@@ -38,10 +38,11 @@
 
 template <typename T>
 __global__ __launch_bounds__(256) void pack_input_aug_kernel(const uint8_t* __restrict__ src, T* __restrict__ dst, int frames_per_sample,
-                                                             const int4* __restrict__ params, int n_params) {
+                                                             const int4* __restrict__ params, int n_params, const uint32_t reverse) {
   __shared__ uint4 rows[4][42];
   __shared__ T lut[3][256];
-  const int n = blockIdx.y;
+  const int n = (int)walk_pos(0u, gridDim.y, blockIdx.y, reverse);
+  const int bx = (int)walk_pos(0u, gridDim.x, blockIdx.x, reverse);
   const int tid = threadIdx.x;
   {
     const float mean[3] = {0.485f, 0.456f, 0.406f};
@@ -65,7 +66,7 @@
     o1 = 3 * X1;
   }
   for (int pr = 0; pr < kPackPairs; ++pr) {
-    const int y0 = 2 * ((int)blockIdx.x * kPackPairs + pr);
+    const int y0 = 2 * (bx * kPackPairs + pr);
     if (y0 >= 115) break;
     const int Y0 = 2 * (y0 - 2);
     const bool inside = (unsigned)Y0 < 224u;
@@ -134,7 +135,13 @@
 
 extern "C" int vdqn_pack_input_aug(const void* src, void* dst, int32_t n_img, int32_t frames_per_sample, const int32_t* params,
                                    int32_t n_params, int32_t dtype, void* stream) {
+  return vdqn_pack_input_aug_ord(src, dst, n_img, frames_per_sample, params, n_params, dtype, 0, stream);
+}
+
+extern "C" int vdqn_pack_input_aug_ord(const void* src, void* dst, int32_t n_img, int32_t frames_per_sample, const int32_t* params,
+                                       int32_t n_params, int32_t dtype, int32_t tile_order, void* stream) {
   VDQN_CHECK(src && dst && params, "vdqn_pack_input_aug: null arg");
+  VDQN_CHECK(tile_order == 0 || tile_order == 1, "vdqn_pack_input_aug: tile_order %d", tile_order);
   VDQN_CHECK(n_img > 0 && frames_per_sample > 0 && n_params > 0, "vdqn_pack_input_aug: n_img %d, frames_per_sample %d, n_params %d must be > 0",
              n_img, frames_per_sample, n_params);
   VDQN_CHECK(dtype == VDQN_F32 || dtype == VDQN_BF16, "vdqn_pack_input_aug: bad dtype");
@@ -143,10 +150,10 @@
   const dim3 grid((58 + kPackPairs - 1) / kPackPairs, n_img);
   if (dtype == VDQN_BF16)
     hipLaunchKernelGGL((pack_input_aug_kernel<bf16raw>), grid, dim3(256), 0, (hipStream_t)stream, (const uint8_t*)src, (bf16raw*)dst,
-                       (int)frames_per_sample, (const int4*)params, (int)n_params);
+                       (int)frames_per_sample, (const int4*)params, (int)n_params, (uint32_t)tile_order);
   else
     hipLaunchKernelGGL((pack_input_aug_kernel<float>), grid, dim3(256), 0, (hipStream_t)stream, (const uint8_t*)src, (float*)dst,
-                       (int)frames_per_sample, (const int4*)params, (int)n_params);
+                       (int)frames_per_sample, (const int4*)params, (int)n_params, (uint32_t)tile_order);
   VDQN_LAUNCH_CHECK();
   return VDQN_OK;
 }
diff --git a/video_dqn_amd/csrc/common.h b/video_dqn_amd/csrc/common.h
--- a/video_dqn_amd/csrc/common.h
+++ b/video_dqn_amd/csrc/common.h
@@ -61,6 +61,15 @@
   return (x < r ? x * (q + 1) : r * (q + 1) + (x - r) * q) + i;
 }
 
+__host__ __device__ __forceinline__ uint32_t walk_pos(uint32_t first, uint32_t count, uint32_t i, uint32_t reverse) {
+  const uint32_t m = 0u - reverse;
+  return first + (i ^ m) + (count & m);
+}
+__host__ __device__ __forceinline__ uint32_t tile_walk(uint32_t bid, uint32_t nblk, uint32_t reverse) {
+  const uint32_t q = nblk >> 3, r = nblk & 7, x = bid & 7, i = bid >> 3;
+  return walk_pos(x < r ? x * (q + 1) : r * (q + 1) + (x - r) * q, q + (x < r ? 1u : 0u), i, reverse);
+}
+
 void vdqn_set_error(const char* fmt, ...);
 
 void vdqn_ensure_dyn_smem(const void* kernel, size_t bytes);
diff --git a/video_dqn_amd/csrc/engine.hip b/video_dqn_amd/csrc/engine.hip
--- a/video_dqn_amd/csrc/engine.hip
+++ b/video_dqn_amd/csrc/engine.hip
@@ -17,6 +17,10 @@
 }
 extern "C" const char* vdqn_last_error(void) { return g_err; }
 extern "C" int vdqn_abi_version(void) { return 15; }
+extern "C" int32_t vdqn_tile_walk(int32_t bid, int32_t n_tiles, int32_t tile_order) {
+  if (n_tiles <= 0 || bid < 0 || bid >= n_tiles || (tile_order != 0 && tile_order != 1)) return -1;
+  return (int32_t)tile_walk((uint32_t)bid, (uint32_t)n_tiles, (uint32_t)tile_order);
+}
 extern "C" int32_t vdqn_abi_struct_size(int32_t which) {
   switch (which) {
     case 0: return (int32_t)sizeof(vdqn_conv_args);
@@ -108,6 +112,7 @@
   int l_b_conv1[8], l_b_conv2[8], l_b_ds[8];
   BnSync bn_sync = {nullptr, nullptr, nullptr, 1};
   int wgrad_rr = 0;
+  int dgrad_k = 0;
   int overlap = 1;
   int bwd_samples = 0;
   const float* sample_w = nullptr;
@@ -189,7 +194,19 @@
 extern "C" void vdqn_debug_set_wgrad_streams(int v) { g_wgrad_streams_override = v; }
 static int g_stem_wgrad_main_override = -1;
 extern "C" void vdqn_debug_set_stem_wgrad_main(int v) { g_stem_wgrad_main_override = v; }
+static int g_tile_alternate_override = -1;
+extern "C" void vdqn_debug_set_tile_alternate(int v) { g_tile_alternate_override = v; }
 namespace {
+int tile_alternate_mask() {
+  static const int env = [] { const char* e = getenv("VDQN_TILE_ALTERNATE"); return e ? atoi(e) & 3 : 3; }();
+  return g_tile_alternate_override >= 0 ? g_tile_alternate_override & 3 : env;
+}
+struct TileChain {
+  bool on;
+  int k;
+  int next() { return on ? (k++ & 1) : 0; }
+  int same() const { return on ? ((k - 1) & 1) : 0; }
+};
 hipStream_t wgrad_stream(vdqn_net* net, hipStream_t main) {
   if (!wgrad_two_streams(net)) return fork_side(net, main);
   net->wgrad_rr ^= 1;
@@ -845,7 +862,7 @@
 bool fuse_ds_fwd(int dtype) { return (fuse_ds_mask() & 2) != 0 && (dtype == VDQN_BF16 || (fuse_ds_mask() & 4) != 0); }
 
 int run_conv(const vdqn_net* net, const Layer& L, const unsigned char* packed, const void* in, void* out, int n_units, const void* resid,
-             int relu, float* out_f32, hipStream_t st, const Layer* sib = nullptr, void* sib_out = nullptr) {
+             int relu, float* out_f32, hipStream_t st, const Layer* sib = nullptr, void* sib_out = nullptr, int tile_order = 0) {
   vdqn_conv_args a;
   memset(&a, 0, sizeof(a));
   a.in = in;
@@ -861,6 +878,7 @@
   a.stride = L.kind == K_CONV1_S2D ? 1 : L.stride;
   a.pad = L.kind == K_CONV1_S2D ? 0 : L.pad;
   a.mode = 0; a.relu = relu; a.dtype = net->gemm_dtype;
+  a.tile_order = tile_order;
   g_prof_alg_flops = 2.0 * n_units * L.ho * L.wo * (double)L.co * L.ci * L.r * L.s;
   if (sib) {
     a.wt2 = packed + sib->wf_off;
@@ -875,7 +893,7 @@
 
 int run_dgrad(const vdqn_net* net, const Layer& L, const unsigned char* packed, const void* gy, void* gx, int n_units, const void* resid,
               const void* mask, hipStream_t st, void* colsum_part = nullptr, const Layer* sib = nullptr, const void* sib_gy = nullptr,
-              int* part_rows = nullptr) {
+              int* part_rows = nullptr, int tile_order = 0) {
   vdqn_conv_args a;
   memset(&a, 0, sizeof(a));
   a.in = gy;
@@ -889,6 +907,7 @@
   a.ho = L.hi; a.wo = L.wi; a.co = L.k_ci; a.ldo = L.k_ci;
   a.r = L.k_r; a.s = L.k_s; a.stride = L.stride; a.pad = L.pad;
   a.mode = 1; a.relu = 0; a.dtype = net->gemm_dtype;
+  a.tile_order = tile_order;
   g_prof_alg_flops = 2.0 * n_units * L.ho * L.wo * (double)L.co * L.ci * L.r * L.s;
   if (sib) {
     a.in2 = sib_gy;
@@ -948,13 +967,14 @@
   const int dt = net->cfg.dtype;
   static const bool stem_noidx = [] { const char* e = getenv("VDQN_STEM_NOIDX"); return !(e && e[0] == '0'); }();
   const int n_idx = (grad_samples >= 0 && stem_noidx) ? (grad_samples * net->cfg.num_frames < n ? grad_samples * net->cfg.num_frames : n) : n;
+  TileChain tc = {(tile_alternate_mask() & 1) != 0, 1};
   if (A.c1 >= 0) {
     RC(run_conv(net, net->layers[net->l_conv1], packed, t_in, acts + A.c1, n, nullptr, 1, nullptr, st));
     RC(vdqn_maxpool_fwd(acts + A.c1, acts + A.pool, acts + A.idx, n, 112, 112, 64, dt, st));
   } else {
     const Layer& L1 = net->layers[net->l_conv1];
     prof_layer(L1, n);
-    RC(vdqn_stem_conv_pool_n(t_in, packed + L1.wf_off, reinterpret_cast<const float*>(packed + L1.bias_off), acts + A.pool, acts + A.idx, n, n_idx, net->gemm_dtype, st));
+    RC(vdqn_stem_conv_pool_ord(t_in, packed + L1.wf_off, reinterpret_cast<const float*>(packed + L1.bias_off), acts + A.pool, acts + A.idx, n, n_idx, net->gemm_dtype, 0, st));
   }
   const unsigned char* x = acts + A.pool;
   for (int b = 0; b < 8; ++b) {
@@ -962,16 +982,16 @@
     const Layer& c2 = net->layers[net->l_b_conv2[b]];
     const void* identity = x;
     if (net->l_b_ds[b] >= 0 && fuse_ds_fwd(dt)) {
-      RC(run_conv(net, c1, packed, x, acts + A.h[b], n, nullptr, 1, nullptr, st, &net->layers[net->l_b_ds[b]], acts + A.ds[b]));
+      RC(run_conv(net, c1, packed, x, acts + A.h[b], n, nullptr, 1, nullptr, st, &net->layers[net->l_b_ds[b]], acts + A.ds[b], tc.next()));
       identity = acts + A.ds[b];
     } else {
-      RC(run_conv(net, c1, packed, x, acts + A.h[b], n, nullptr, 1, nullptr, st));
+      RC(run_conv(net, c1, packed, x, acts + A.h[b], n, nullptr, 1, nullptr, st, nullptr, nullptr, tc.next()));
       if (net->l_b_ds[b] >= 0) {
-        RC(run_conv(net, net->layers[net->l_b_ds[b]], packed, x, acts + A.ds[b], n, nullptr, 0, nullptr, st));
+        RC(run_conv(net, net->layers[net->l_b_ds[b]], packed, x, acts + A.ds[b], n, nullptr, 0, nullptr, st, nullptr, nullptr, tc.same()));
         identity = acts + A.ds[b];
       }
     }
-    RC(run_conv(net, c2, packed, acts + A.h[b], acts + A.o[b], n, identity, 1, nullptr, st));
+    RC(run_conv(net, c2, packed, acts + A.h[b], acts + A.o[b], n, identity, 1, nullptr, st, nullptr, nullptr, tc.next()));
     x = acts + A.o[b];
   }
   if (trunk_only) return VDQN_OK;
@@ -980,10 +1000,10 @@
     RC(run_conv(net, net->layers[net->l_top4], packed, acts + A.avg, acts + A.q, n_samples, nullptr, 0, reinterpret_cast<float*>(acts + A.qf), st));
     return VDQN_OK;
   }
-  RC(run_conv(net, net->layers[net->l_f8], packed, x, acts + A.f8, n, nullptr, 1, nullptr, st));
-  RC(run_conv(net, net->layers[net->l_top0], packed, acts + A.f8, acts + A.l0, n_samples, nullptr, 1, nullptr, st));
-  RC(run_conv(net, net->layers[net->l_top2], packed, acts + A.l0, acts + A.l1, n_samples, nullptr, 1, nullptr, st));
-  RC(run_conv(net, net->layers[net->l_top4], packed, acts + A.l1, acts + A.q, n_samples, nullptr, 0, reinterpret_cast<float*>(acts + A.qf), st));
+  RC(run_conv(net, net->layers[net->l_f8], packed, x, acts + A.f8, n, nullptr, 1, nullptr, st, nullptr, nullptr, tc.next()));
+  RC(run_conv(net, net->layers[net->l_top0], packed, acts + A.f8, acts + A.l0, n_samples, nullptr, 1, nullptr, st, nullptr, nullptr, tc.next()));
+  RC(run_conv(net, net->layers[net->l_top2], packed, acts + A.l0, acts + A.l1, n_samples, nullptr, 1, nullptr, st, nullptr, nullptr, tc.next()));
+  RC(run_conv(net, net->layers[net->l_top4], packed, acts + A.l1, acts + A.q, n_samples, nullptr, 0, reinterpret_cast<float*>(acts + A.qf), st, nullptr, nullptr, tc.next()));
   return VDQN_OK;
 }
 
@@ -1345,20 +1365,22 @@
   hipStream_t ws = wgrad_stream(net, st);
   RC(run_wgrad(net, c2, bw, g_out, ao + A.h[b], n, ws));
   if (net->l_b_ds[b] >= 0) RC(run_wgrad(net, net->layers[net->l_b_ds[b]], bw, g_out, x, n, ws));
-  RC(run_dgrad(net, c2, pk, g_out, bw + W.g_h[b], n, nullptr, ao + A.h[b], st, bw + W.p_h[b]));
+  TileChain tc = {(tile_alternate_mask() & 2) != 0, net->dgrad_k};
+  RC(run_dgrad(net, c2, pk, g_out, bw + W.g_h[b], n, nullptr, ao + A.h[b], st, bw + W.p_h[b], nullptr, nullptr, nullptr, tc.next()));
+  net->dgrad_k += 2;
   ws = wgrad_stream(net, st);
   RC(run_wgrad(net, c1, bw, bw + W.g_h[b], x, n, ws));
   const void* resid = g_out;
   if (net->l_b_ds[b] >= 0) {
     const Layer& ds = net->layers[net->l_b_ds[b]];
     if (fuse_ds()) {
-      RC(run_dgrad(net, c1, pk, bw + W.g_h[b], gx, n, nullptr, x, st, b > 0 ? bw + W.p_o[b - 1] : bw + W.p_pool, &ds, g_out));
+      RC(run_dgrad(net, c1, pk, bw + W.g_h[b], gx, n, nullptr, x, st, b > 0 ? bw + W.p_o[b - 1] : bw + W.p_pool, &ds, g_out, nullptr, tc.next()));
       return VDQN_OK;
     }
-    RC(run_dgrad(net, ds, pk, g_out, bw + W.dsg[b], n, nullptr, nullptr, st));
+    RC(run_dgrad(net, ds, pk, g_out, bw + W.dsg[b], n, nullptr, nullptr, st, nullptr, nullptr, nullptr, nullptr, tc.same()));
     resid = bw + W.dsg[b];
   }
-  RC(run_dgrad(net, c1, pk, bw + W.g_h[b], gx, n, resid, x, st, b > 0 ? bw + W.p_o[b - 1] : bw + W.p_pool));
+  RC(run_dgrad(net, c1, pk, bw + W.g_h[b], gx, n, resid, x, st, b > 0 ? bw + W.p_o[b - 1] : bw + W.p_pool, nullptr, nullptr, nullptr, tc.next()));
   return VDQN_OK;
 }
 
@@ -1488,6 +1510,7 @@
     RC(run_dgrad(net, t0, pk, bw + W.g_l0, bw + W.g_f8, B, nullptr, ao + A.f8, st, bw + W.p_f8, nullptr, nullptr, &pr_f8));
     RC(run_wgrad(net, f8, bw, bw + W.g_f8, ao + A.o[7], n, wgrad_stream(net, st)));
     RC(run_dgrad(net, f8, pk, bw + W.g_f8, bw + W.g_o[7], n, nullptr, ao + A.o[7], st, bw + W.p_o[7]));
+    net->dgrad_k = 1;
     RC(block_backward(net, a, 7, A, W, n, st));
     RC(block_backward(net, a, 6, A, W, n, st));
   } else if (stage == 1) {
diff --git a/video_dqn_amd/csrc/igemm.hip b/video_dqn_amd/csrc/igemm.hip
--- a/video_dqn_amd/csrc/igemm.hip
+++ b/video_dqn_amd/csrc/igemm.hip
@@ -2,7 +2,7 @@
 
 #include "common.h"
 
-int vdqn_stem_bf16(const void* t_in, const void* wt, const float* bias, void* pool, void* idx, int n_img, int n_idx_img, hipStream_t st);
+int vdqn_stem_bf16(const void* t_in, const void* wt, const float* bias, void* pool, void* idx, int n_img, int n_idx_img, int tile_order, hipStream_t st);
 int vdqn_launch_win9s(const void* igemm_params, hipStream_t stream);
 int vdqn_win9s_supports(int cpk, int has_sib);
 int vdqn_launch_win9d(const void* igemm_params, hipStream_t stream);
@@ -34,7 +34,7 @@
 
   const int tid = threadIdx.x;
   const int lane = tid & 63, wave = tid >> 6;
-  const uint32_t lb = xcd_remap(blockIdx.x, gridDim.x);
+  const uint32_t lb = tile_walk(blockIdx.x, gridDim.x, (uint32_t)p.reverse);
   const int tile_n = (int)(lb % (uint32_t)p.tiles_n), tile_m = (int)(lb / (uint32_t)p.tiles_n);
   const bool sib = MODE == 0 && tile_n >= p.tiles_n1;
   const int n0 = (sib ? tile_n - p.tiles_n1 : tile_n) * BN;
@@ -515,7 +515,7 @@
 
   const int tid = threadIdx.x;
   const int lane = tid & 63, wave = tid >> 6;
-  const uint32_t lb = xcd_remap(blockIdx.x, gridDim.x);
+  const uint32_t lb = tile_walk(blockIdx.x, gridDim.x, (uint32_t)p.reverse);
   const int tile_n = (int)(lb % (uint32_t)p.tiles_n), tile_m = (int)(lb / (uint32_t)p.tiles_n);
   const int n0 = tile_n * BN, m0 = tile_m * BM;
   const int nk = p.nk;
@@ -762,7 +762,7 @@
     if (hwid_p & 1) __builtin_amdgcn_s_setprio(VDQN_PRIO);
   }
 #endif
-  const uint32_t lb = xcd_remap(blockIdx.x, gridDim.x);
+  const uint32_t lb = tile_walk(blockIdx.x, gridDim.x, (uint32_t)p.reverse);
   const int tile_n = (int)(lb % (uint32_t)p.tiles_n), tile_m = (int)(lb / (uint32_t)p.tiles_n);
   const int n0 = tile_n * BN, m0 = tile_m * BM;
   const int nk = p.nk;
@@ -1115,9 +1115,9 @@
   constexpr bool kSpread = VDQN_C64_SPREAD == 2 || (VDQN_C64_SPREAD == 1 && MODE == 0);
   const uint32_t c64_adv_oh = (uint32_t)((16 / W) % H), c64_adv_ow = (uint32_t)(16 - (16 / W) * W);
   int t = g_bid, buf = 0;
-  if (t < g_tiles) issue_window(g_first + (int)xcd_remap((uint32_t)t, (uint32_t)g_tiles), 0);
+  if (t < g_tiles) issue_window(g_first + (int)tile_walk((uint32_t)t, (uint32_t)g_tiles, (uint32_t)p.reverse), 0);
   for (; t < g_tiles; t += g_blocks, buf ^= 1) {
-    const int tl = g_first + (int)xcd_remap((uint32_t)t, (uint32_t)g_tiles);
+    const int tl = g_first + (int)tile_walk((uint32_t)t, (uint32_t)g_tiles, (uint32_t)p.reverse);
     const int m0 = tl * 128;
 #ifdef VDQN_STAMP
     const unsigned long long st_w0 = __builtin_amdgcn_s_memtime();
@@ -1130,7 +1130,7 @@
     if (st_row && tid == 0) { st_row[0] = st_w0; st_row[1] = __builtin_amdgcn_s_memtime(); }
 #endif
     const bool c64_has_nx = t + g_blocks < g_tiles;
-    const int c64_tl_nx = c64_has_nx ? g_first + (int)xcd_remap((uint32_t)(t + g_blocks), (uint32_t)g_tiles) : 0;
+    const int c64_tl_nx = c64_has_nx ? g_first + (int)tile_walk((uint32_t)(t + g_blocks), (uint32_t)g_tiles, (uint32_t)p.reverse) : 0;
     if constexpr (!kSpread) {
       if (c64_has_nx) issue_window(c64_tl_nx, buf ^ 1);
     }
@@ -1416,6 +1416,8 @@
   p.co2 = p.ldo2 = p.relu2 = p.ci2 = p.wt2_bytes = 0;
   static const int no_lean = [] { const char* e = getenv("VDQN_LEAN_EPILOGUE"); return (e && e[0] == '0') ? 1 : 0; }();
   p.no_lean = no_lean;
+  VDQN_CHECK(a->tile_order == 0 || a->tile_order == 1, "vdqn_conv2d: tile_order %d", a->tile_order);
+  p.reverse = a->tile_order;
   p.n_img = a->n_img; p.hi = a->hi; p.wi = a->wi; p.ci = a->ci; p.pix_stride = a->pix_stride;
   p.ho = a->ho; p.wo = a->wo; p.co = a->co; p.ldo = a->ldo; p.r = a->r; p.s = a->s; p.stride = a->stride; p.pad = a->pad;
   p.relu = a->relu;
@@ -1524,6 +1526,12 @@
 
 extern "C" int vdqn_stem_conv_pool_n(const void* t_in, const void* wt, const float* bias, void* pool, void* idx, int32_t n_img, int32_t n_idx_img,
                                      int32_t dtype, void* stream) {
+  return vdqn_stem_conv_pool_ord(t_in, wt, bias, pool, idx, n_img, n_idx_img, dtype, 0, stream);
+}
+
+extern "C" int vdqn_stem_conv_pool_ord(const void* t_in, const void* wt, const float* bias, void* pool, void* idx, int32_t n_img, int32_t n_idx_img,
+                                       int32_t dtype, int32_t tile_order, void* stream) {
+  VDQN_CHECK(tile_order == 0 || tile_order == 1, "vdqn_stem_conv_pool: tile_order %d", tile_order);
   VDQN_CHECK(t_in && wt && bias && pool && n_img > 0 && n_idx_img >= 0 && n_idx_img <= n_img && (idx || n_idx_img == 0), "vdqn_stem_conv_pool: bad args");
   VDQN_CHECK(dtype == VDQN_F32 || dtype == VDQN_BF16 || dtype == VDQN_F32X3, "vdqn_stem_conv_pool: bad dtype %d", dtype);
   VDQN_CHECK((((uintptr_t)t_in | (uintptr_t)wt | (uintptr_t)pool | (uintptr_t)idx) & 15) == 0, "vdqn_stem_conv_pool: tensors must be 16-byte aligned");
@@ -1543,9 +1551,10 @@
   p.in_bytes = (long long)n_img * 115 * 115 * 16 * esz;
   p.wt_bytes = 64 * p.ktot * esz;
   p.vec_ok = 1;
+  p.reverse = tile_order;
   hipStream_t st = (hipStream_t)stream;
   static const bool persistent = [] { const char* e = getenv("VDQN_STEM_PERSISTENT"); return !(e && e[0] == '0'); }();
-  if (dtype == VDQN_BF16 && persistent) return vdqn_stem_bf16(t_in, wt, bias, pool, idx, n_img, n_idx_img, st);
+  if (dtype == VDQN_BF16 && persistent) return vdqn_stem_bf16(t_in, wt, bias, pool, idx, n_img, n_idx_img, tile_order, st);
   if (dtype == VDQN_F32X3) return launch_igemm<float, 256, 64, 3, 2, true>(p, st);
   return dtype == VDQN_BF16 ? launch_igemm<bf16raw, 256, 64, 3>(p, st) : launch_igemm<float, 256, 64, 3>(p, st);
 }
diff --git a/video_dqn_amd/csrc/igemm_common.h b/video_dqn_amd/csrc/igemm_common.h
--- a/video_dqn_amd/csrc/igemm_common.h
+++ b/video_dqn_amd/csrc/igemm_common.h
@@ -31,6 +31,7 @@
   const float* bias2;
   void* out2;
   int co2, ldo2, relu2, ci2, wt2_bytes, tiles_n1;
+  int reverse;
   int no_lean;
 };
 
diff --git a/video_dqn_amd/csrc/pointwise.hip b/video_dqn_amd/csrc/pointwise.hip
--- a/video_dqn_amd/csrc/pointwise.hip
+++ b/video_dqn_amd/csrc/pointwise.hip
@@ -52,10 +52,11 @@
 
 constexpr int kPackPairs = 4;
 template <typename T>
-__global__ __launch_bounds__(256) void pack_input_rows_kernel(const uint8_t* __restrict__ src, T* __restrict__ dst) {
+__global__ __launch_bounds__(256) void pack_input_rows_kernel(const uint8_t* __restrict__ src, T* __restrict__ dst, const uint32_t reverse) {
   __shared__ uint4 rows[4][42];
   __shared__ T lut[3][256];
-  const int n = blockIdx.y;
+  const int n = (int)walk_pos(0u, gridDim.y, blockIdx.y, reverse);
+  const int bx = (int)walk_pos(0u, gridDim.x, blockIdx.x, reverse);
   const int tid = threadIdx.x;
   {
     const float mean[3] = {0.485f, 0.456f, 0.406f};
@@ -65,7 +66,7 @@
   }
   const int yy = tid / 115, x = tid - yy * 115;
   for (int pr = 0; pr < kPackPairs; ++pr) {
-    const int y0 = 2 * ((int)blockIdx.x * kPackPairs + pr);
+    const int y0 = 2 * (bx * kPackPairs + pr);
     if (y0 >= 115) break;
     const int Y0 = 2 * (y0 - 2);
     __syncthreads();
@@ -457,14 +458,20 @@
 }
 
 extern "C" int vdqn_pack_input(const void* src, int32_t src_kind, void* dst, int32_t n_img, int32_t dtype, void* stream) {
+  return vdqn_pack_input_ord(src, src_kind, dst, n_img, dtype, 0, stream);
+}
+
+extern "C" int vdqn_pack_input_ord(const void* src, int32_t src_kind, void* dst, int32_t n_img, int32_t dtype, int32_t tile_order, void* stream) {
   VDQN_CHECK(src && dst && n_img > 0, "vdqn_pack_input: bad args");
+  VDQN_CHECK(tile_order == 0 || tile_order == 1, "vdqn_pack_input: tile_order %d", tile_order);
+  const uint32_t rev = (uint32_t)tile_order;
   VDQN_CHECK(src_kind == 0 || src_kind == 1, "vdqn_pack_input: src_kind %d", src_kind);
   VDQN_CHECK(dtype == VDQN_F32 || dtype == VDQN_BF16, "vdqn_pack_input: bad dtype");
   const int g = grid_for((long)n_img * 115 * 115);
   ProfScope ps_("pack_input", 0.0, (double)n_img * (224.0 * 224 * 3 * (src_kind == 0 ? 1 : 4) + 115.0 * 115 * 16 * (dtype == VDQN_BF16 ? 2 : 4)), (hipStream_t)stream);
   if (src_kind == 0 && n_img <= 65535 && (((uintptr_t)src) & 15) == 0) {
-    if (dtype == VDQN_BF16) hipLaunchKernelGGL((pack_input_rows_kernel<bf16raw>), dim3((58 + kPackPairs - 1) / kPackPairs, n_img), dim3(256), 0, (hipStream_t)stream, (const uint8_t*)src, (bf16raw*)dst);
-    else hipLaunchKernelGGL((pack_input_rows_kernel<float>), dim3((58 + kPackPairs - 1) / kPackPairs, n_img), dim3(256), 0, (hipStream_t)stream, (const uint8_t*)src, (float*)dst);
+    if (dtype == VDQN_BF16) hipLaunchKernelGGL((pack_input_rows_kernel<bf16raw>), dim3((58 + kPackPairs - 1) / kPackPairs, n_img), dim3(256), 0, (hipStream_t)stream, (const uint8_t*)src, (bf16raw*)dst, rev);
+    else hipLaunchKernelGGL((pack_input_rows_kernel<float>), dim3((58 + kPackPairs - 1) / kPackPairs, n_img), dim3(256), 0, (hipStream_t)stream, (const uint8_t*)src, (float*)dst, rev);
     VDQN_LAUNCH_CHECK();
     return VDQN_OK;
   }
diff --git a/video_dqn_amd/csrc/stem.hip b/video_dqn_amd/csrc/stem.hip
--- a/video_dqn_amd/csrc/stem.hip
+++ b/video_dqn_amd/csrc/stem.hip
@@ -14,6 +14,7 @@
   uint8_t* idx;
   int n_img, n_tiles;
   int n_idx_img;
+  int reverse;
   void* stamps;
 };
 
@@ -28,6 +29,7 @@
 constexpr int kSmem = kXchOff + 3 * 7 * 128;
 constexpr unsigned kOobS = 0x80000000u;
 
+template <bool REV>
 __global__ __launch_bounds__(256, 2) void stem_kernel(const StemParams p) {
   extern __shared__ __attribute__((aligned(16))) unsigned char smem[];
   unsigned char* sW = smem;
@@ -90,9 +92,15 @@
   const int Tn = p.n_tiles - Ta, G = (int)gridDim.x, b0 = (int)blockIdx.x;
   const int ka = b0 < Ta ? (Ta - b0 + G - 1) / G : 0;
   const int kn = b0 < Tn ? (Tn - b0 + G - 1) / G : 0;
+  constexpr uint32_t rev = REV ? 1u : 0u;
   auto tile_at = [&](int k) {
-    if (k < ka) return (int)xcd_remap((uint32_t)(b0 + k * G), (uint32_t)Ta);
-    if (k < ka + kn) return Ta + (int)xcd_remap((uint32_t)(b0 + (k - ka) * G), (uint32_t)Tn);
+    if constexpr (!REV) {
+      if (k < ka) return (int)tile_walk((uint32_t)(b0 + k * G), (uint32_t)Ta, rev);
+      if (k < ka + kn) return Ta + (int)tile_walk((uint32_t)(b0 + (k - ka) * G), (uint32_t)Tn, rev);
+    } else {
+      if (k < kn) return Ta + (int)tile_walk((uint32_t)(b0 + k * G), (uint32_t)Tn, rev);
+      if (k < kn + ka) return (int)tile_walk((uint32_t)(b0 + (k - kn) * G), (uint32_t)Ta, rev);
+    }
     return -1;
   };
   auto tile = [&](auto kind, const int k, const u32x4 (&fb)[4][2][4]) {
@@ -333,28 +341,43 @@
 #endif
   };
   if (ka + kn > 0) issue_window(tile_at(0), 0);
-  if (ka > 0) {
-    u32x4 fb[4][2][4];
-    load_weights(fb);
-    for (int k = 0; k < ka; ++k) tile(KindArg{}, k, fb);
-  }
-  if (kn > 0) {
-    u32x4 fb[4][2][4];
-    load_weights(fb);
-    for (int k = ka; k < ka + kn; ++k) tile(KindPlain{}, k, fb);
+  if constexpr (!REV) {
+    if (ka > 0) {
+      u32x4 fb[4][2][4];
+      load_weights(fb);
+      for (int k = 0; k < ka; ++k) tile(KindArg{}, k, fb);
+    }
+    if (kn > 0) {
+      u32x4 fb[4][2][4];
+      load_weights(fb);
+      for (int k = ka; k < ka + kn; ++k) tile(KindPlain{}, k, fb);
+    }
+  } else {
+    if (kn > 0) {
+      u32x4 fb[4][2][4];
+      load_weights(fb);
+      for (int k = 0; k < kn; ++k) tile(KindPlain{}, k, fb);
+    }
+    if (ka > 0) {
+      u32x4 fb[4][2][4];
+      load_weights(fb);
+      for (int k = kn; k < kn + ka; ++k) tile(KindArg{}, k, fb);
+    }
   }
 }
 
 }
 
-int vdqn_stem_bf16(const void* t_in, const void* wt, const float* bias, void* pool, void* idx, int n_img, int n_idx_img, hipStream_t st) {
-  vdqn_ensure_dyn_smem(reinterpret_cast<const void*>(&stem_kernel), (size_t)kSmem);
+int vdqn_stem_bf16(const void* t_in, const void* wt, const float* bias, void* pool, void* idx, int n_img, int n_idx_img, int tile_order, hipStream_t st) {
+  auto kern = tile_order ? &stem_kernel<true> : &stem_kernel<false>;
+  vdqn_ensure_dyn_smem(reinterpret_cast<const void*>(kern), (size_t)kSmem);
   const int n_cu = vdqn_num_cus();
   StemParams p;
   p.t_in = (const bf16raw*)t_in; p.wt = (const bf16raw*)wt; p.bias = bias; p.pool = (bf16raw*)pool; p.idx = (uint8_t*)idx;
   p.n_img = n_img;
   p.n_idx_img = idx ? n_idx_img : 0;
   p.n_tiles = n_img * 64;
+  p.reverse = tile_order;
   p.stamps = nullptr;
 #ifdef VDQN_STAMP
   { extern void* g_stamp_buffer; p.stamps = g_stamp_buffer; }
@@ -362,7 +385,7 @@
   const int grid = p.n_tiles < 2 * n_cu ? p.n_tiles : 2 * n_cu;
   vdqn_prof_begin("stem_conv_pool<bf16>", 2.0 * n_img * 112 * 112 * 64 * 147,
                   2.0 * ((double)n_img * 115 * 115 * 16 + 64.0 * 256 + (double)n_img * 56 * 56 * 64) + (double)p.n_idx_img * 56 * 56 * 64, st);
-  hipLaunchKernelGGL(stem_kernel, dim3(grid), dim3(256), kSmem, st, p);
+  hipLaunchKernelGGL(kern, dim3(grid), dim3(256), kSmem, st, p);
   vdqn_prof_end(st);
   VDQN_LAUNCH_CHECK();
   return VDQN_OK;
diff --git a/video_dqn_amd/csrc/win9.hip b/video_dqn_amd/csrc/win9.hip
--- a/video_dqn_amd/csrc/win9.hip
+++ b/video_dqn_amd/csrc/win9.hip
@@ -43,6 +43,8 @@
   int tile_n, tile_m, n0, m0;
   const int m_end = p.M;
   if (lt >= x_count) return;
+  lt = walk_pos(0u, x_count, lt, (uint32_t)p.reverse);
+  const uint32_t x_step = p.reverse ? 0u - x_blocks : x_blocks;
   tile_n = (int)((x_first + lt) % (uint32_t)p.tiles_n);
   tile_m = (int)((x_first + lt) / (uint32_t)p.tiles_n);
   n0 = tile_n * BN;
@@ -258,7 +260,7 @@
 #pragma unroll
       for (int j = 0; j < NF; ++j) acc[f][j] = (f32x4){0.f, 0.f, 0.f, 0.f};
     VDQN_LOAD_FRAGS(0, 0, 0, 0)
-    const uint32_t lt_nx = lt + x_blocks;
+    const uint32_t lt_nx = lt + x_step;
     const bool has_nx = lt_nx < x_count;
     const int tn_nx = !has_nx ? tile_n : (int)((x_first + lt_nx) % (uint32_t)p.tiles_n);
     const int tm_nx = !has_nx ? tile_m : (int)((x_first + lt_nx) / (uint32_t)p.tiles_n);
diff --git a/video_dqn_amd/csrc/win9d.hip b/video_dqn_amd/csrc/win9d.hip
--- a/video_dqn_amd/csrc/win9d.hip
+++ b/video_dqn_amd/csrc/win9d.hip
@@ -50,6 +50,8 @@
     lt -= (uint32_t)grp * n_a;
   }
   if (lt >= x_count) return;
+  lt = walk_pos(0u, x_count, lt, (uint32_t)p.reverse);
+  if (p.reverse) lt_step = 0u - lt_step;
   int tile_n = (int)((x_first + lt) % (uint32_t)tiles_n), tile_m = (int)((x_first + lt) / (uint32_t)tiles_n);
   int n0 = tile_n * BN, m0 = tile_m * BM;
   const int Wo = p.wi, Ho = p.hi, Wi = p.wo;
diff --git a/video_dqn_amd/csrc/win9s.hip b/video_dqn_amd/csrc/win9s.hip
--- a/video_dqn_amd/csrc/win9s.hip
+++ b/video_dqn_amd/csrc/win9s.hip
@@ -29,7 +29,7 @@
   constexpr int PSTR = 32 * 128;
   extern __shared__ __attribute__((aligned(16))) unsigned char smem[];
   const int tid = threadIdx.x, lane = tid & 63, wave = tid >> 6;
-  const uint32_t lb = xcd_remap(blockIdx.x, gridDim.x);
+  const uint32_t lb = tile_walk(blockIdx.x, gridDim.x, (uint32_t)p.reverse);
   const int tile_n = (int)(lb % (uint32_t)p.tiles_n), tile_m = (int)(lb / (uint32_t)p.tiles_n);
   const int n0 = tile_n * BN, m0 = tile_m * BM;
   const int Wo = p.wo, rows_total = p.M;
@@ -224,6 +224,8 @@
   const uint32_t x_blocks = (gridDim.x >> 3) + (xcd < (gridDim.x & 7u) ? 1u : 0u);
   uint32_t lt = blockIdx.x >> 3;
   if (lt >= x_count) return;
+  lt = walk_pos(0u, x_count, lt, (uint32_t)p.reverse);
+  const uint32_t x_step = p.reverse ? 0u - x_blocks : x_blocks;
   int tile_n = (int)((x_first + lt) % (uint32_t)tiles_n), tile_m = (int)((x_first + lt) / (uint32_t)tiles_n);
   int n0 = tile_n * BN, m0 = tile_m * BM;
   const int Wo = p.wo, rows_total = p.M;
@@ -500,7 +502,7 @@
 #pragma unroll
       for (int j = 0; j < NF; ++j) acc[f][j] = (f32x4){0.f, 0.f, 0.f, 0.f};
     VDQN_P_LOAD_STEP(0, 0, 0)
-    const uint32_t lt_nx = lt + x_blocks;
+    const uint32_t lt_nx = lt + x_step;
     const bool has_nx = lt_nx < x_count;
     const int tn_nx = has_nx ? (int)((x_first + lt_nx) % (uint32_t)tiles_n) : tile_n;
     const int tm_nx = has_nx ? (int)((x_first + lt_nx) / (uint32_t)tiles_n) : tile_m;
diff --git a/video_dqn_amd/ops.py b/video_dqn_amd/ops.py
--- a/video_dqn_amd/ops.py
+++ b/video_dqn_amd/ops.py
@@ -35,7 +35,7 @@
            relu: bool = False, mode: int = 0, pix_stride: Optional[int] = None, ci: Optional[int] = None,
            want_f32: bool = False, ldo: Optional[int] = None, want_colsum: bool = False,
            wt2: Optional[torch.Tensor] = None, bias2: Optional[torch.Tensor] = None, co2: int = 0, relu2: bool = False,
-           in2: Optional[torch.Tensor] = None, precision: Optional[str] = None):
+           in2: Optional[torch.Tensor] = None, precision: Optional[str] = None, tile_order: int = 0):
     lib = _lib.load()
     require_gpu()
     n, hi, wi, cx = x.shape
@@ -51,6 +51,7 @@
     a.ho, a.wo, a.co, a.ldo = ho, wo, co, ldo
     a.r, a.s, a.stride, a.pad = r, s, stride, pad
     a.mode, a.relu, a.dtype = mode, int(relu), gemm_dtype_code(x, precision)
+    a.tile_order = int(tile_order)
     out2 = None
     if wt2 is not None and mode == 0:
         out2 = torch.empty((n, ho, wo, co2), dtype=x.dtype, device=x.device)
@@ -105,10 +106,10 @@
     return (dw, db) if want_dbias else dw
 
 
-def pack_input(src: torch.Tensor, src_kind: int, n_img: int, dtype: torch.dtype) -> torch.Tensor:
+def pack_input(src: torch.Tensor, src_kind: int, n_img: int, dtype: torch.dtype, tile_order: int = 0) -> torch.Tensor:
     lib = _lib.load()
     dst = torch.empty((n_img, 115, 115, 16), dtype=dtype, device=src.device)
-    _lib.check(lib.vdqn_pack_input(_ptr(src), src_kind, _ptr(dst), n_img, dtype_code(dst), _stream()), "vdqn_pack_input")
+    _lib.check(lib.vdqn_pack_input_ord(_ptr(src), src_kind, _ptr(dst), n_img, dtype_code(dst), int(tile_order), _stream()), "vdqn_pack_input")
     return dst
 
 
@@ -242,17 +243,17 @@
 
 
 def stem_conv_pool(t_in: torch.Tensor, wt: torch.Tensor, bias: torch.Tensor, want_idx: bool = True, n_idx: int = None,
-                   precision: Optional[str] = None):
+                   precision: Optional[str] = None, tile_order: int = 0):
     lib = _lib.load()
     n = t_in.shape[0]
     dt = gemm_dtype_code(t_in, precision)
     pool = torch.empty((n, 56, 56, 64), dtype=t_in.dtype, device=t_in.device)
     if n_idx is not None:
         idx = torch.zeros((n, 56, 56, 64), dtype=torch.uint8, device=t_in.device)
-        _lib.check(lib.vdqn_stem_conv_pool_n(_ptr(t_in), _ptr(wt), _ptr(bias), _ptr(pool), _ptr(idx), n, int(n_idx), dt, _stream()),
+        _lib.check(lib.vdqn_stem_conv_pool_ord(_ptr(t_in), _ptr(wt), _ptr(bias), _ptr(pool), _ptr(idx), n, int(n_idx), dt, int(tile_order), _stream()),
                    "vdqn_stem_conv_pool_n")
         return pool, idx
     idx = torch.empty((n, 56, 56, 64), dtype=torch.uint8, device=t_in.device) if want_idx else None
-    _lib.check(lib.vdqn_stem_conv_pool(_ptr(t_in), _ptr(wt), _ptr(bias), _ptr(pool), _ptr(idx) if want_idx else None, n, dt, _stream()),
-               "vdqn_stem_conv_pool")
+    _lib.check(lib.vdqn_stem_conv_pool_ord(_ptr(t_in), _ptr(wt), _ptr(bias), _ptr(pool), _ptr(idx) if want_idx else None, n, n if want_idx else 0, dt,
+                                           int(tile_order), _stream()), "vdqn_stem_conv_pool")
     return pool, idx
```

Measured after the change: 41320 tuples/s. 3.1% lower.
